# santiagolmedo/gnn_qot_estimation

Hardware: AMD Instinct MI355X
Metric: graphs/sec (train step) on 100-node/400-edge synthetic topologies, batch=1024 (higher is better)
Workload: dtype f32; 1 GPU; configs[1]: 2-layer TopologicalGNN (TransformerConv+NNConv) hidden=64, 100-node/400-directed-edge topologies, batch=1024 graphs per GPU, dropout 0.5, SGD momentum 0.9, SmoothL1; CSR build included in every step; graphs_per_gpu=1024, global_batch=1024, distinct_graphs_per_gpu=1024, launch=hip-graph replay, 4 whole steps (fwd+bwd+optimizer each) per graph, steps_per_graph=4, collective_in_graph=False, parallelism=dp1, prime_steps=45, collective_world_size=1, all_reduce_floats=68715

## Files before the change

### gnn_qot_estimation_amd/_lib.py

```python
from __future__ import annotations

import ctypes as C
import os
import subprocess

import torch

_HERE = os.path.dirname(os.path.abspath(__file__))
LIB_PATH = os.environ.get("QOT_LIB_PATH") or os.path.join(_HERE, "libqot_gnn.so")
CSRC_DIR = os.path.join(_HERE, "csrc")

_p = C.c_void_p
_i64 = C.c_int64
_int = C.c_int
_f = C.c_float
_u64 = C.c_uint64
_sz = C.c_size_t

ABI_VERSION = 11

SIGNATURES = {
    "qot_abi_version": (_int, []),
    "qot_error_string": (C.c_char_p, [_int]),
    "qot_csr_workspace_bytes": (_sz, [_i64, _i64, _int]),
    "qot_csr_build": (_int, [_p, _i64, _i64, _int, _p, _p, _p, _p, _p, _p, _p, _p, _p, _p, _sz, _p]),
    "qot_csr_gat_by_graph_supported": (_int, [_i64, _i64]),
    "qot_csr_build_gat_by_graph": (_int, [_p, _i64, _i64, _p, _p, _i64, _i64, _i64, _p, _p, _p, _p, _p, _p, _p, _p, _p, _p, _p,
                                          _p]),
    "qot_csr_build_by_graph": (_int, [_p, _i64, _i64, _p, _p, _i64, _i64, _i64, _p, _p, _p, _p, _p, _p, _p, _p, _p,
                                      _p, _p, _p, _p, _p, _p, _p]),
    "qot_i32_gather": (_int, [_p, _p, _p, _i64, _p]),
    "qot_i64_to_i32": (_int, [_p, _p, _i64, _p]),
    "qot_batch_ptr": (_int, [_p, _i64, _i64, _p, _p]),
    "qot_embed_fwd": (_int, [_p, _p, _p, _i64, _int, _int, _p]),
    "qot_embed_bwd": (_int, [_p, _p, _p, _i64, _int, _int, _p]),
    "qot_tconv_fwd_scores": (_int, [_p, _p, _p, _int, _p, _int, _p, _p, _p, _p, _p, _p, _p, _p, _i64, _int, _int,
                                    _int, _f, _f, _u64, _p, _p]),
    "qot_tconv_rows_supported": (_int, [_int, _int, _int]),
    "qot_tconv_rows_npad": (_int, [_int]),
    "qot_tconv_rows_ld": (_int, [_int, _int, _int]),
    "qot_tconv_bwd_dst_rows": (_int, [_p, _p, _p, _int, _p, _p, _p, _p, _p, _p, _p, _int, _p, _p, _p, _p, _f, _f, _u64, _p,
                                      _int, _i64, _int, _p, _p, _int, _int, _p]),
    "qot_tconv_fwd_rows": (_int, [_p, _p, _p, _int, _p, _int, _p, _p, _p, _p, _p, _p, _p, _int, _i64, _int, _int, _int,
                                  _int, _f, _f, _u64, _p, _p]),
    "qot_tconv_bwd_src_rows": (_int, [_p, _p, _p, _p, _p, _int, _i64, _int, _p, _int, _p]),
    "qot_tconv_fwd": (_int, [_p, _p, _p, _p, _int, _p, _p, _p, _p, _p, _p, _p, _p, _i64, _int, _int,
                             _int, _f, _f, _u64, _p, _p]),
    "qot_tconv_fwd_tile": (_int, [_p, _p, _p, _p, _int, _p, _p, _p, _p, _p, _p, _p, _p, _i64, _int, _int, _int, _i64,
                                  _int, _f, _f, _u64, _p, _p]),
    "qot_tconv_bwd_dst_workspace_floats": (_sz, [_i64, _int, _int]),
    "qot_tconv_rows_per_block": (_int, [_int]),
    "qot_tconv_bwd_dst_blocks": (_i64, [_i64, _int, _int, _i64]),
    "qot_tconv_bwd_dst": (_int, [_p, _p, _p, _p, _int, _p, _p, _p, _p, _p, _p, _p, _p, _p, _int, _p, _p, _p, _p,
                                 _p, _f, _f, _u64, _p, _p, _p, _int, _i64, _p, _i64, _int, _int, _p]),
    "qot_tconv_bwd_src": (_int, [_p, _int, _p, _int, _p, _p, _p, _p, _p, _p, _p, _p, _int, _int, _i64, _p, _i64, _int,
                                 _p]),
    "qot_tconv_graph_supported": (_int, [_int, _int, _int, _int]),
    "qot_tconv_graph_ldm": (_int, [_int]),
    "qot_tconv_graph_row_floats": (_sz, [_int, _int, _int]),
    "qot_tconv_bwd_graph_blocks": (_int, [_i64]),
    "qot_table_scores": (_int, [_p, _p, _p, _p, _p, _p, _p, _p, _int, _int, _int, _p]),
    "qot_tconv_fwd_graph": (_int, [_p, _int, _p, _p, _p, _p, _p, _p, _p, _p, _p, _p, _p, _p, _int, _i64, _int, _int, _int,
                                   _int, _f, _f, _u64, _p, _p]),
    "qot_tconv_bwd_graph": (_int, [_p, _p, _f, _f, _u64, _p, _p, _int, _p, _p, _p, _p, _p, _p, _p, _p, _p, _p, _p, _int,
                                   _i64, _int, _int, _int, _p]),
    "qot_table_project_bwd_scores": (_int, [_p, _p, _p, _p, _p, _p, _p, _p, _p, _p, _p, _p, _int, _int, _int, _int, _p]),
    "qot_nnconv_agg": (_int, [_p, _int, _p, _p, _p, _p, _p, _p, _p, _p, _int, _p, _i64, _int, _int, _p]),
    "qot_nnconv_fused": (_int, [_p, _int, _p, _p, _p, _p, _p, _p, _p, _int, _p, _p, _p, _i64, _int, _int,
                                _int, _f, _f, _u64, _p, _p]),
    "qot_nnconv_bwd_finalize": (_int, [_p, _p, _p, _p, _p, _i64, _int, _int, _p]),
    "qot_nnconv_dw_workspace_floats": (_sz, [_i64, _int, _int]),
    "qot_nnconv_dw": (_int, [_p, _int, _p, _int, _p, _p, _p, _p, _p, _p, _p, _p, _p, _i64, _int, _int, _p]),
    "qot_gemm_tn_workspace_floats": (_sz, [_int]),
    "qot_gemm_tn": (_int, [_p, _int, _p, _int, _i64, _int, _p, _p, _p]),
    "qot_nnconv_adjoint_dw_workspace_floats": (_sz, [_int]),
    "qot_nnconv_adjoint_dw": (_int, [_p, _int, _p, _int, _p, _p, _p, _p, _p, _p, _p, _p, _p, _p, _int, _p, _i64,
                                     _int, _int, _p]),
    "qot_nnconv_gradh_workspace_floats": (_sz, [_int]),
    "qot_nnconv_gradh_fused": (_int, [_p, _int, _p, _int, _p, _p, _p, _p, _p, _p, _p, _p, _p, _p, _p, _i64, _int,
                                      _int, _p]),
    "qot_nnconv_bwd_edge": (_int, [_p, _int, _p, _int, _p, _p, _p, _p, _p, _p, _p, _p, _p, _i64, _int,
                                   _int, _p]),
    "qot_tconv_edge_attr_grad": (_int, [_p, _p, _f, _f, _u64, _p, _p, _int, _p, _p, _p, _p, _p, _p, _p, _i64, _int, _int,
                                        _p]),
    "qot_nnconv_edge_attr_grad": (_int, [_p, _int, _p, _int, _p, _p, _p, _p, _p, _p, _p, _p, _i64, _int, _int, _p]),
    "qot_act_fwd": (_int, [_p, _p, _i64, _f, _f, _u64, _p, _p]),
    "qot_act_bwd": (_int, [_p, _p, _p, _i64, _f, _f, _u64, _p, _p]),
    "qot_pool_fwd": (_int, [_p, _p, _p, _i64, _int, _p]),
    "qot_pool_bwd": (_int, [_p, _p, _p, _p, _i64, _i64, _int, _p]),
    "qot_gat_blocks": (_int, [_i64, _int, _int]),
    "qot_gat_bn_partials_floats": (_sz, [_i64, _int, _int]),
    "qot_gat_logits": (_int, [_p, _p, _p, _p, _p, _i64, _int, _int, _p]),
    "qot_gat_fwd": (_int, [_p, _p, _p, _p, _p, _p, _p, _p, _i64, _int, _int, _f, _p, _p]),
    "qot_gat_att_grad": (_int, [_p, _p, _p, _p, _p, _p, _i64, _int, _int, _p]),
    "qot_gat_chunk_rows": (_i64, [_i64, _int, _int]),
    "qot_bn_stats_from_partials": (_int, [_p, _p, _int, _i64, _i64, _int, _f, _f, _p, _p, _p, _p, _p]),
    "qot_gat_thin_supported": (_int, [_int, _int, _int]),
    "qot_gat_fwd_thin": (_int, [_p, _int, _p, _p, _p, _p, _p, _p, _p, _p, _i64, _int, _int, _f, _p, _p]),
    "qot_gat_bwd_dst_thin": (_int, [_p, _p, _int, _p, _p, _p, _p, _p, _p, _p, _p, _p, _i64, _int, _int, _f, _p, _p, _p]),
    "qot_gat_bwd_dst": (_int, [_p, _p, _p, _p, _p, _p, _p, _p, _p, _p, _i64, _int, _int, _f, _p, _p, _p]),
    "qot_gat_bwd_src": (_int, [_p, _p, _p, _p, _p, _p, _p, _p, _p, _p, _i64, _int, _int, _f, _p, _p, _p, _p]),
    "qot_bn_partials_floats": (_sz, [_i64, _int]),
    "qot_bn_stats": (_int, [_p, _i64, _int, _f, _f, _p, _p, _p, _p, _p, _p]),
    "qot_bn_apply": (_int, [_p, _p, _p, _p, _p, _p, _i64, _int, _int, _p]),
    "qot_bn_bwd_reduce": (_int, [_p, _p, _p, _p, _p, _p, _p, _i64, _int, _int, _p, _p, _p, _p]),
    "qot_bn_bwd_apply": (_int, [_p, _p, _p, _p, _p, _p, _p, _p, _p, _i64, _int, _int, _int, _p, _p]),
    "qot_bn_apply_rows": (_int, [_p, _p, _i64, _p, _p, _p, _p, _p, _int, _int, _p]),
    "qot_bn_bwd_reduce_rows": (_int, [_p, _p, _i64, _p, _p, _p, _p, _p, _int, _int, _p, _p, _p, _p]),
    "qot_bn_bwd_apply_rows": (_int, [_p, _p, _i64, _p, _p, _p, _p, _p, _p, _p, _i64, _int, _int, _p, _p]),
    "qot_sgd_momentum": (_int, [_p, _p, _p, _i64, _f, _f, _int, _p]),
    "qot_sgd_momentum_multi": (_int, [_p, _p, _p, _int, _p, _p, _i64, _f, _p, _f, _int, _p]),
    "qot_sgd_momentum_dev": (_int, [_p, _p, _p, _i64, _p, _f, _int, _p]),
    "qot_small_gemm": (_int, [_p, _i64, _i64, _p, _i64, _i64, _p, _p, _int, _int, _int, _int, _int, _p]),
    "qot_colsum_workspace_floats": (_sz, [_int]),
    "qot_colsum": (_int, [_p, _int, _i64, _int, _p, _p, _p]),
    "qot_rowsum_wide_workspace_floats": (_sz, [_i64]),
    "qot_rowsum_wide": (_int, [_p, _i64, _i64, _p, _p, _p]),
    "qot_head_fwd": (_int, [_p, _p, _p, _p, _p, _p, _p, _p, _p, _i64, _int, _int, _f, _f, _u64, _p, _p]),
    "qot_head_fwd_loss": (_int, [_p, _p, _p, _p, _p, _p, _p, _p, _p, _i64, _int, _int, _f, _f, _u64, _p, _p, _f, _p, _p, _p]),
    "qot_head_train": (_int, [_p, _p, _p, _p, _p, _p, _p, _f, _p, _p, _p, _p, _p, _i64, _int, _int, _f, _f, _u64, _p, _int,
                              _f, _f, _u64, _p, _p]),
    "qot_head_train_blocks": (_int, [_i64, _int]),
    "qot_head_bwd_workspace_floats": (_sz, [_int, _int]),
    "qot_head_bwd_blocks": (_int, [_i64]),
    "qot_head_bwd": (_int, [_p, _p, _p, _p, _p, _p, _p, _p, _p, _i64, _int, _int, _f, _f, _u64, _p,
                            _p, _f, _f, _u64, _p, _p]),
    "qot_act_bwd_colsum": (_int, [_p, _p, _p, _i64, _int, _f, _f, _u64, _p, _p, _p, _p]),
    "qot_smooth_l1_workspace_floats": (_sz, []),
    "qot_smooth_l1": (_int, [_p, _p, _i64, _f, _p, _p, _p, _p]),
    "qot_table_project_fwd": (_int, [_p, _p, _p, _p, _p, _p, _p, _p, _p, _p, _int, _int, _p, _p, _p]),
    "qot_table_project_bwd": (_int, [_p, _p, _p, _p, _p, _p, _p, _p, _p, _int, _int, _p]),
    "qot_table_maps": (_int, [_p, _p, _p, _p, _p, _p, _i64, _i64, _p]),
    "qot_step_advance": (_int, [_p, _p, _p]),
    "qot_gather3": (_int, [_p, _i64, _p, _i64, _p, _p, _p, _i64, _p]),
    "qot_gemm_nt": (_int, [_p, _i64, _p, _i64, _p, _i64, _i64, _int, _int, _p, _p, _p, _p]),
    "qot_gemm_nt_planes": (_int, [_p, _i64, _p, _i64, _p, _i64, _int, _int, _int, _p]),
    "qot_gemm_tn_splits": (_int, [_int, _int, _i64]),
    "qot_gemm256_takes": (_int, [_i64, _int]),
    "qot_gemm_tn_planes": (_int, [_p, _i64, _p, _i64, _p, _int, _int, _i64, _int, _p, _p, _p]),
    "qot_skinny_linear_fwd": (_int, [_p, _p, _p, _i64, _int, _int, _p]),
    "qot_skinny_linear_fwd_logits": (_int, [_p, _p, _p, _i64, _int, _int, _p, _p, _p, _p, _p]),
    "qot_gemm_nt_logits": (_int, [_p, _i64, _p, _i64, _p, _i64, _i64, _int, _int, _p, _p, _p, _p, _p, _p, _p, _p]),
    "qot_skinny_linear_dw_blocks": (_int, [_i64]),
    "qot_skinny_linear_dw": (_int, [_p, _p, _p, _i64, _int, _int, _p]),
    "qot_run_roles": (_int, [_p, _int, _p]),
    "qot_rows_gather": (_int, [_p, _p, _p, _i64, _int, _p]),
    "qot_rows_scatter": (_int, [_p, _p, _p, _i64, _int, _p]),
}

MAX_ROLES = 12
(ROLE_CSR_BY_GRAPH, ROLE_TABLE_PROJECT_FWD, ROLE_GATHER3, ROLE_SUM_ROWS, ROLE_NNCONV_FINALIZE64, ROLE_TABLE_PROJECT_BWD,
 ROLE_TABLE_SCORES, ROLE_TABLE_PROJECT_BWD_SCORES) = range(1, 9)


class Role(C.Structure):
    _fields_ = [("kind", C.c_int32), ("reserved", C.c_int32), ("p", C.c_void_p * 18), ("i", C.c_int64 * 8)]


def make_role(kind: int, ptrs, ints) -> Role:
    r = Role()
    r.kind = kind
    for k, t in enumerate(ptrs):
        r.p[k] = None if t is None else (t.data_ptr() if isinstance(t, torch.Tensor) else int(t))
    for k, v in enumerate(ints):
        r.i[k] = int(v)
    return r


def run_roles(roles, stream_handle=None):
    if not roles:
        return
    if len(roles) > MAX_ROLES:
        for k in range(0, len(roles), MAX_ROLES):
            run_roles(roles[k:k + MAX_ROLES], stream_handle)
        return
    arr = (Role * len(roles))(*roles)
    code = (_lib or load()).qot_run_roles(C.addressof(arr), len(roles), stream() if stream_handle is None else stream_handle)
    if code != 0:
        check(code, "qot_run_roles")


_lib = None


class QotError(RuntimeError):
    """A libqot_gnn entry point returned a non-zero status."""


def build_library(verbose: bool = False) -> str:
    cmd = ["make", "-C", CSRC_DIR, "-j", str(min(8, os.cpu_count() or 1))]
    res = subprocess.run(cmd, capture_output=True, text=True)
    if res.returncode != 0:
        raise RuntimeError("building libqot_gnn.so failed:\n" + res.stdout[-4000:] + res.stderr[-8000:])
    if verbose:
        print(res.stdout[-2000:])
    return LIB_PATH


def load():
    global _lib
    if _lib is not None:
        return _lib
    if not os.path.exists(LIB_PATH):
        raise QotError(
            f"{LIB_PATH} not found: build it with `python -c 'import __graft_entry__ as g; g.build()'` "
            "or `make -C gnn_qot_estimation_amd/csrc` -- there is no CPU fallback for the HIP path"
        )
    lib = C.CDLL(LIB_PATH)
    for name, (res, args) in SIGNATURES.items():
        fn = getattr(lib, name)
        fn.restype = res
        fn.argtypes = args
    if lib.qot_abi_version() != ABI_VERSION:
        raise QotError(f"libqot_gnn ABI version {lib.qot_abi_version()} != {ABI_VERSION} expected by this package: "
                       "rebuild with `make -C gnn_qot_estimation_amd/csrc`")
    _lib = lib
    return lib


def ptr(t):
    return None if t is None else t.data_ptr()


_raw_stream = getattr(torch._C, "_cuda_getCurrentRawStream", None)
_raw_device = getattr(torch._C, "_cuda_getDevice", None)


def stream():
    if _raw_stream is not None and _raw_device is not None:
        return _raw_stream(_raw_device())
    return torch.cuda.current_stream().cuda_stream


def check(code: int, what: str):
    if code != 0:
        msg = load().qot_error_string(code).decode()
        raise QotError(f"{what} failed with status {code}: {msg}")


def call(name: str, *args):
    if any(isinstance(a, torch.Tensor) for a in args):
        raw = tuple(a.data_ptr() if isinstance(a, torch.Tensor) else a for a in args)
    else:
        raw = args
    code = getattr(_lib or load(), name)(*raw, stream())
    if code != 0:
        check(code, name)
```

### gnn_qot_estimation_amd/csrc/nnconv_gradh64.hip

```cpp
#include "common.hpp"
#include "mfma_tile.hpp"

namespace qot {

constexpr int kGaLd = 516;

constexpr int kGhCap = 256;

template <int D, int VARIANT = 0>
__global__ __launch_bounds__(256, 2) void nnconv_gradh64_kernel(
    const float* __restrict__ g, int ldg, const float* __restrict__ x, int ldx, const float* __restrict__ ea,
    const float* __restrict__ w1, const float* __restrict__ b1, const int32_t* __restrict__ rowptr,
    const int32_t* __restrict__ col, const int32_t* __restrict__ eidx, const float* __restrict__ invdeg,
    const float* __restrict__ Bp, float* __restrict__ partials, int64_t N) {
    constexpr int K = 2 * D;
    static_assert(K <= 8, "one k per lane of the 8-lane group");
    constexpr int NB = K * 2;
    constexpr int NBW = NB / 4;
    constexpr int EPG = kGhCap / 32;
    constexpr int EPF = 5;
    __shared__ __attribute__((aligned(16))) float Gt[8 * 2 * 32 * 4];
    __shared__ __attribute__((aligned(16))) float GAt[32 * (K * 64 + 4)];
    __shared__ int sj[kGhCap], sr[kGhCap];
    __shared__ __attribute__((aligned(16))) float sea[kGhCap * D];
    __shared__ int rp_l[36];
    constexpr int LDGA = K * 64 + 4;
    float4* Gt4 = reinterpret_cast<float4*>(Gt);
    const int lane = threadIdx.x & 63, wave = threadIdx.x >> 6;
    const int r31 = lane & 31, hi = lane >> 5;
    const int sub = threadIdx.x & 7, il = threadIdx.x >> 3;
    const int c0 = 8 * sub;
    const int64_t ntiles = (N + 31) / 32;

    float wrow[D], brow, aw[D], ab = 0.f;
    brow = (sub < K) ? b1[sub] : 0.f;
#pragma unroll
    for (int d = 0; d < D; ++d) { wrow[d] = (sub < K) ? w1[sub * D + d] : 0.f; aw[d] = 0.f; }

    auto edge = [&](int r, const float4& x0, const float4& x1, const float (&ee)[D]) {
        float pd[8];
#pragma unroll
        for (int k = 0; k < 8; ++k) {
            float a = 0.f;
            if (k < K) {
                const float4 u0 = *reinterpret_cast<const float4*>(&GAt[r * LDGA + k * 64 + c0]);
                const float4 u1 = *reinterpret_cast<const float4*>(&GAt[r * LDGA + k * 64 + c0 + 4]);
                float a0 = u0.x * x0.x, a1 = u0.y * x0.y;
                a0 = fmaf(u0.z, x0.z, a0); a1 = fmaf(u0.w, x0.w, a1);
                a0 = fmaf(u1.x, x1.x, a0); a1 = fmaf(u1.y, x1.y, a1);
                a0 = fmaf(u1.z, x1.z, a0); a1 = fmaf(u1.w, x1.w, a1);
                a = a0 + a1;
            }
            pd[k] = a;
        }
        float t4[4];
#pragma unroll
        for (int m = 0; m < 4; ++m) {
            const float keep = (sub & 4) ? pd[m + 4] : pd[m];
            const float send = (sub & 4) ? pd[m] : pd[m + 4];
            t4[m] = keep + dpp_move<0x141>(send);
        }
        float t2[2];
#pragma unroll
        for (int m = 0; m < 2; ++m) {
            const float keep = (sub & 2) ? t4[m + 2] : t4[m];
            const float send = (sub & 2) ? t4[m] : t4[m + 2];
            t2[m] = keep + dpp_move<0x4E>(send);
        }
        const float keep = (sub & 1) ? t2[1] : t2[0];
        const float send = (sub & 1) ? t2[0] : t2[1];
        const float tot = keep + dpp_move<0xB1>(send);
        float pre = brow;
#pragma unroll
        for (int d = 0; d < D; ++d) pre = fmaf(wrow[d], ee[d], pre);
        const float gh = (pre > 0.f && sub < K) ? tot : 0.f;
        ab += gh;
#pragma unroll
        for (int d = 0; d < D; ++d) aw[d] = fmaf(gh, ee[d], aw[d]);
    };

#pragma unroll 1
    for (int64_t it = 0;; ++it) {
        const int64_t tile = xcd_tile(it, ntiles);
        if (tile < 0) break;
        const int64_t tile0 = tile * 32;
        const int64_t i = tile0 + il;
        const int64_t tend = (tile0 + 32 < N) ? tile0 + 32 : N;
        float4 bf[2][8];
        {
            const float4* bp = reinterpret_cast<const float4*>(Bp) + (int64_t)(wave * NBW) * 8 * 64 + lane;
#pragma unroll
            for (int gq = 0; gq < 8; ++gq) bf[0][gq] = bp[gq * 64];
        }
        const int e_t0 = rowptr[tile0], e_t1 = rowptr[tend];
        const int nt = e_t1 - e_t0;
        const int ncap = nt < kGhCap ? nt : kGhCap;
        int64_t my_e = 0;
        if ((int)threadIdx.x < ncap) {
            sj[threadIdx.x] = col[e_t0 + threadIdx.x];
            my_e = eidx[e_t0 + threadIdx.x];
        }
        if (threadIdx.x < 33) rp_l[threadIdx.x] = rowptr[tile0 + threadIdx.x < N ? tile0 + threadIdx.x : N];
        {
            float4 g0 = f4zero(), g1 = f4zero();
            if (i < N) {
                const float sc = invdeg[i];
                const int beg = rowptr[i], end = rowptr[i + 1];
                g0 = scale4(sc, ld4(g + i * ldg + c0)); g1 = scale4(sc, ld4(g + i * ldg + c0 + 4));
                const int lim = e_t0 + ncap;
                for (int p = beg + sub; p < end && p < lim; p += 8) sr[p - e_t0] = il;
            }
            Gt4[at4_slot(sub, 0, il)] = make_float4(g0.x, g0.z, g1.x, g1.z);
            Gt4[at4_slot(sub, 1, il)] = make_float4(g0.y, g0.w, g1.y, g1.w);
        }
        float my_ea[D];
#pragma unroll
        for (int d = 0; d < D; ++d) my_ea[d] = ((int)threadIdx.x < ncap) ? ea[my_e * D + d] : 0.f;
        lds_barrier();
        const int mine = (ncap - il + 31) / 32;
        float4 xr0[EPF], xr1[EPF];
#pragma unroll
        for (int t = 0; t < EPF; ++t) {
            if (t < mine) {
                const float* xp = x + (int64_t)sj[il + 32 * t] * ldx + c0;
                xr0[t] = ld4(xp); xr1[t] = ld4(xp + 4);
            }
        }
        if (VARIANT != 3) {
            float4 af[8];
#pragma unroll
            for (int gq = 0; gq < 8; ++gq) af[gq] = Gt4[at4_slot(gq, hi, r31)];
#pragma unroll
            for (int t = 0; t < NBW; ++t) {
                const int nb = wave * NBW + t;
                if (t + 1 < NBW) {
                    const float4* bp = reinterpret_cast<const float4*>(Bp) +
                                       (int64_t)((VARIANT == 5) ? wave * NBW : nb + 1) * 8 * 64 + lane;
#pragma unroll
                    for (int gq = 0; gq < 8; ++gq) bf[(t + 1) & 1][gq] = bp[gq * 64];
                }
                f32x16 c;
#pragma unroll
                for (int r = 0; r < 16; ++r) c[r] = 0.f;
#pragma unroll
                for (int gq = 0; gq < 8; ++gq) {
                    c = __builtin_amdgcn_mfma_f32_32x32x2f32(af[gq].x, bf[t & 1][gq].x, c, 0, 0, 0);
                    c = __builtin_amdgcn_mfma_f32_32x32x2f32(af[gq].y, bf[t & 1][gq].y, c, 0, 0, 0);
                    c = __builtin_amdgcn_mfma_f32_32x32x2f32(af[gq].z, bf[t & 1][gq].z, c, 0, 0, 0);
                    c = __builtin_amdgcn_mfma_f32_32x32x2f32(af[gq].w, bf[t & 1][gq].w, c, 0, 0, 0);
                }
#pragma unroll
                for (int r = 0; r < 16; ++r) {
                    const int row = (r & 3) + 8 * (r >> 2) + 4 * hi;
                    GAt[row * LDGA + nb * 32 + r31] = c[r];
                }
            }
        }
        if ((int)threadIdx.x < ncap) {
#pragma unroll
            for (int d = 0; d < D; ++d) sea[threadIdx.x * D + d] = my_ea[d];
        }
        lds_barrier();
        if (VARIANT != 2) {
#pragma unroll
            for (int t = 0; t < EPF; ++t) {
                if (t < mine) {
                    const int s = il + 32 * t;
                    float ee[D];
#pragma unroll
                    for (int d = 0; d < D; ++d) ee[d] = sea[s * D + d];
                    edge(sr[s], xr0[t], xr1[t], ee);
                }
            }
            for (int t = EPF; t < mine; ++t) {
                const int s = il + 32 * t;
                const float* xp = x + (int64_t)sj[s] * ldx + c0;
                const float4 y0 = ld4(xp), y1 = ld4(xp + 4);
                float ee[D];
#pragma unroll
                for (int d = 0; d < D; ++d) ee[d] = sea[s * D + d];
                edge(sr[s], y0, y1, ee);
            }
            for (int s = kGhCap + il; s < nt; s += 32) {
                const int pp = e_t0 + s;
                int lo = 0;
#pragma unroll
                for (int st = 16; st > 0; st >>= 1)
                    if (rp_l[lo + st] <= pp) lo += st;
                const int64_t e = eidx[pp];
                const float* xp = x + (int64_t)col[pp] * ldx + c0;
                const float4 y0 = ld4(xp), y1 = ld4(xp + 4);
                float ee[D];
#pragma unroll
                for (int d = 0; d < D; ++d) ee[d] = ea[e * D + d];
                edge(lo, y0, y1, ee);
            }
        }
        lds_barrier();
    }
    float* red = GAt;
#pragma unroll
    for (int d = 0; d < D; ++d) red[(d * 32 + il) * 8 + sub] = aw[d];
    red[(D * 32 + il) * 8 + sub] = ab;
    lds_barrier();
    if (threadIdx.x < (D + 1) * 8) {
        const int s8 = threadIdx.x & 7, d = threadIdx.x >> 3;
        float sum = 0.f;
        for (int g32 = 0; g32 < 32; ++g32) sum += red[(d * 32 + g32) * 8 + s8];
        if (s8 < K) partials[(int64_t)blockIdx.x * (K * (D + 1)) + (d < D ? s8 * D + d : K * D + s8)] = sum;
    }
}

}

using namespace qot;

int qot_nnconv_gradh64_launch(const float* grad_out, int ld_g, const float* x, int ld_x, const float* edge_attr, const float* w1,
                              const float* b1, const int32_t* rowptr, const int32_t* col, const int32_t* eid, const float* invdeg,
                              const float* b_perm, float* workspace, int64_t N, int D, int grid, int variant, hipStream_t stream) {
#ifdef QOT_DIAG
    if (variant >= 1 && variant <= 5 && D == 4) {
#define QOT_GH_V(V) nnconv_gradh64_kernel<4, V><<<grid, 256, 0, stream>>>(grad_out, ld_g, x, ld_x, edge_attr, w1, b1, rowptr, col, \
                                                                        eid, invdeg, b_perm, workspace, N)
        switch (variant) {
            case 1: QOT_GH_V(1); break;
            case 2: QOT_GH_V(2); break;
            case 3: QOT_GH_V(3); break;
            case 4: QOT_GH_V(4); break;
            default: QOT_GH_V(5); break;
        }
#undef QOT_GH_V
        QOT_LAUNCH_CHECK();
        return QOT_OK;
    }
#endif
    (void)variant;
    QOT_DISPATCH_D(D, {
        if (kD <= 4)
            nnconv_gradh64_kernel<(kD <= 4 ? kD : 4)><<<grid, 256, 0, stream>>>(
                grad_out, ld_g, x, ld_x, edge_attr, w1, b1, rowptr, col, eid, invdeg, b_perm, workspace, N);
    });
    QOT_LAUNCH_CHECK();
    return QOT_OK;
}
```

### gnn_qot_estimation_amd/csrc/nnconv_mfma.hip

```cpp
#include "common.hpp"
#include "mfma_tile.hpp"
#include "nnconv_finalize_dev.hpp"

namespace qot {

template <int D, bool TRANSPOSE, int GV = 0>
__device__ __forceinline__ void nnconv_gather_tile(
    float* __restrict__ At, const float* __restrict__ x, int ldx, const float* __restrict__ ea,
    const float* __restrict__ w1, const float* __restrict__ b1, const int32_t* __restrict__ rowptr,
    const int32_t* __restrict__ col, const int32_t* __restrict__ eidx, const float* __restrict__ invdeg,
    int64_t tile0, int64_t N, float4& root0, float4& root1) {
    constexpr int K = 2 * D;
    const int sub = threadIdx.x & 7, il = threadIdx.x >> 3;
    const int c0 = 8 * sub;
    const int64_t i = tile0 + il;
    float4 acc0[K + 1], acc1[K + 1];
    root0 = f4zero(); root1 = f4zero();
    int beg = 0, end = 0;
    float srow = 0.f;
    if (i < N) {
        beg = rowptr[i]; end = rowptr[i + 1];
        if (!TRANSPOSE) srow = invdeg[i];
        root0 = ld4(x + i * ldx + c0);
        root1 = ld4(x + i * ldx + c0 + 4);
    }
    const int own = (i < N) ? (int)i : 0;
#define QOT_ACC(FIRSTSLOT, H, X, A) ((FIRSTSLOT) ? scale4((H), (X)) : fma4((H), (X), (A)))
#define QOT_EDGE4(U0, FIRST)                                                                            \
        {                                                                                               \
            float4 xa[4], xb[4];                                                                        \
            float sc[4];                                                                                \
            int jj[4];                                                                                  \
            jj[0] = group8_bcast<U0 + 0>(myj); jj[1] = group8_bcast<U0 + 1>(myj);                       \
            jj[2] = group8_bcast<U0 + 2>(myj); jj[3] = group8_bcast<U0 + 3>(myj);                       \
            sc[0] = group8_bcast<U0 + 0>(mysc); sc[1] = group8_bcast<U0 + 1>(mysc);                     \
            sc[2] = group8_bcast<U0 + 2>(mysc); sc[3] = group8_bcast<U0 + 3>(mysc);                     \
            _Pragma("unroll") for (int u = 0; u < 4; ++u) {                                             \
                const float* xr = x + (int64_t)(GV == 6 ? (jj[u] & 1) : jj[u]) * ldx + c0;              \
                xa[u] = ld4(xr);                                                                        \
                xb[u] = ld4(xr + 4);                                                                    \
            }                                                                                           \
            _Pragma("unroll") for (int kk = 0; kk < (GV == 8 ? 1 : K); ++kk) {                          \
                const float h0 = group8_bcast<U0 + 0>(myh[kk]), h1 = group8_bcast<U0 + 1>(myh[kk]);     \
                acc0[kk] = QOT_ACC(FIRST, h0, xa[0], acc0[kk]); acc1[kk] = QOT_ACC(FIRST, h0, xb[0], acc1[kk]); \
                acc0[kk] = fma4(h1, xa[1], acc0[kk]); acc1[kk] = fma4(h1, xb[1], acc1[kk]);             \
            }                                                                                           \
            if (GV == 8 && (FIRST)) {                                                                   \
                _Pragma("unroll") for (int kk = 1; kk < K; ++kk) { acc0[kk] = f4zero(); acc1[kk] = f4zero(); } \
            }                                                                                           \
            acc0[K] = QOT_ACC(FIRST, sc[0], xa[0], acc0[K]); acc1[K] = QOT_ACC(FIRST, sc[0], xb[0], acc1[K]); \
            acc0[K] = fma4(sc[1], xa[1], acc0[K]); acc1[K] = fma4(sc[1], xb[1], acc1[K]);               \
             \
             \
            if (cnt > U0 + 2) {                                                                         \
                _Pragma("unroll") for (int kk = 0; kk < (GV == 8 ? 1 : K); ++kk) {                      \
                    const float h2 = group8_bcast<U0 + 2>(myh[kk]), h3 = group8_bcast<U0 + 3>(myh[kk]); \
                    acc0[kk] = fma4(h2, xa[2], acc0[kk]); acc1[kk] = fma4(h2, xb[2], acc1[kk]);         \
                    acc0[kk] = fma4(h3, xa[3], acc0[kk]); acc1[kk] = fma4(h3, xb[3], acc1[kk]);         \
                }                                                                                       \
                _Pragma("unroll") for (int u = 2; u < 4; ++u) {                                         \
                    acc0[K] = fma4(sc[u], xa[u], acc0[K]);                                              \
                    acc1[K] = fma4(sc[u], xb[u], acc1[K]);                                              \
                }                                                                                       \
            }                                                                                           \
        }
#define QOT_FWD_BATCH(FIRST)                                                                            \
    {                                                                                                   \
        const int p = base + sub;                                                                       \
        int myj = own;                                                                                  \
        float myh[K], mysc = 0.f;                                                                       \
        _Pragma("unroll") for (int kk = 0; kk < K; ++kk) myh[kk] = 0.f;                                 \
        if (p < end) {                                                                                  \
            myj = (GV == 7) ? (int)(i ^ (p & 31)) : col[p];                                             \
            const int64_t e = (GV == 7) ? (int64_t)p : (int64_t)eidx[p];                                \
            float ee[D];                                                                                \
            _Pragma("unroll") for (int d = 0; d < D; ++d) ee[d] = ea[e * D + d];                        \
            mysc = TRANSPOSE ? invdeg[myj] : srow;                                                      \
            _Pragma("unroll") for (int kk = 0; kk < K; ++kk) {                                          \
                float h = b1[kk];                                                                       \
                _Pragma("unroll") for (int d = 0; d < D; ++d) h = fmaf(w1[kk * D + d], ee[d], h);       \
                myh[kk] = fmaxf(h, 0.f) * mysc;                                                         \
            }                                                                                           \
        }                                                                                               \
        const int cnt = (end - base < 8) ? end - base : 8;                                              \
        QOT_EDGE4(0, FIRST)                                                                             \
        if (cnt > 4) QOT_EDGE4(4, false)                                                                \
    }
    int base = beg;
    QOT_FWD_BATCH(true)
    for (base = beg + 8; base < end; base += 8) QOT_FWD_BATCH(false)
#undef QOT_FWD_BATCH
#undef QOT_EDGE4
#undef QOT_ACC
    float4* At4 = reinterpret_cast<float4*>(At);
#pragma unroll
    for (int kk = 0; kk <= K; ++kk) {
        const int g = kk * 8 + sub;
        At4[at4_slot(g, 0, il)] = make_float4(acc0[kk].x, acc0[kk].z, acc1[kk].x, acc1[kk].z);
        At4[at4_slot(g, 1, il)] = make_float4(acc0[kk].y, acc0[kk].w, acc1[kk].y, acc1[kk].w);
    }
}

#ifdef QOT_DIAG
#define QOT_DIAG_SECTION 1
#include "diag/nnconv_mfma_diag.inc"
#undef QOT_DIAG_SECTION
#endif

#ifdef QOT_DIAG
#define QOT_DIAG_SECTION 2
#include "diag/nnconv_mfma_diag.inc"
#undef QOT_DIAG_SECTION
#else
#define QOT_STAMP(slot)
#endif

template <int D, bool TRANSPOSE, int VARIANT = 0>
__global__ __launch_bounds__(256, 2) void nnconv_mfma64_kernel(
    const float* __restrict__ x, int ldx, const float* __restrict__ ea, const float* __restrict__ w1,
    const float* __restrict__ b1, const int32_t* __restrict__ rowptr, const int32_t* __restrict__ col,
    const int32_t* __restrict__ eidx, const float* __restrict__ invdeg, const float* __restrict__ Wp,
    const float* __restrict__ bias, float* __restrict__ out, int64_t N, ActParams act) {
    constexpr int K = 2 * D;
    constexpr int KM = (K + 1) * 64;
    constexpr int GM = KM / 16;
    constexpr int CH = 4;
    __shared__ __attribute__((aligned(16))) float At[KM * 32];
    const int64_t ntiles = (N + 31) / 32;
    const float bz = bias ? bias[((threadIdx.x >> 6) & 1) * 32 + (threadIdx.x & 31)] : 0.f;
    const uint64_t drop_step = (act.enabled && act.thr16) ? (uint64_t)act.step[0] : 0;
#pragma unroll 1
    for (int64_t it = 0;; ++it) {
    const int64_t tile = xcd_tile(it, ntiles);
    if (tile < 0) break;
    const int64_t tile0 = tile * 32;
    float4 root0, root1;
    unsigned long long t_prev = 0;
    if (VARIANT == 3 || VARIANT == 9) t_prev = __builtin_amdgcn_s_memtime();

#ifdef QOT_DIAG
    if (VARIANT == 11) {
        nnconv_gather_tile_rank1_shape<D>(At, x, ldx, rowptr, col, tile0, N, root0, root1);
    } else
#endif
    if (VARIANT != 1 && VARIANT != 4 && VARIANT != 5 && VARIANT != 9) {
        nnconv_gather_tile<D, TRANSPOSE, (VARIANT >= 6 && VARIANT <= 8) ? VARIANT : 0>(At, x, ldx, ea, w1, b1, rowptr, col, eidx, invdeg, tile0, N, root0, root1);
    } else {
        for (int t = threadIdx.x; t < KM * 32; t += 256) At[t] = 1.0f + (float)(t & 7);
        root0 = root1 = make_float4(1.f, 1.f, 1.f, 1.f);
    }
    const float4* At4 = reinterpret_cast<const float4*>(At);
    const int lane = threadIdx.x & 63, wave = threadIdx.x >> 6;
    const int nh = wave & 1, kh = wave >> 1;
    const int r31 = lane & 31, hi = lane >> 5;
    const float4* wpn = reinterpret_cast<const float4*>(Wp) + (int64_t)nh * (2 * GM + 8) * 64 + lane;
    const float4* wp = wpn + (int64_t)kh * GM * 64;
    const float4* rbp = wpn + (int64_t)(2 * GM + kh * 4) * 64;
    asm volatile("" : "+v"(rbp));
    float4 rb[4];
#pragma unroll
    for (int u = 0; u < 4; ++u) rb[u] = rbp[u * 64];
    constexpr int NCH = GM / CH;
    constexpr int NB = 4;
    float4 bb[NB][CH];
#pragma unroll
    for (int q = 0; q < NB - 1; ++q)
#pragma unroll
        for (int u = 0; u < CH; ++u) bb[q][u] = wp[(q * CH + u) * 64];
    QOT_STAMP(0)
    lds_barrier();
    QOT_STAMP(1)
    if (VARIANT == 2) {
        if (threadIdx.x < 32 && tile0 + threadIdx.x < N) out[(tile0 + threadIdx.x) * 64] = At[threadIdx.x * 33] + root0.x + rb[0].x + bb[0][0].x;
        __syncthreads();
        continue;
    }

    f32x16 c;
#pragma unroll
    for (int r = 0; r < 16; ++r) c[r] = 0.f;
    int ch = 0;
#pragma unroll 1
    for (; ch + NB <= NCH; ch += NB) {
#pragma unroll
        for (int q = 0; q < NB; ++q) {
            if (ch + q + NB - 1 < NCH && VARIANT != 4 && VARIANT != 5 && VARIANT != 9) {
#pragma unroll
                for (int u = 0; u < CH; ++u) bb[(q + NB - 1) % NB][u] = wp[((ch + q + NB - 1) * CH + u) * 64];
            }
#pragma unroll
            for (int u = 0; u < CH; ++u) {
                if (VARIANT == 5 || VARIANT == 9) {
                    const float4 a = rb[u & 3], b = bb[q][u];
                    c = __builtin_amdgcn_mfma_f32_32x32x2f32(a.x, b.x, c, 0, 0, 0);
                    c = __builtin_amdgcn_mfma_f32_32x32x2f32(a.y, b.y, c, 0, 0, 0);
                    c = __builtin_amdgcn_mfma_f32_32x32x2f32(a.z, b.z, c, 0, 0, 0);
                    c = __builtin_amdgcn_mfma_f32_32x32x2f32(a.w, b.w, c, 0, 0, 0);
                } else {
                    c = mfma_group(At4, kh * GM + (ch + q) * CH + u, hi, r31, bb[q][u], c);
                }
            }
        }
    }
#pragma unroll
    for (int q = 0; q < NB - 1; ++q) {
        if (ch + q < NCH) {
#pragma unroll
            for (int u = 0; u < CH; ++u) c = mfma_group(At4, kh * GM + (ch + q) * CH + u, hi, r31, bb[q][u], c);
        }
    }
    QOT_STAMP(2)
    lds_barrier();
    QOT_STAMP(3)
    {
        float4* At4 = reinterpret_cast<float4*>(At);
        const int sub = threadIdx.x & 7, il = threadIdx.x >> 3;
        At4[at4_slot(sub, 0, il)] = make_float4(root0.x, root0.z, root1.x, root1.z);
        At4[at4_slot(sub, 1, il)] = make_float4(root0.y, root0.w, root1.y, root1.w);
    }
    __syncthreads();
#pragma unroll
    for (int u = 0; u < 4; ++u) c = mfma_group(At4, kh * 4 + u, hi, r31, rb[u], c);
    QOT_STAMP(4)
    float* red = At + 64 * 32;
    if (kh) {
#pragma unroll
        for (int r = 0; r < 8; ++r) red[((2 + nh) * 8 + r) * 64 + lane] = c[r];
    } else {
#pragma unroll
        for (int r = 0; r < 8; ++r) red[(nh * 8 + r) * 64 + lane] = c[8 + r];
    }
    lds_barrier();
    {
        const int colg = nh * 32 + r31;
        float v[8];
        if (kh) {
#pragma unroll
            for (int r = 0; r < 8; ++r) v[r] = c[8 + r] + red[(nh * 8 + r) * 64 + lane] + bz;
        } else {
#pragma unroll
            for (int r = 0; r < 8; ++r) v[r] = c[r] + red[((2 + nh) * 8 + r) * 64 + lane] + bz;
        }
        uint32_t zlo[8], zhi[8];
        const bool drop = act.enabled && act.thr16;
        if (drop) {
            const int jq = r31 & 3;
            uint32_t mylo[2], myhi[2];
#pragma unroll
            for (int t = 0; t < 2; ++t) {
                const int rr = kh * 8 + 2 * jq + t;
                const int row = (rr & 3) + 8 * (rr >> 2) + 4 * hi;
                const uint64_t flat = (uint64_t)((tile0 + row) * 64 + colg);
                const uint64_t z = act_hash64(act.seed, drop_step, flat >> 2);
                mylo[t] = (uint32_t)z; myhi[t] = (uint32_t)(z >> 32);
            }
#define QOT_ZSHARE(S)                                                                                   \
            zlo[2 * (S)] = __builtin_amdgcn_update_dpp(0, mylo[0], (S) * 0x55, 0xF, 0xF, true);         \
            zhi[2 * (S)] = __builtin_amdgcn_update_dpp(0, myhi[0], (S) * 0x55, 0xF, 0xF, true);         \
            zlo[2 * (S) + 1] = __builtin_amdgcn_update_dpp(0, mylo[1], (S) * 0x55, 0xF, 0xF, true);     \
            zhi[2 * (S) + 1] = __builtin_amdgcn_update_dpp(0, myhi[1], (S) * 0x55, 0xF, 0xF, true);
            QOT_ZSHARE(0) QOT_ZSHARE(1) QOT_ZSHARE(2) QOT_ZSHARE(3)
#undef QOT_ZSHARE
        }
#pragma unroll
        for (int r = 0; r < 8; ++r) {
            const int rr = kh * 8 + r;
            const int row = (rr & 3) + 8 * (rr >> 2) + 4 * hi;
            const int64_t i = tile0 + row;
            float y = v[r];
            if (act.enabled) {
                y = y > 0.f ? y : act.slope * y;
                if (drop) {
                    const uint64_t z = ((uint64_t)zhi[r] << 32) | zlo[r];
                    const bool keep = ((uint32_t)(z >> (16 * (colg & 3))) & 0xFFFFu) >= act.thr16;
                    y = keep ? y * act.keep_scale : 0.f;
                }
            }
            if (i < N) out[i * 64 + colg] = y;
        }
    }
    QOT_STAMP(5)
    lds_barrier();
    QOT_STAMP(6)
    }
}


template <int D, int VARIANT = 0>
__global__ __launch_bounds__(512, 2) void nnconv_adjoint_dw64_kernel(
    const float* __restrict__ g, int ldg, const float* __restrict__ xf, int ldx, const float* __restrict__ ea,
    const float* __restrict__ w1, const float* __restrict__ b1, const int32_t* __restrict__ rowptr_t,
    const int32_t* __restrict__ col_t, const int32_t* __restrict__ eid_t, const float* __restrict__ invdeg,
    const float* __restrict__ Wp, float* __restrict__ gx, float* __restrict__ slabs, int64_t N) {
    constexpr int K = 2 * D;
    constexpr int KT = (K + 2) * 64;
    constexpr int GQ = KT / 8 / 4;
    constexpr int MB = KT / 32;
    constexpr int TPW = MB * 2 / 8;
    static_assert(GQ % 4 == 0 || GQ % 5 == 0, "chunking");
    constexpr int CH = (GQ % 4 == 0) ? 4 : 5;
    __shared__ __attribute__((aligned(16))) float Ut[KT * 32];
    __shared__ __attribute__((aligned(16))) float red[8 * 3 * 4 * 64];
    __shared__ __attribute__((aligned(16))) float xs[32 * 64];
    float4* Ut4 = reinterpret_cast<float4*>(Ut);
    const int lane = threadIdx.x & 63, wave = threadIdx.x >> 6;
    const int r31 = lane & 31, hi = lane >> 5;
    const int nh = wave & 1, kq = wave >> 1;
    const int ah = wave & 1, mb0 = wave >> 1;
    const int64_t ntiles = (N + 31) / 32;

    f32x16 dw[TPW];
#pragma unroll
    for (int t = 0; t < TPW; ++t)
#pragma unroll
        for (int r = 0; r < 16; ++r) dw[t][r] = 0.f;
    int dwoff[4];
    {
        const int kcol = mb0 * 32 + r31;
        const int gg = kcol >> 3, within = kcol & 7;
        const int base0 = ((2 * gg + (within & 1)) * 32) * 4 + (within >> 1);
        const int m = gg & 7;
#pragma unroll
        for (int b = 0; b < 4; ++b) dwoff[b] = base0 + ((((b ^ (m >> 1)) << 1) | (hi ^ (m & 1))) << 2);
    }
    const float4* wp = reinterpret_cast<const float4*>(Wp) + ((int64_t)nh * (KT / 8) + kq * GQ) * 64 + lane;
#ifdef QOT_ADJ_SETPRIO
    if (wave >= 4) __builtin_amdgcn_s_setprio(1);
#endif

#pragma unroll 1
    for (int64_t it = 0;; ++it) {
        const int64_t tile = xcd_tile(it, ntiles);
        if (tile < 0) break;
        const int64_t tile0 = tile * 32;
        float4 xown;
        {
            const int64_t j = tile0 + (threadIdx.x >> 4);
            xown = (j < N) ? ld4(xf + j * ldx + 4 * (threadIdx.x & 15)) : f4zero();
        }
        if (VARIANT != 4) {
            const int sub = threadIdx.x & 15, il = threadIdx.x >> 4;
            const int c0 = 4 * sub;
            const int64_t j = tile0 + il;
            float4 acc[K + 2];
            acc[K + 1] = f4zero();
            int beg = 0, end = 0;
            if (j < N) { beg = rowptr_t[j]; end = rowptr_t[j + 1]; acc[K + 1] = ld4(g + j * ldg + c0); }
            const int own = (j < N) ? (int)j : 0;
#define QOT_ADJ_EDGE(U)                                                                                  \
                {                                                                                        \
                    const int64_t i = (VARIANT == 1) ? (int64_t)(row16_bcast<U>(myi) & 1) : (int64_t)row16_bcast<U>(myi); \
                    gr[(U) & 3] = ld4(g + i * ldg + c0);                                                 \
                    sc[(U) & 3] = row16_bcast<U>(mysc);                                                  \
                }
#define QOT_ADJ_FMA(U, FIRSTSLOT)                                                                        \
                {                                                                                        \
                    _Pragma("unroll") for (int kk = 0; kk < (VARIANT == 6 ? 1 : K); ++kk)                \
                        acc[kk] = (FIRSTSLOT) ? scale4(row16_bcast<U>(myh[kk]), gr[(U) & 3])             \
                                              : fma4(row16_bcast<U>(myh[kk]), gr[(U) & 3], acc[kk]);     \
                    if (VARIANT == 6 && (FIRSTSLOT)) {                                                   \
                        _Pragma("unroll") for (int kk = 1; kk < K; ++kk) acc[kk] = f4zero();             \
                    }                                                                                    \
                    acc[K] = (FIRSTSLOT) ? scale4(sc[(U) & 3], gr[(U) & 3]) : fma4(sc[(U) & 3], gr[(U) & 3], acc[K]); \
                }
#define QOT_ADJ_EDGE4(U0, FIRST)                                                                         \
                {                                                                                        \
                    float4 gr[4];                                                                        \
                    float sc[4];                                                                         \
                    QOT_ADJ_EDGE(U0) QOT_ADJ_EDGE(U0 + 1) QOT_ADJ_EDGE(U0 + 2) QOT_ADJ_EDGE(U0 + 3)      \
                    QOT_ADJ_FMA(U0, FIRST) QOT_ADJ_FMA(U0 + 1, false)                                    \
                     \
                     \
                    if (cnt > U0 + 2) { QOT_ADJ_FMA(U0 + 2, false) QOT_ADJ_FMA(U0 + 3, false) }          \
                }
#define QOT_ADJ_BATCH(FIRST)                                                                             \
            {                                                                                            \
                const int p = base + sub;                                                                \
                int myi = own;                                                                           \
                float myh[K], mysc = 0.f;                                                                \
                _Pragma("unroll") for (int kk = 0; kk < K; ++kk) myh[kk] = 0.f;                          \
                if (p < end) {                                                                           \
                    myi = (VARIANT == 7) ? (int)(j ^ (p & 31)) : col_t[p];        \
                    const int64_t e = (VARIANT == 7) ? (int64_t)p : (int64_t)eid_t[p];                   \
                    float ee[D];                                                                         \
                    _Pragma("unroll") for (int d = 0; d < D; ++d) ee[d] = ea[e * D + d];                 \
                    mysc = (VARIANT == 7) ? 0.25f : invdeg[myi];                                         \
                    _Pragma("unroll") for (int kk = 0; kk < K; ++kk) {                                   \
                        float h = b1[kk];                                                                \
                        _Pragma("unroll") for (int d = 0; d < D; ++d) h = fmaf(w1[kk * D + d], ee[d], h); \
                        myh[kk] = fmaxf(h, 0.f) * mysc;                                                  \
                    }                                                                                    \
                }                                                                                        \
                const int cnt = (end - base < 16) ? end - base : 16;                                     \
                QOT_ADJ_EDGE4(0, FIRST)                                                                  \
                if (cnt > 4) QOT_ADJ_EDGE4(4, false)                                                     \
                if (cnt > 8) QOT_ADJ_EDGE4(8, false)                                                     \
                if (cnt > 12) QOT_ADJ_EDGE4(12, false)                                                   \
            }
            int base = beg;
            QOT_ADJ_BATCH(true)
            for (base = beg + 16; base < end; base += 16) QOT_ADJ_BATCH(false)
#undef QOT_ADJ_BATCH
#undef QOT_ADJ_EDGE4
#undef QOT_ADJ_FMA
#undef QOT_ADJ_EDGE
#pragma unroll
            for (int kk = 0; kk < K + 2; ++kk) {
                const int gg = kk * 8 + (sub >> 1);
                float2* s0 = reinterpret_cast<float2*>(&Ut4[at4_slot(gg, 0, il)]) + (sub & 1);
                float2* s1 = reinterpret_cast<float2*>(&Ut4[at4_slot(gg, 1, il)]) + (sub & 1);
                *s0 = make_float2(acc[kk].x, acc[kk].z);
                *s1 = make_float2(acc[kk].y, acc[kk].w);
            }
        }
        {
            const int sub = threadIdx.x & 15, il = threadIdx.x >> 4;
            *reinterpret_cast<float4*>(&xs[il * 64 + 4 * sub]) = xown;
        }
        constexpr int NCH = GQ / CH;
        float4 bc[CH], bn[CH];
#pragma unroll
        for (int u = 0; u < CH; ++u) bc[u] = wp[u * 64];
        lds_barrier();
        f32x16 c;
#pragma unroll
        for (int r = 0; r < 16; ++r) c[r] = 0.f;
        if (VARIANT != 2 && VARIANT != 5) {
            int ch = 0;
#pragma unroll 1
            for (; ch + 1 < NCH; ch += 2) {
#pragma unroll
                for (int u = 0; u < CH; ++u) bn[u] = wp[((ch + 1) * CH + u) * 64];
#pragma unroll
                for (int u = 0; u < CH; ++u) c = mfma_group(Ut4, kq * GQ + ch * CH + u, hi, r31, bc[u], c);
                if (ch + 2 < NCH) {
#pragma unroll
                    for (int u = 0; u < CH; ++u) bc[u] = wp[((ch + 2) * CH + u) * 64];
                }
#pragma unroll
                for (int u = 0; u < CH; ++u) c = mfma_group(Ut4, kq * GQ + (ch + 1) * CH + u, hi, r31, bn[u], c);
            }
            if (NCH & 1) {
#pragma unroll
                for (int u = 0; u < CH; ++u) c = mfma_group(Ut4, kq * GQ + (NCH - 1) * CH + u, hi, r31, bc[u], c);
            }
        }
#define QOT_GIVE(OWNER, SLOT)                                                                        \
        _Pragma("unroll") for (int rr = 0; rr < 4; ++rr)                                             \
            red[((((OWNER) * 2 + nh) * 3 + (SLOT)) * 4 + rr) * 64 + lane] = c[4 * (OWNER) + rr];
        if (kq == 0) { QOT_GIVE(1, 0) QOT_GIVE(2, 0) QOT_GIVE(3, 0) }
        else if (kq == 1) { QOT_GIVE(0, 0) QOT_GIVE(2, 1) QOT_GIVE(3, 1) }
        else if (kq == 2) { QOT_GIVE(0, 1) QOT_GIVE(1, 1) QOT_GIVE(3, 2) }
        else { QOT_GIVE(0, 2) QOT_GIVE(1, 2) QOT_GIVE(2, 2) }
#undef QOT_GIVE
        if (VARIANT != 3 && VARIANT != 5) {
            float abuf[2][TPW], xbuf[2];
            const float* xsl = xs + hi * 64 + ah * 32 + r31;
#pragma unroll
            for (int t = 0; t < TPW; ++t) abuf[0][t] = Ut[dwoff[0] + t * 4096];
            xbuf[0] = xsl[0];
#pragma unroll
            for (int sidx = 0; sidx < 16; ++sidx) {
                const int cur = sidx & 1;
                if (sidx + 1 < 16) {
                    const int sn = sidx + 1;
#pragma unroll
                    for (int t = 0; t < TPW; ++t) abuf[cur ^ 1][t] = Ut[dwoff[sn & 3] + (sn >> 2) * 32 + t * 4096];
                    xbuf[cur ^ 1] = xsl[sn * 128];
                }
                __builtin_amdgcn_sched_barrier(0);
#pragma unroll
                for (int t = 0; t < TPW; ++t)
                    dw[t] = __builtin_amdgcn_mfma_f32_32x32x2f32(abuf[cur][t], xbuf[cur], dw[t], 0, 0, 0);
                __builtin_amdgcn_sched_barrier(0);
            }
        }
        lds_barrier();
        {
            float v[4];
            if (kq == 0) { v[0] = c[0]; v[1] = c[1]; v[2] = c[2]; v[3] = c[3]; }
            else if (kq == 1) { v[0] = c[4]; v[1] = c[5]; v[2] = c[6]; v[3] = c[7]; }
            else if (kq == 2) { v[0] = c[8]; v[1] = c[9]; v[2] = c[10]; v[3] = c[11]; }
            else { v[0] = c[12]; v[1] = c[13]; v[2] = c[14]; v[3] = c[15]; }
            const int colg = nh * 32 + r31;
#pragma unroll
            for (int rr = 0; rr < 4; ++rr) {
#pragma unroll
                for (int slot = 0; slot < 3; ++slot) v[rr] += red[(((kq * 2 + nh) * 3 + slot) * 4 + rr) * 64 + lane];
                const int reg = 4 * kq + rr;
                const int row = (reg & 3) + 8 * (reg >> 2) + 4 * hi;
                const int64_t j = tile0 + row;
                if (j < N) gx[j * 64 + colg] = v[rr];
            }
        }
        lds_barrier();
    }
    float* slab = slabs + (int64_t)blockIdx.x * KT * 64;
#pragma unroll
    for (int t = 0; t < TPW; ++t)
#pragma unroll
        for (int r = 0; r < 16; ++r) {
            const int row = (r & 3) + 8 * (r >> 2) + 4 * hi;
            slab[((mb0 + 4 * t) * 32 + row) * 64 + ah * 32 + r31] = dw[t][r];
        }
}

__global__ void adj_slab_reduce_kernel(const float* __restrict__ slabs, int nslabs, int per_group, int64_t elems,
                                       int64_t slab_stride, float* __restrict__ dst, int64_t dst_stride) {
    int64_t t = blockIdx.x * (int64_t)blockDim.x + threadIdx.x;
    if (t * 4 >= elems) return;
    const int s0 = blockIdx.y * per_group;
    int s1 = s0 + per_group;
    if (s1 > nslabs) s1 = nslabs;
    float4 acc = f4zero();
    int sidx = s0;
    for (; sidx + 8 <= s1; sidx += 8) {
        float4 v[8];
#pragma unroll
        for (int u = 0; u < 8; ++u) v[u] = ld4(slabs + (int64_t)(sidx + u) * slab_stride + 4 * t);
#pragma unroll
        for (int u = 0; u < 8; ++u) acc = add4(acc, v[u]);
    }
    for (; sidx < s1; ++sidx) acc = add4(acc, ld4(slabs + (int64_t)sidx * slab_stride + 4 * t));
    st4(dst + blockIdx.y * dst_stride + 4 * t, acc);
}

__global__ void adj_slab_final_params_kernel(const float* __restrict__ slabs, int nslabs, int64_t elems,
                                             int64_t slab_stride, float* __restrict__ dst, int K) {
    int64_t t = blockIdx.x * (int64_t)blockDim.x + threadIdx.x;
    if (t * 4 >= elems) return;
    float4 acc = f4zero();
    for (int sidx = 0; sidx < nslabs; ++sidx) acc = add4(acc, ld4(slabs + (int64_t)sidx * slab_stride + 4 * t));
    const int64_t e = 4 * t;
    const int a0 = (int)(e & 63), o = (int)((e >> 6) & 63), kb = (int)(e >> 12);
    const float v[4] = {acc.x, acc.y, acc.z, acc.w};
#pragma unroll
    for (int c = 0; c < 4; ++c) {
        const int a = a0 + c;
        int64_t idx;
        if (kb < K) idx = ((int64_t)a * 64 + o) * K + kb;
        else if (kb == K) idx = (int64_t)4096 * K + a * 64 + o;
        else idx = (int64_t)4096 * (K + 1) + o * 64 + a;
        dst[idx] = v[c];
    }
}

__global__ void gradh_partial_sum_kernel(const float* __restrict__ partials, int nblk, int n, int KD,
                                         float* __restrict__ gw1, float* __restrict__ gb1) {
    const int t = blockIdx.x * (blockDim.x >> 6) + (threadIdx.x >> 6);
    if (t >= n) return;
    const float s = wave_sum_partials(partials, nblk, n, t);
    if ((threadIdx.x & 63) == 0) { if (t < KD) gw1[t] = s; else gb1[t - KD] = s; }
}

}

using namespace qot;

int qot_nnconv_gen_launch(const float* x, int ld_x, const float* edge_attr, const float* w1, const float* b1,
                          const int32_t* rowptr, const int32_t* col, const int32_t* edge_ids, const float* invdeg,
                          int transpose, const float* w_perm, const float* bias, float* out, int64_t N, int H, int D,
                          const ActParams& ap, hipStream_t stream);
int qot_nnconv_gradh_gen_launch(const float* grad_out, int ld_g, const float* x, int ld_x, const float* edge_attr,
                                const float* w1, const float* b1, const int32_t* rowptr, const int32_t* col,
                                const int32_t* eid, const float* invdeg, const float* b_perm, float* gw1, float* gb1,
                                float* workspace, int64_t N, int H, int D, hipStream_t stream);

#ifdef QOT_DIAG
extern "C" int qot_nnconv_fused_ws(const float* x, int ld_x, const float* edge_attr, const float* w1,
                                   const float* b1, const int32_t* rowptr, const int32_t* col,
                                   const int32_t* edge_ids, const float* invdeg, int transpose,
                                   const float* w_perm, const float* bias, float* out, int64_t N, int H, int D,
                                   int act, float act_slope, float act_p, uint64_t act_seed,
                                   const int64_t* act_step, qot_stream_t stream);

static int g_variant = 0;
extern "C" void qot_debug_set_variant(int v) { g_variant = v; }
extern "C" void qot_debug_stamps(unsigned long long* host8, int reset) {
    if (reset) { unsigned long long z[8] = {0}; (void)hipMemcpyToSymbol(HIP_SYMBOL(qot::g_stamps), z, sizeof(z)); }
    else (void)hipMemcpyFromSymbol(host8, HIP_SYMBOL(qot::g_stamps), 8 * sizeof(unsigned long long));
}
#endif

extern "C" int qot_nnconv_fused(const float* x, int ld_x, const float* edge_attr, const float* w1,
                                const float* b1, const int32_t* rowptr, const int32_t* col,
                                const int32_t* edge_ids, const float* invdeg, int transpose,
                                const float* w_perm, const float* bias, float* out, int64_t N, int H, int D,
                                int act, float act_slope, float act_p, uint64_t act_seed,
                                const int64_t* act_step, qot_stream_t stream) {
    if (N < 0 || !rowptr) return QOT_ERR_BADARG;
    if (H != 16 && H != 32 && H != 64 && H != 128 && H != 256) return QOT_ERR_UNSUPPORTED;
    if (N == 0) return QOT_OK;
    if (!x || !w1 || !b1 || !invdeg || !w_perm || !out || (ld_x & 3)) return QOT_ERR_BADARG;
    if (H != 64 || transpose == 2 || transpose == 3) {
        if (D > 4) return QOT_ERR_UNSUPPORTED;
        return qot_nnconv_gen_launch(x, ld_x, edge_attr, w1, b1, rowptr, col, edge_ids, invdeg, transpose & 1, w_perm,
                                     bias, out, N, H, D, make_act(act, act_slope, act_p, act_seed, act_step),
                                     (hipStream_t)stream);
    }
#ifdef QOT_DIAG
    static int use_ws = -1;
    if (use_ws < 0) { const char* e = getenv("QOT_NNCONV_WS"); use_ws = (e && e[0] == '1') ? 1 : 0; }
    if (use_ws && D <= 4 && !g_variant)
        return qot_nnconv_fused_ws(x, ld_x, edge_attr, w1, b1, rowptr, col, edge_ids, invdeg, transpose, w_perm, bias,
                                   out, N, H, D, act, act_slope, act_p, act_seed, act_step, stream);
#endif
    int grid = grid_for(N, 32);
    if (grid > 2 * num_cus()) grid = 2 * num_cus();
    const ActParams ap = make_act(act, act_slope, act_p, act_seed, act_step);
#ifdef QOT_DIAG
    if (g_variant >= 100 && g_variant < 110 && D == 4 && !transpose) {
        const int v = g_variant - 100, g1 = grid > num_cus() ? num_cus() : grid;
        if (v == 0)
            nnconv_mfma64_kernel<4, false, 0><<<g1, 256, 0, (hipStream_t)stream>>>(
                x, ld_x, edge_attr, w1, b1, rowptr, col, edge_ids, invdeg, w_perm, bias, out, N, ap);
        else if (v == 1)
            nnconv_mfma64_kernel<4, false, 1><<<g1, 256, 0, (hipStream_t)stream>>>(
                x, ld_x, edge_attr, w1, b1, rowptr, col, edge_ids, invdeg, w_perm, bias, out, N, ap);
        else if (v == 4)
            nnconv_mfma64_kernel<4, false, 4><<<g1, 256, 0, (hipStream_t)stream>>>(
                x, ld_x, edge_attr, w1, b1, rowptr, col, edge_ids, invdeg, w_perm, bias, out, N, ap);
        else if (v == 5)
            nnconv_mfma64_kernel<4, false, 5><<<g1, 256, 0, (hipStream_t)stream>>>(
                x, ld_x, edge_attr, w1, b1, rowptr, col, edge_ids, invdeg, w_perm, bias, out, N, ap);
        else if (v == 9)
            nnconv_mfma64_kernel<4, false, 9><<<g1, 256, 0, (hipStream_t)stream>>>(
                x, ld_x, edge_attr, w1, b1, rowptr, col, edge_ids, invdeg, w_perm, bias, out, N, ap);
        else
            nnconv_mfma64_kernel<4, false, 2><<<g1, 256, 0, (hipStream_t)stream>>>(
                x, ld_x, edge_attr, w1, b1, rowptr, col, edge_ids, invdeg, w_perm, bias, out, N, ap);
        QOT_LAUNCH_CHECK();
        return QOT_OK;
    }
    if (g_variant && g_variant <= 10 && D == 4 && !transpose) {
        if (g_variant == 3)
            nnconv_mfma64_kernel<4, false, 3><<<grid, 256, 0, (hipStream_t)stream>>>(
                x, ld_x, edge_attr, w1, b1, rowptr, col, edge_ids, invdeg, w_perm, bias, out, N, ap);
        else if (g_variant == 1)
            nnconv_mfma64_kernel<4, false, 1><<<grid, 256, 0, (hipStream_t)stream>>>(
                x, ld_x, edge_attr, w1, b1, rowptr, col, edge_ids, invdeg, w_perm, bias, out, N, ap);
        else if (g_variant == 4)
            nnconv_mfma64_kernel<4, false, 4><<<grid, 256, 0, (hipStream_t)stream>>>(
                x, ld_x, edge_attr, w1, b1, rowptr, col, edge_ids, invdeg, w_perm, bias, out, N, ap);
        else if (g_variant == 5)
            nnconv_mfma64_kernel<4, false, 5><<<grid, 256, 0, (hipStream_t)stream>>>(
                x, ld_x, edge_attr, w1, b1, rowptr, col, edge_ids, invdeg, w_perm, bias, out, N, ap);
        else if (g_variant == 6)
            nnconv_mfma64_kernel<4, false, 6><<<grid, 256, 0, (hipStream_t)stream>>>(
                x, ld_x, edge_attr, w1, b1, rowptr, col, edge_ids, invdeg, w_perm, bias, out, N, ap);
        else if (g_variant == 7)
            nnconv_mfma64_kernel<4, false, 7><<<grid, 256, 0, (hipStream_t)stream>>>(
                x, ld_x, edge_attr, w1, b1, rowptr, col, edge_ids, invdeg, w_perm, bias, out, N, ap);
        else if (g_variant == 8)
            nnconv_mfma64_kernel<4, false, 8><<<grid, 256, 0, (hipStream_t)stream>>>(
                x, ld_x, edge_attr, w1, b1, rowptr, col, edge_ids, invdeg, w_perm, bias, out, N, ap);
        else if (g_variant == 9)
            nnconv_mfma64_kernel<4, false, 9><<<grid, 256, 0, (hipStream_t)stream>>>(
                x, ld_x, edge_attr, w1, b1, rowptr, col, edge_ids, invdeg, w_perm, bias, out, N, ap);
        else if (g_variant == 10)
            nnconv_mfma64_kernel<4, false, 11><<<grid, 256, 0, (hipStream_t)stream>>>(
                x, ld_x, edge_attr, w1, b1, rowptr, col, edge_ids, invdeg, w_perm, bias, out, N, ap);
        else
            nnconv_mfma64_kernel<4, false, 2><<<grid, 256, 0, (hipStream_t)stream>>>(
                x, ld_x, edge_attr, w1, b1, rowptr, col, edge_ids, invdeg, w_perm, bias, out, N, ap);
        QOT_LAUNCH_CHECK();
        return QOT_OK;
    }
#endif
    QOT_DISPATCH_D(D, {
        if (transpose)
            nnconv_mfma64_kernel<kD, true><<<grid, 256, 0, (hipStream_t)stream>>>(
                x, ld_x, edge_attr, w1, b1, rowptr, col, edge_ids, invdeg, w_perm, bias, out, N, ap);
        else
            nnconv_mfma64_kernel<kD, false><<<grid, 256, 0, (hipStream_t)stream>>>(
                x, ld_x, edge_attr, w1, b1, rowptr, col, edge_ids, invdeg, w_perm, bias, out, N, ap);
    });
    QOT_LAUNCH_CHECK();
    return QOT_OK;
}

int qot_nnconv_gradh64_launch(const float* grad_out, int ld_g, const float* x, int ld_x, const float* edge_attr, const float* w1,
                              const float* b1, const int32_t* rowptr, const int32_t* col, const int32_t* eid, const float* invdeg,
                              const float* b_perm, float* workspace, int64_t N, int D, int grid, int variant, hipStream_t stream);
extern "C" size_t qot_nnconv_gradh_workspace_floats(int D) {
    return (size_t)2 * 256 * 2 * (size_t)(2 * D * (D + 1));
}

extern "C" int qot_nnconv_gradh_fused(const float* grad_out, int ld_g, const float* x, int ld_x,
                                      const float* edge_attr, const float* w1, const float* b1,
                                      const int32_t* rowptr, const int32_t* col, const int32_t* eid,
                                      const float* invdeg, const float* b_perm, float* gw1, float* gb1,
                                      float* workspace, int64_t N, int H, int D, qot_stream_t stream_) {
    hipStream_t stream = (hipStream_t)stream_;
    if (N < 0 || !rowptr) return QOT_ERR_BADARG;
    if ((H != 16 && H != 32 && H != 64 && H != 128 && H != 256) || D > 4) return QOT_ERR_UNSUPPORTED;
    if (!grad_out || !x || !w1 || !b1 || !invdeg || !b_perm || (!gw1 != !gb1) || !workspace || (ld_g & 3) || (ld_x & 3))
        return QOT_ERR_BADARG;
    if (!gw1 && H != 64) return QOT_ERR_UNSUPPORTED;
#ifdef QOT_DIAG
    if (H == 64 && g_variant == 9)
        return qot_nnconv_gradh_gen_launch(grad_out, ld_g, x, ld_x, edge_attr, w1, b1, rowptr, col, eid, invdeg, b_perm,
                                           gw1, gb1, workspace, N, H, D, stream);
#endif
    if (H != 64)
        return qot_nnconv_gradh_gen_launch(grad_out, ld_g, x, ld_x, edge_attr, w1, b1, rowptr, col, eid, invdeg, b_perm,
                                           gw1, gb1, workspace, N, H, D, stream);
    int grid = grid_for(N > 0 ? N : 1, 32);
    if (grid > 2 * num_cus()) grid = 2 * num_cus();
    const int K = 2 * D;
    int variant = 0;
#ifdef QOT_DIAG
    if (g_variant >= 31 && g_variant <= 35 && D == 4) variant = g_variant - 30;
#endif
    {
        const int rc = qot_nnconv_gradh64_launch(grad_out, ld_g, x, ld_x, edge_attr, w1, b1, rowptr, col, eid, invdeg, b_perm,
                                                 workspace, N, D, grid, variant, stream);
        if (rc != QOT_OK) return rc;
    }
    QOT_LAUNCH_CHECK();
    if (!gw1) return QOT_OK;
    const int n = K * (D + 1);
    gradh_partial_sum_kernel<<<grid_for(n, 4), 256, 0, stream>>>(workspace, grid, n, K * D, gw1, gb1);
    QOT_LAUNCH_CHECK();
    return QOT_OK;
}

extern "C" int qot_nnconv_bwd_finalize(const float* adj_workspace, const float* gradh_workspace, float* grad_params,
                                       float* gw1, float* gb1, int64_t N, int H, int D, qot_stream_t stream_) {
    if (N <= 0 || H != 64 || D < 1 || D > 4) return (H != 64 || D > 4) ? QOT_ERR_UNSUPPORTED : QOT_ERR_BADARG;
    qot_role_t r{};
    r.kind = QOT_ROLE_NNCONV_FINALIZE64;
    r.p[0] = adj_workspace; r.p[1] = gradh_workspace; r.p[2] = grad_params; r.p[3] = gw1; r.p[4] = gb1;
    r.i[0] = N; r.i[1] = D;
    return qot_run_roles(&r, 1, stream_);
}

extern "C" size_t qot_nnconv_adjoint_dw_workspace_floats(int D) {
    return (size_t)(num_cus() > 256 ? num_cus() : 256) * kAdjBlocksPerCu * (size_t)((2 * D + 2) * 64) * 64;
}

extern "C" int qot_nnconv_adjoint_dw(const float* grad_out, int ld_g, const float* x, int ld_x,
                                     const float* edge_attr, const float* w1, const float* b1,
                                     const int32_t* rowptr_t, const int32_t* col_t, const int32_t* eid_t,
                                     const float* invdeg, const float* w_perm, float* grad_x, float* gwcat_t,
                                     int param_layout, float* workspace, int64_t N, int H, int D,
                                     qot_stream_t stream_) {
    hipStream_t stream = (hipStream_t)stream_;
    if (N <= 0 || !rowptr_t) return QOT_ERR_BADARG;
    if (H != 64 || D > 4) return QOT_ERR_UNSUPPORTED;
    if (!grad_out || !x || !w1 || !b1 || !invdeg || !w_perm || !grad_x || !gwcat_t || !workspace || (ld_g & 3))
        return QOT_ERR_BADARG;
    int grid = grid_for(N, 32);
    const int cap = num_cus() * kAdjBlocksPerCu;
    if (grid > cap) grid = cap;
#ifdef QOT_DIAG
    if (g_variant >= 11 && g_variant <= 17 && D == 4) {
#define QOT_ADJ_V(V) nnconv_adjoint_dw64_kernel<4, V><<<grid, 512, 0, stream>>>(grad_out, ld_g, x, ld_x, edge_attr, w1, b1, \
            rowptr_t, col_t, eid_t, invdeg, w_perm, grad_x, workspace, N)
        switch (g_variant) {
            case 11: QOT_ADJ_V(1); break;
            case 12: QOT_ADJ_V(2); break;
            case 13: QOT_ADJ_V(3); break;
            case 14: QOT_ADJ_V(4); break;
            case 16: QOT_ADJ_V(6); break;
            case 17: QOT_ADJ_V(7); break;
            default: QOT_ADJ_V(5); break;
        }
#undef QOT_ADJ_V
        QOT_LAUNCH_CHECK();
        return QOT_OK;
    }
#endif
    QOT_DISPATCH_D(D, {
        if (kD <= 4)
            nnconv_adjoint_dw64_kernel<(kD <= 4 ? kD : 4)><<<grid, 512, 0, stream>>>(
                grad_out, ld_g, x, ld_x, edge_attr, w1, b1, rowptr_t, col_t, eid_t, invdeg, w_perm, grad_x,
                workspace, N);
    });
    QOT_LAUNCH_CHECK();
    if (param_layout == 2) return QOT_OK;
    const int64_t elems = (int64_t)(2 * D + 2) * 64 * 64;
    const int per_group = 16;
    const int groups = (grid + per_group - 1) / per_group;
    adj_slab_reduce_kernel<<<dim3(grid_for(elems / 4, 256), groups), 256, 0, stream>>>(
        workspace, grid, per_group, elems, elems, workspace, (int64_t)per_group * elems);
    QOT_LAUNCH_CHECK();
    if (param_layout)
        adj_slab_final_params_kernel<<<grid_for(elems / 4, 256), 256, 0, stream>>>(
            workspace, groups, elems, (int64_t)per_group * elems, gwcat_t, 2 * D);
    else
        adj_slab_reduce_kernel<<<dim3(grid_for(elems / 4, 256), 1), 256, 0, stream>>>(
            workspace, groups, groups, elems, (int64_t)per_group * elems, gwcat_t, 0);
    QOT_LAUNCH_CHECK();
    return QOT_OK;
}
```

### gnn_qot_estimation_amd/csrc/roles.hip

```cpp
#include <cstdlib>
#include "common.hpp"
#include "graph_prep_dev.hpp"
#include "mfma_tile.hpp"
#include "nnconv_finalize_dev.hpp"
#include "reduce_dev.hpp"
#include "small_dev.hpp"
#include "tconv_graph_dev.hpp"

namespace qot {

struct RoleTable {
    int n;
    int first[QOT_MAX_ROLES + 1];
    qot_role_t role[QOT_MAX_ROLES];
};

template <typename T>
__device__ __forceinline__ T* rp(const qot_role_t& r, int k) { return reinterpret_cast<T*>(const_cast<void*>(r.p[k])); }

#define QOT_ROLE_H(H, ...)                                            \
    switch (H) {                                                      \
        case 16:  { constexpr int kH = 16;  __VA_ARGS__; } break;     \
        case 32:  { constexpr int kH = 32;  __VA_ARGS__; } break;     \
        case 64:  { constexpr int kH = 64;  __VA_ARGS__; } break;     \
        case 128: { constexpr int kH = 128; __VA_ARGS__; } break;     \
        case 256: { constexpr int kH = 256; __VA_ARGS__; } break;     \
        default: break;                                               \
    }

__global__ __launch_bounds__(256) void roles_kernel(const RoleTable t_by_value) {
    extern __shared__ __attribute__((aligned(16))) int dyn_lds[];
#if defined(__HIP_DEVICE_COMPILE__)
    typedef const RoleTable __attribute__((address_space(4))) * KernargTable;
    const RoleTable& t = *(const RoleTable*)(KernargTable)__builtin_amdgcn_kernarg_segment_ptr();
    (void)t_by_value;
#else
    const RoleTable& t = t_by_value;
#endif
    int r = 0;
    while (r + 1 < t.n && (int)blockIdx.x >= t.first[r + 1]) ++r;
    const qot_role_t& ro = t.role[r];
    const int vb = (int)blockIdx.x - t.first[r];
    switch (ro.kind) {
    case QOT_ROLE_CSR_BY_GRAPH:
        csr_by_graph_body(rp<const int64_t>(ro, 0), ro.i[0], ro.i[1], rp<const int64_t>(ro, 1), rp<const int64_t>(ro, 2),
                          ro.i[2], rp<int32_t>(ro, 3), rp<int32_t>(ro, 4), rp<int32_t>(ro, 5), rp<int32_t>(ro, 6),
                          rp<int32_t>(ro, 7), rp<int32_t>(ro, 8), rp<int32_t>(ro, 9), rp<int32_t>(ro, 10),
                          rp<float>(ro, 11), rp<int32_t>(ro, 12), (int)ro.i[3], (int)ro.i[4], rp<const int64_t>(ro, 13),
                          rp<int32_t>(ro, 14), rp<int32_t>(ro, 15), rp<int32_t>(ro, 16), rp<int32_t>(ro, 17), (int64_t)vb,
                          dyn_lds);
        break;
    case QOT_ROLE_TABLE_PROJECT_FWD: {
        const Proj4 p{{rp<const float>(ro, 1), rp<const float>(ro, 3), rp<const float>(ro, 5), rp<const float>(ro, 7)},
                      {rp<const float>(ro, 2), rp<const float>(ro, 4), rp<const float>(ro, 6), rp<const float>(ro, 8)}};
        QOT_ROLE_H((int)ro.i[1], table_project_fwd_body<kH, 1>(rp<const float>(ro, 0), p, rp<float>(ro, 9), rp<int64_t>(ro, 10),
                                                               rp<int64_t>(ro, 11), (int)ro.i[0], vb,
                                                               reinterpret_cast<float*>(dyn_lds)));
        break;
    }
    case QOT_ROLE_GATHER3:
        gather3_body(rp<const float>(ro, 0), (int)ro.i[0], rp<const float>(ro, 1), (int)ro.i[1], rp<const float>(ro, 2),
                     rp<const int32_t>(ro, 3), rp<float>(ro, 4), ro.i[2], (int64_t)vb);
        break;
    case QOT_ROLE_SUM_ROWS:
        sum_rows_body(rp<const float>(ro, 0), rp<float>(ro, 1), ro.i[0], ro.i[1], ro.i[2], (int)ro.i[3], vb,
                      reinterpret_cast<float*>(dyn_lds));
        break;
    case QOT_ROLE_NNCONV_FINALIZE64:
        nnconv_bwd_finalize64_body(rp<const float>(ro, 0), (int)ro.i[2], ro.i[3], rp<float>(ro, 2), (int)ro.i[4], (int)ro.i[5],
                                   rp<const float>(ro, 1), (int)ro.i[6], (int)ro.i[7], (int)ro.i[4] * (int)ro.i[1],
                                   rp<float>(ro, 3), rp<float>(ro, 4), vb);
        break;
    case QOT_ROLE_TABLE_PROJECT_BWD: {
        const Proj4 p{{rp<const float>(ro, 2), rp<const float>(ro, 3), rp<const float>(ro, 4), rp<const float>(ro, 5)},
                      {nullptr, nullptr, nullptr, nullptr}};
        QOT_ROLE_H((int)ro.i[1], table_project_bwd_body<kH, 1>(rp<const float>(ro, 0), rp<const float>(ro, 1), p, rp<float>(ro, 6),
                                                               rp<float>(ro, 7), rp<float>(ro, 8), (int)ro.i[0], vb,
                                                               reinterpret_cast<float*>(dyn_lds)));
        break;
    }
    case QOT_ROLE_TABLE_SCORES:
        QOT_ROLE_H((int)ro.i[1], table_scores_body<kH>(rp<const float>(ro, 0), rp<const float>(ro, 1), rp<const float>(ro, 2),
                                                       rp<const float>(ro, 3), rp<const float>(ro, 4), rp<const float>(ro, 5),
                                                       rp<float>(ro, 6), rp<float>(ro, 7), (int)ro.i[0], (int)ro.i[2], vb,
                                                       reinterpret_cast<float*>(dyn_lds)));
        break;
    case QOT_ROLE_TABLE_PROJECT_BWD_SCORES: {
        const Proj4 p{{rp<const float>(ro, 4), rp<const float>(ro, 5), rp<const float>(ro, 6), rp<const float>(ro, 7)},
                      {nullptr, nullptr, nullptr, nullptr}};
        QOT_ROLE_H((int)ro.i[2], table_project_bwd_scores_body<kH>(rp<const float>(ro, 0), rp<const float>(ro, 1),
                                                                   rp<const float>(ro, 2), rp<const float>(ro, 3), p,
                                                                   rp<float>(ro, 8), rp<float>(ro, 9), rp<float>(ro, 10),
                                                                   rp<float>(ro, 11), (int)ro.i[0], (int)ro.i[1], (int)ro.i[3], vb,
                                                                   reinterpret_cast<float*>(dyn_lds)));
        break;
    }
    default:
        break;
    }
}

template <int H>
__global__ __launch_bounds__(256) void table_project_fwd_block_kernel(const float* __restrict__ table, Proj4 p,
                                                                      float* __restrict__ out, int64_t* __restrict__ counter,
                                                                      int64_t* __restrict__ snapshot, int V) {
    extern __shared__ __attribute__((aligned(16))) int dyn_lds[];
    table_project_fwd_body<H, kTableBlock>(table, p, out, counter, snapshot, V, (int)blockIdx.x, reinterpret_cast<float*>(dyn_lds));
}
template <int H>
__global__ __launch_bounds__(256) void table_project_bwd_block_kernel(const float* __restrict__ gp, const float* __restrict__ table,
                                                                      Proj4 p, float* __restrict__ gtable, float* __restrict__ gw,
                                                                      float* __restrict__ gb, int V) {
    extern __shared__ __attribute__((aligned(16))) int dyn_lds[];
    table_project_bwd_body<H, kTableBlock>(gp, table, p, gtable, gw, gb, V, (int)blockIdx.x, reinterpret_cast<float*>(dyn_lds));
}

}

using namespace qot;

static bool width_ok(int64_t H) { return H == 16 || H == 32 || H == 64 || H == 128 || H == 256; }

static int plan_role(qot_role_t& r, int64_t* blocks, size_t* lds) {
    *blocks = 0;
    *lds = 0;
    const void* const* p = r.p;
    int64_t* i = r.i;
    switch (r.kind) {
    case QOT_ROLE_CSR_BY_GRAPH: {
        const int64_t E = i[0], N = i[1], B = i[2], mn = i[3], me = i[4];
        if (p[13] && (!p[14] || (E > 0 && (!p[15] || !p[16])))) return QOT_ERR_BADARG;
        if (E < 0 || N < 0 || B <= 0 || mn < 0 || me < 0 || !p[3] || !p[7] || !p[11]) return QOT_ERR_BADARG;
        if (N >= (int64_t(1) << 31) - 1 || E >= (int64_t(1) << 31) - 1) return QOT_ERR_UNSUPPORTED;
        if (mn > kByGraphMaxNodes || by_graph_lds_bytes(mn, me) > kByGraphLdsMax) return QOT_ERR_UNSUPPORTED;
        if (!p[1] || !p[2] || (E > 0 && (!p[0] || !p[4] || !p[5] || !p[6] || !p[8] || !p[9] || !p[10]))) return QOT_ERR_BADARG;
        *blocks = B;
        *lds = by_graph_lds_bytes(mn, me);
        return QOT_OK;
    }
    case QOT_ROLE_TABLE_PROJECT_FWD: {
        const int64_t V = i[0], H = i[1];
        if (V <= 0 || (p[10] && !p[11])) return QOT_ERR_BADARG;
        if (!width_ok(H)) return QOT_ERR_UNSUPPORTED;
        for (int k = 0; k < 10; ++k) if (!p[k]) return QOT_ERR_BADARG;
        const int R = table_rows_per_block(V);
        *blocks = (V + R - 1) / R;
        *lds = (size_t)R * H * 4;
        return QOT_OK;
    }
    case QOT_ROLE_GATHER3: {
        const int64_t n0 = i[0], n1 = i[1], n = i[2];
        if (n <= 0 || n0 < 0 || n1 < 0 || n0 + n1 > 0x7fffffff) return QOT_ERR_BADARG;
        for (int k = 0; k < 5; ++k) if (!p[k]) return QOT_ERR_BADARG;
        *blocks = (n + 255) / 256;
        return QOT_OK;
    }
    case QOT_ROLE_SUM_ROWS: {
        const int64_t nblk = i[0], n = i[1];
        int64_t per = i[2];
        if (nblk <= 0 || n <= 0 || per < 0 || !p[0] || !p[1]) return QOT_ERR_BADARG;
        if (per == 0 || per > nblk) per = nblk;
        i[2] = per;
        const int64_t groups = (nblk + per - 1) / per;
        const bool v4 = (n % 4 == 0) && ((uintptr_t)p[0] % 16 == 0) && ((uintptr_t)p[1] % 16 == 0);
        i[3] = v4 ? 1 : 0;
        const int64_t cols = v4 ? n / 4 : n;
        i[4] = (cols + kSumCols - 1) / kSumCols;
        *blocks = i[4] * groups;
        *lds = (size_t)256 * 16;
        if (*blocks > 0x7fffffff) return QOT_ERR_UNSUPPORTED;
        return QOT_OK;
    }
    case QOT_ROLE_NNCONV_FINALIZE64: {
        const int64_t N = i[0], D = i[1];
        if (N <= 0 || D < 1) return QOT_ERR_BADARG;
        if (D > 4) return QOT_ERR_UNSUPPORTED;
        for (int k = 0; k < 5; ++k) if (!p[k]) return QOT_ERR_BADARG;
        int64_t agrid = (N + 31) / 32;
        if (agrid > (int64_t)num_cus() * kAdjBlocksPerCu) agrid = (int64_t)num_cus() * kAdjBlocksPerCu;
        int64_t hgrid = (N + 31) / 32;
        if (hgrid > 2 * (int64_t)num_cus()) hgrid = 2 * (int64_t)num_cus();
        const int64_t K = 2 * D;
        const int64_t elems = (K + 2) * 64 * 64;
        const int64_t nb1 = (elems / 4 * 16 + 255) / 256;
        const int64_t hn = K * (D + 1);
        i[2] = agrid; i[3] = elems; i[4] = K; i[5] = nb1; i[6] = hgrid; i[7] = hn;
        *blocks = nb1 + (hn + 3) / 4;
        return QOT_OK;
    }
    case QOT_ROLE_TABLE_PROJECT_BWD: {
        const int64_t V = i[0], H = i[1];
        if (V <= 0) return QOT_ERR_BADARG;
        if (!width_ok(H)) return QOT_ERR_UNSUPPORTED;
        for (int k = 0; k < 9; ++k) if (!p[k]) return QOT_ERR_BADARG;
        const int R = table_rows_per_block(V);
        *blocks = 4 * H / R + (V + R - 1) / R;
        *lds = (size_t)(512 * R + R * 4 * H) * 4;
        return QOT_OK;
    }
    case QOT_ROLE_TABLE_SCORES: {
        const int64_t n = i[0], H = i[1], D = i[2];
        if (n <= 0 || D <= 0) return QOT_ERR_BADARG;
        if (!width_ok(H) || D > 8) return QOT_ERR_UNSUPPORTED;
        for (int k = 0; k < 8; ++k) if (!p[k]) return QOT_ERR_BADARG;
        *blocks = (n + kScoreRows - 1) / kScoreRows;
        *lds = (size_t)kScoreRows * (3 * H + 1) * 4;
        return QOT_OK;
    }
    case QOT_ROLE_TABLE_PROJECT_BWD_SCORES: {
        const int64_t V = i[0], n = i[1], H = i[2], D = i[3];
        if (V <= 0 || n <= 0 || n > V || D <= 0) return QOT_ERR_BADARG;
        if (!width_ok(H) || D > 8 || table_rows_per_block(V) > 1) return QOT_ERR_UNSUPPORTED;
        if (n > kTgMaxN) return QOT_ERR_UNSUPPORTED;
        for (int k = 0; k < 12; ++k) if (!p[k]) return QOT_ERR_BADARG;
        *blocks = 4 * H + V + 1;
        *lds = (size_t)tg_bwd_scores_lds_floats((int)n, (int)H, (int)D) * 4;
        return QOT_OK;
    }
    default:
        return QOT_ERR_BADARG;
    }
}

__global__ __launch_bounds__(1024) void csr_by_graph_wide_kernel(
    const int64_t* __restrict__ ei, int64_t E, int64_t N, const int64_t* __restrict__ node_ptr,
    const int64_t* __restrict__ edge_ptr, int64_t B, int32_t* __restrict__ rowptr, int32_t* __restrict__ col,
    int32_t* __restrict__ eid, int32_t* __restrict__ row, int32_t* __restrict__ rowptr_t, int32_t* __restrict__ col_t,
    int32_t* __restrict__ pos_t, int32_t* __restrict__ eid_t, float* __restrict__ invdeg, int32_t* __restrict__ status,
    int cap_n, int cap_m, const int64_t* __restrict__ node_ids, int32_t* __restrict__ ids32, int32_t* __restrict__ colf,
    int32_t* __restrict__ colf_t, int32_t* __restrict__ ptr32) {
    extern __shared__ int wide_lds[];
    csr_by_graph_body<1024>(ei, E, N, node_ptr, edge_ptr, B, rowptr, col, eid, row, rowptr_t, col_t, pos_t, eid_t, invdeg, status,
                            cap_n, cap_m, node_ids, ids32, colf, colf_t, ptr32, (int64_t)blockIdx.x, wide_lds);
}
constexpr size_t kCsrWideMinLds = 64 * 1024;

static int launch_wide_csr(const qot_role_t& ro, int64_t blocks, size_t lds, hipStream_t stream) {
    static size_t allowed[kMaxDevices];
    const int lrc = ensure_dyn_lds(reinterpret_cast<const void*>(csr_by_graph_wide_kernel), lds, allowed);
    if (lrc != QOT_OK) return lrc;
    auto P = [&](int k) { return const_cast<void*>(ro.p[k]); };
    csr_by_graph_wide_kernel<<<(int)blocks, 1024, lds, stream>>>(
        (const int64_t*)P(0), ro.i[0], ro.i[1], (const int64_t*)P(1), (const int64_t*)P(2), ro.i[2], (int32_t*)P(3), (int32_t*)P(4),
        (int32_t*)P(5), (int32_t*)P(6), (int32_t*)P(7), (int32_t*)P(8), (int32_t*)P(9), (int32_t*)P(10), (float*)P(11),
        (int32_t*)P(12), (int)ro.i[3], (int)ro.i[4], (const int64_t*)P(13), (int32_t*)P(14), (int32_t*)P(15), (int32_t*)P(16),
        (int32_t*)P(17));
    QOT_LAUNCH_CHECK();
    return QOT_OK;
}

static int launch_heavy_role(const qot_role_t& ro, int64_t blocks, size_t lds, hipStream_t stream) {
    const int V = (int)ro.i[0];
    auto P = [&](int k) { return const_cast<void*>(ro.p[k]); };
    if (ro.kind == QOT_ROLE_TABLE_PROJECT_FWD) {
        const Proj4 p{{(const float*)P(1), (const float*)P(3), (const float*)P(5), (const float*)P(7)},
                      {(const float*)P(2), (const float*)P(4), (const float*)P(6), (const float*)P(8)}};
        QOT_ROLE_H((int)ro.i[1], (table_project_fwd_block_kernel<kH><<<(int)blocks, 256, lds, stream>>>(
                                      (const float*)P(0), p, (float*)P(9), (int64_t*)P(10), (int64_t*)P(11), V)));
    } else {
        const Proj4 p{{(const float*)P(2), (const float*)P(3), (const float*)P(4), (const float*)P(5)},
                      {nullptr, nullptr, nullptr, nullptr}};
        QOT_ROLE_H((int)ro.i[1], (table_project_bwd_block_kernel<kH><<<(int)blocks, 256, lds, stream>>>(
                                      (const float*)P(0), (const float*)P(1), p, (float*)P(6), (float*)P(7), (float*)P(8), V)));
    }
    QOT_LAUNCH_CHECK();
    return QOT_OK;
}

extern "C" int qot_run_roles(const qot_role_t* roles, int n_roles, qot_stream_t stream_) {
    hipStream_t stream = (hipStream_t)stream_;
    if (n_roles < 0 || n_roles > QOT_MAX_ROLES || (n_roles > 0 && !roles)) return QOT_ERR_BADARG;
    if (n_roles == 0) return QOT_OK;
    RoleTable t;
    t.n = 0;
    size_t lds = 0;
    int64_t total = 0;
    int n_light = 0;
    for (int r = 0; r < n_roles; ++r) {
        qot_role_t ro = roles[r];
        int64_t blocks;
        size_t need;
        const int rc = plan_role(ro, &blocks, &need);
        if (rc != QOT_OK) return rc;
        if ((ro.kind == QOT_ROLE_TABLE_PROJECT_FWD || ro.kind == QOT_ROLE_TABLE_PROJECT_BWD) && table_rows_per_block(ro.i[0]) > 1) {
            const int hrc = launch_heavy_role(ro, blocks, need, stream);
            if (hrc != QOT_OK) return hrc;
            continue;
        }
        if (ro.kind == QOT_ROLE_CSR_BY_GRAPH && need > kCsrWideMinLds && !getenv("QOT_NO_WIDE_CSR")) {
            const int hrc = launch_wide_csr(ro, blocks, need, stream);
            if (hrc != QOT_OK) return hrc;
            continue;
        }
        t.role[n_light] = ro;
        t.first[n_light] = (int)total;
        ++n_light;
        total += blocks;
        if (total > 0x7fffffff) return QOT_ERR_UNSUPPORTED;
        if (need > lds) lds = need;
    }
    if (n_light == 0) return QOT_OK;
    t.n = n_light;
    for (int r = n_light; r <= QOT_MAX_ROLES; ++r) t.first[r] = (int)total;
    {
        static size_t allowed[kMaxDevices];
        const int lrc = ensure_dyn_lds(reinterpret_cast<const void*>(roles_kernel), lds, allowed);
        if (lrc != QOT_OK) return lrc;
    }
    roles_kernel<<<(int)total, 256, lds, stream>>>(t);
    QOT_LAUNCH_CHECK();
    return QOT_OK;
}
```

### gnn_qot_estimation_amd/csrc/small_dev.hpp

```cpp
#pragma once
#include "common.hpp"

namespace qot {

struct Proj4 {
    const float* w[4];
    const float* b[4];
};
__device__ __forceinline__ const float* proj_w(const Proj4& p, int s) { return s == 0 ? p.w[0] : (s == 1 ? p.w[1] : (s == 2 ? p.w[2] : p.w[3])); }
__device__ __forceinline__ const float* proj_b(const Proj4& p, int s) { return s == 0 ? p.b[0] : (s == 1 ? p.b[1] : (s == 2 ? p.b[2] : p.b[3])); }

constexpr int kTableBlock = 8;
constexpr int kTableBlockMinV = 512;
__host__ __device__ inline int table_rows_per_block(int64_t V) { return V >= kTableBlockMinV ? kTableBlock : 1; }

template <int H, int R>
__device__ __forceinline__ void table_project_fwd_rows(const float* __restrict__ table, const Proj4& p,
                                                       float* __restrict__ out, int V, int v0, float* __restrict__ row) {
    for (int c = threadIdx.x; c < R * H; c += 256) {
        const int r = c / H, a = c % H;
        row[c] = v0 + r < V ? table[(int64_t)(v0 + r) * H + a] : 0.f;
    }
    __syncthreads();
    for (int c = threadIdx.x; c < 4 * H; c += 256) {
        const int s = H >= 64 ? __builtin_amdgcn_readfirstlane(c / H) : c / H, o = c % H;
        const float* w = proj_w(p, s) + (int64_t)o * H;
        float acc[R];
        const float b0 = p.b[0][o], b1 = p.b[1][o], b2 = p.b[2][o], b3 = p.b[3][o];
        const float bz = s == 0 ? b0 : (s == 1 ? b1 : (s == 2 ? b2 : b3));
#pragma unroll
        for (int r = 0; r < R; ++r) acc[r] = bz;
#pragma unroll 4
        for (int a = 0; a < H; a += 4) {
            const float4 ww = ld4(w + a);
#pragma unroll
            for (int r = 0; r < R; ++r) {
                const float4 xv = *reinterpret_cast<const float4*>(row + r * H + a);
                acc[r] = fmaf(ww.x, xv.x, acc[r]); acc[r] = fmaf(ww.y, xv.y, acc[r]);
                acc[r] = fmaf(ww.z, xv.z, acc[r]); acc[r] = fmaf(ww.w, xv.w, acc[r]);
            }
        }
#pragma unroll
        for (int r = 0; r < R; ++r)
            if (v0 + r < V) out[(int64_t)(v0 + r) * 4 * H + c] = acc[r];
    }
}

template <int H, int R>
__device__ __forceinline__ void table_project_fwd_body(const float* __restrict__ table, const Proj4& p,
                                                       float* __restrict__ out, int64_t* __restrict__ counter,
                                                       int64_t* __restrict__ snapshot, int V, int vb, float* __restrict__ row) {
    if (counter && vb == 0 && threadIdx.x == 0) {
        const int64_t cc = counter[0] + 1;
        counter[0] = cc;
        snapshot[0] = cc;
    }
    table_project_fwd_rows<H, R>(table, p, out, V, vb * R, row);
}

template <int H, int CB>
__device__ __forceinline__ void table_project_bwd_w(const float* __restrict__ gp, const float* __restrict__ table,
                                                    float* __restrict__ gw, float* __restrict__ gb, int V, int c0,
                                                    float* __restrict__ lds) {
    constexpr int PH = (H >= 256) ? 1 : 256 / H;
    float* red = lds;
    float* redb = lds + 256 * CB;
    const int a = threadIdx.x % H, ph = threadIdx.x / H;
    float acc[CB], sb[CB];
#pragma unroll
    for (int u = 0; u < CB; ++u) { acc[u] = 0.f; sb[u] = 0.f; }
    if constexpr (CB == 1) {
        const int c = c0;
        int v = ph;
        for (; v + 7 * PH < V; v += 8 * PH) {
            float gv[8], tv[8];
#pragma unroll
            for (int u = 0; u < 8; ++u) {
                gv[u] = gp[(int64_t)(v + u * PH) * 4 * H + c];
                tv[u] = table[(int64_t)(v + u * PH) * H + a];
            }
#pragma unroll
            for (int u = 0; u < 8; ++u) { acc[0] = fmaf(gv[u], tv[u], acc[0]); sb[0] += gv[u]; }
        }
        for (; v < V; v += PH) {
            const float gv = gp[(int64_t)v * 4 * H + c];
            acc[0] = fmaf(gv, table[(int64_t)v * H + a], acc[0]);
            sb[0] += gv;
        }
    } else {
        static_assert(CB == 1 || CB == 8, "two float4 of gp per row");
        int v = ph;
        for (; v + 3 * PH < V; v += 4 * PH) {
            float4 g0[4], g1[4];
            float tv[4];
#pragma unroll
            for (int u = 0; u < 4; ++u) {
                const float* gr = gp + (int64_t)(v + u * PH) * 4 * H + c0;
                g0[u] = ld4(gr); g1[u] = ld4(gr + 4);
                tv[u] = table[(int64_t)(v + u * PH) * H + a];
            }
#pragma unroll
            for (int u = 0; u < 4; ++u) {
                const float gv[8] = {g0[u].x, g0[u].y, g0[u].z, g0[u].w, g1[u].x, g1[u].y, g1[u].z, g1[u].w};
#pragma unroll
                for (int q = 0; q < 8; ++q) { acc[q] = fmaf(gv[q], tv[u], acc[q]); sb[q] += gv[q]; }
            }
        }
        for (; v < V; v += PH) {
            const float* gr = gp + (int64_t)v * 4 * H + c0;
            const float4 g0 = ld4(gr), g1 = ld4(gr + 4);
            const float tv = table[(int64_t)v * H + a];
            const float gv[8] = {g0.x, g0.y, g0.z, g0.w, g1.x, g1.y, g1.z, g1.w};
#pragma unroll
            for (int q = 0; q < 8; ++q) { acc[q] = fmaf(gv[q], tv, acc[q]); sb[q] += gv[q]; }
        }
    }
#pragma unroll
    for (int u = 0; u < CB; ++u) { red[u * 256 + threadIdx.x] = acc[u]; redb[u * 256 + threadIdx.x] = sb[u]; }
    __syncthreads();
    if (ph == 0) {
#pragma unroll
        for (int u = 0; u < CB; ++u) {
            float s = acc[u], t = sb[u];
            for (int k = 1; k < PH; ++k) { s += red[u * 256 + k * H + a]; t += redb[u * 256 + k * H + a]; }
            gw[(int64_t)(c0 + u) * H + a] = s;
            if (a == 0) gb[c0 + u] = t;
        }
    }
}

template <int H, int R>
__device__ __forceinline__ void table_project_bwd_t(const float* __restrict__ gp, const Proj4& p, float* __restrict__ gtable,
                                                    int V, int v0, float* __restrict__ lds) {
    constexpr int PH = (H >= 256) ? 1 : 256 / H;
    float* red = lds;
    float* g = lds + 512 * R;
    const int a = threadIdx.x % H, ph = threadIdx.x / H;
    for (int c = threadIdx.x; c < R * 4 * H; c += 256) {
        const int r = c / (4 * H);
        g[c] = v0 + r < V ? gp[(int64_t)(v0 + r) * 4 * H + c % (4 * H)] : 0.f;
    }
    __syncthreads();
    float acc[R];
#pragma unroll
    for (int r = 0; r < R; ++r) acc[r] = 0.f;
    for (int c0 = ph; c0 < 4 * H; c0 += 8 * PH) {
        float wv[8];
#pragma unroll
        for (int u = 0; u < 8; ++u) {
            const int c = c0 + u * PH;
            const int cc = c < 4 * H ? c : ph;
            wv[u] = proj_w(p, cc / H)[(int64_t)(cc % H) * H + a];
        }
#pragma unroll
        for (int u = 0; u < 8; ++u) {
            const int c = c0 + u * PH;
            if (c < 4 * H) {
#pragma unroll
                for (int r = 0; r < R; ++r) acc[r] = fmaf(g[r * 4 * H + c], wv[u], acc[r]);
            }
        }
    }
#pragma unroll
    for (int r = 0; r < R; ++r) red[r * 256 + threadIdx.x] = acc[r];
    __syncthreads();
    if (ph == 0) {
#pragma unroll
        for (int r = 0; r < R; ++r) {
            float s = acc[r];
            for (int k = 1; k < PH; ++k) s += red[r * 256 + k * H + a];
            if (v0 + r < V) gtable[(int64_t)(v0 + r) * H + a] = s;
        }
    }
}

template <int H, int R>
__device__ __forceinline__ void table_project_bwd_body(const float* __restrict__ gp, const float* __restrict__ table,
                                                       const Proj4& p, float* __restrict__ gtable,
                                                       float* __restrict__ gw, float* __restrict__ gb, int V, int vb,
                                                       float* __restrict__ lds) {
    constexpr int NW = 4 * H / R;
    if (vb < NW) table_project_bwd_w<H, R>(gp, table, gw, gb, V, vb * R, lds);
    else table_project_bwd_t<H, R>(gp, p, gtable, V, (vb - NW) * R, lds);
}

__device__ __forceinline__ void gather3_body(const float* __restrict__ s0, int n0, const float* __restrict__ s1, int n1,
                                             const float* __restrict__ s2, const int32_t* __restrict__ idx,
                                             float* __restrict__ out, int64_t n, int64_t vb) {
    const int64_t i = vb * 256 + threadIdx.x;
    if (i >= n) return;
    const int v = idx[i];
    out[i] = v < 0 ? 0.f : (v < n0 ? s0[v] : (v < n0 + n1 ? s1[v - n0] : s2[v - n0 - n1]));
}

}
```

### gnn_qot_estimation_amd/functional.py

```python
from __future__ import annotations

import os
from typing import Optional

import torch

from . import _lib, launch_group as LG
from .graph import GraphIndex, require_cuda

P = _lib.ptr


def _f32c(t: torch.Tensor) -> torch.Tensor:
    if t.dtype != torch.float32:
        raise TypeError("the HIP path computes in fp32; got %s" % t.dtype)
    return t.contiguous()


def _off(t: torch.Tensor, floats: int) -> int:
    return t.data_ptr() + 4 * floats


class EmbedFn(torch.autograd.Function):

# ... 327 lines not shown
                per = 128
                groups = (blocks + per - 1) // per
                level1 = torch.empty(groups, H * D, dtype=torch.float32, device=dev)
                LG.defer(_lib.ROLE_SUM_ROWS, (ws, level1), (blocks, H * D, per), stage=1)
                LG.defer(_lib.ROLE_SUM_ROWS, (level1, gwe_flat), (groups, H * D, 0), stage=2)
            else:
                LG.defer(_lib.ROLE_SUM_ROWS, (ws, gwe_flat), (blocks, H * D, 0), stage=1)
        if not tiled:
            gq = gnode
        else:
            if gb == 1:
                gq = gpart[0]
            else:
                gq_flat = torch.empty(n * H4, dtype=torch.float32, device=dev)
                if LG.enabled() and ctx.table_from_project:
                    LG.defer(_lib.ROLE_SUM_ROWS, (gpart, gq_flat), (gb, n * H4, 0), stage=1)
                else:
                    wsr = torch.empty(_lib.load().qot_rowsum_wide_workspace_floats(n * H4), dtype=torch.float32, device=dev)
                    _lib.call("qot_rowsum_wide", P(gpart), gb, n * H4, P(gq_flat), P(wsr))
                gq = gq_flat.view(n, H4)
            if n < qkvs.shape[0]:
                if LG.enabled():
                    LG.flush()
                gq = torch.cat([gq, gq.new_zeros(qkvs.shape[0] - n, H4)], 0)
        return gq, gea, gwe_flat.view(H, D), None, None, None


def tconv_edge_attr_grad(g, y, act, act_step, qkvs, edge_attr, w_edge, graph: GraphIndex, maps):
    H = qkvs.shape[1] // 4
    E, D = edge_attr.shape
    gea = torch.empty(E, D, dtype=torch.float32, device=g.device)
    if act is not None:
        slope, p, seed = act
        act_args = (y, float(slope), float(p if act_step is not None else 0.0), int(seed), act_step)
    else:
        act_args = (None, 0.0, 0.0, 0, None)
    rowmap, col = (maps[0], maps[1]) if maps is not None else (None, graph.col)
    _lib.call("qot_tconv_edge_attr_grad", g, *act_args, qkvs, qkvs.shape[1], rowmap, col, graph.rowptr, graph.eid,
              edge_attr, w_edge, gea, graph.num_nodes, H, D)
    return gea


def tconv_rows_ok(qkvs: torch.Tensor, maps, H: int, D: int) -> bool:
    if maps is None or os.environ.get("QOT_NO_TCONV_ROWS"):
        return False
    B, n = maps[3]
    return (B >= 1 and n == qkvs.shape[0] and bool(_lib.load().qot_tconv_rows_supported(int(n), int(H), int(D))))


def _tconv_backward_rows(ctx, g, qkvs, edge_attr, w_edge, stats, y, act_step):
    graph, maps = ctx.graph, ctx.maps
    lib = _lib.load()
    dev = qkvs.device
    H4 = qkvs.shape[1]
    H = H4 // 4
    D = w_edge.shape[1]
    N = graph.num_nodes
    B, n = maps[3]
    colf = maps[1]
    scores = ctx.scores
    parts = int(max(1, min(B, 8)))
    npad, ldrow = lib.qot_tconv_rows_npad(n), lib.qot_tconv_rows_ld(n, H, D)
    f32 = dict(dtype=torch.float32, device=dev)
    escr = torch.empty(max(graph.cap, 1), 2, **f32)
    delta = torch.empty(N, **f32)
    gskip = torch.empty(N, H, **f32)
    drows = torch.empty(parts, n * ldrow, **f32)
    wparts = torch.empty(parts * n, H * D, **f32)
    vrows = torch.empty(parts, n * H, **f32)
    if ctx.act is not None:
        slope, p, seed = ctx.act
        act_args = (P(y), float(slope), float(p if act_step is not None else 0.0), int(seed), P(act_step))
    else:
        act_args = (None, 0.0, 0.0, 0, None)
    _lib.call("qot_tconv_bwd_dst_rows", P(g), _off(qkvs, 0), _off(qkvs, 2 * H), H4, P(edge_attr), P(w_edge), P(stats),
              P(graph.rowptr), P(colf), P(graph.eid), P(scores), scores.shape[1], P(gskip), P(escr), P(delta), *act_args,
              int(n), int(B), parts, P(drows), P(wparts), H, D)
    _lib.call("qot_tconv_bwd_src_rows", P(gskip), P(escr), P(graph.rowptr_t), P(graph.col_t), P(graph.pos_t), int(n), int(B),
              parts, P(vrows), H)
    K1 = 32 * (((npad // 32) + 1 + 7) // 8 * 8)
    S_buf = torch.zeros(n * ldrow + K1, **f32)
    S = S_buf[:n * ldrow]
    gv = torch.empty(n * H, **f32)
    gwe_g = torch.empty(H * D, **f32)
    roles = [_lib.make_role(_lib.ROLE_SUM_ROWS, (drows, S), (parts, n * ldrow, 0)),
             _lib.make_role(_lib.ROLE_SUM_ROWS, (vrows, gv), (parts, n * H, 0))]
    blocks = parts * n
    two_level = blocks > 256
    if two_level:
        per = 128
        groups = (blocks + per - 1) // per
        level1 = torch.empty(groups, H * D, **f32)
        roles.append(_lib.make_role(_lib.ROLE_SUM_ROWS, (wparts, level1), (blocks, H * D, per)))
    else:
        roles.append(_lib.make_role(_lib.ROLE_SUM_ROWS, (wparts, gwe_g), (blocks, H * D, 0)))
    _lib.run_roles(roles)
    S = S.view(n, ldrow)
    rs = 1.0 / float(H) ** 0.5
    gM = S[:, H:H + npad]
    gP = S[:, H + npad:H + npad + D]
    tq, tk = qkvs[:, 0:H], qkvs[:, H:2 * H]
    Bq = torch.zeros(H, K1, **f32)
    Bq[:, :n] = tk.t()
    Bq[:, npad:npad + D] = w_edge
    Bq.mul_(rs)
    ks = 8
    planes_q = torch.empty(ks, n * H, **f32)
    _lib.call("qot_gemm_nt_planes", P(gM), ldrow, P(Bq), K1, P(planes_q), n, H, K1, ks)
    splits = lib.qot_gemm_tn_splits(npad, H, n)
    planes_k = torch.empty(splits, npad * H, **f32)
    _lib.call("qot_gemm_tn_planes", P(gM), ldrow, _off(qkvs, 0), H4, P(planes_k), npad, H, n, splits, None, None)
    gq_, gk_ = torch.empty(n * H, **f32), torch.empty(npad * H, **f32)
    roles = [_lib.make_role(_lib.ROLE_SUM_ROWS, (planes_q, gq_), (ks, n * H, 0)),
             _lib.make_role(_lib.ROLE_SUM_ROWS, (planes_k, gk_), (splits, npad * H, 0))]
    if two_level:
        roles.append(_lib.make_role(_lib.ROLE_SUM_ROWS, (level1, gwe_g), (groups, H * D, 0)))
    _lib.run_roles(roles)
    g4 = torch.cat([gq_.view(n, H), gk_.view(npad, H)[:n] * rs, gv.view(n, H), S[:, 0:H]], dim=1)
    tqp = _small_gemm(tq, gP, None, H, D, n, 1, H4, ldrow, 1)
    gwe = torch.add(gwe_g.view(H, D), tqp, alpha=rs)
    return g4, None, gwe, None, None, None


def tconv_graph_plan(table, H: int, D: int, graph: GraphIndex, maps):
    if maps is None or graph.sizes is None or os.environ.get("QOT_NO_TCONV_GRAPH"):
        return None
    B, n = maps[3]
    if B <= 0 or n <= 0 or graph.num_nodes != B * n or table.shape[0] >= 512 or n > table.shape[0]:
        return None
    max_e = int(graph.sizes[1])
    if not _lib.load().qot_tconv_graph_supported(int(n), max_e, int(H), int(D)):
        return None
    return int(n), int(B), max_e


def tconv_graph_prepare(table, wq, bq, wk, bk, wv, bv, ws, bs, w_edge, n: int, step_pair=None, group=None):
    ts = [_f32c(t.detach()) for t in (table, wq, bq, wk, bk, wv, bv, ws, bs, w_edge)]
    require_cuda(*ts)
    table, wq, bq, wk, bk, wv, bv, ws, bs, w_edge = ts
    V, H = table.shape
    D = w_edge.shape[1]
    dev = table.device
    t4 = torch.empty(V, 4 * H, dtype=torch.float32, device=dev)
    M = torch.empty(n, _lib.load().qot_tconv_graph_ldm(n), dtype=torch.float32, device=dev)
    Pm = torch.empty(n, D, dtype=torch.float32, device=dev)
    cnt, snap = step_pair if step_pair is not None else (None, None)
    if group is not None:
        group.add(_lib.ROLE_TABLE_PROJECT_FWD, (table, wq, bq, wk, bk, wv, bv, ws, bs, t4, cnt, snap), (V, H))
        group.add(_lib.ROLE_TABLE_SCORES, (table, wq, bq, wk, bk, w_edge, M, Pm), (n, H, D))
    else:
        _lib.call("qot_table_project_fwd", table, wq, bq, wk, bk, wv, bv, ws, bs, t4, V, H, P(cnt), P(snap))
        _lib.call("qot_table_scores", table, wq, bq, wk, bk, w_edge, M, Pm, n, H, D)
    return t4, M, Pm


class TConvGraphFn(torch.autograd.Function):

    @staticmethod
    def forward(ctx, table, wq, bq, wk, bk, wv, bv, ws, bs, w_edge, edge_attr, pre, graph: GraphIndex, maps, plan, act=None):
        t4, M, Pm = pre
        n, B, max_e = plan
        edge_attr, w_edge_c = _f32c(edge_attr), _f32c(w_edge.detach())
        require_cuda(edge_attr, t4, M, Pm)
        H, D = table.shape[1], w_edge.shape[1]
        N = graph.num_nodes
        if edge_attr.shape != (graph.num_edges_in, D):
            raise ValueError(f"edge_attr must be [{graph.num_edges_in}, {D}], got {tuple(edge_attr.shape)}")
        dev = t4.device
        out = torch.empty(N, H, dtype=torch.float32, device=dev)
        E = max(graph.num_edges_in, 1)
        alpha = torch.empty(E, dtype=torch.float32, device=dev)
        ea_csr = torch.empty(E, D, dtype=torch.float32, device=dev)
        aa = torch.empty(max(N, 1), D, dtype=torch.float32, device=dev)
        _lib.call("qot_tconv_fwd_graph", t4, 4 * H, M, Pm, w_edge_c, edge_attr, graph.rowptr, maps[1], graph.eid, graph.row,
                  out, alpha, ea_csr, aa, n, B, max_e, H, D, *_act_args(act))
        ctx.save_for_backward(table, wq, wk, wv, ws, w_edge_c, t4, alpha, ea_csr, aa, out if act is not None else None,
                              act[3] if act is not None else None, edge_attr if ctx.needs_input_grad[10] else None)
        ctx.graph, ctx.maps, ctx.plan = graph, maps, plan
        ctx.act = None if act is None else (act[0], act[1], act[2])
        return out

    @staticmethod
    def backward(ctx, g):
        table, wq, wk, wv, ws, w_edge, t4, alpha, ea_csr, aa, y, act_step, edge_attr = ctx.saved_tensors
        graph, maps = ctx.graph, ctx.maps
        n, B, max_e = ctx.plan
        g = _f32c(g)
        gea = tconv_edge_attr_grad(g, y, ctx.act, act_step, t4, edge_attr, w_edge, graph, maps) \
            if ctx.needs_input_grad[10] else None
        V, H = table.shape
        D = w_edge.shape[1]
        dev = g.device
        lib = _lib.load()
        blocks, rowlen = int(lib.qot_tconv_bwd_graph_blocks(B)), int(lib.qot_tconv_graph_row_floats(n, H, D))
        partials = torch.empty(blocks, rowlen, dtype=torch.float32, device=dev)
        if ctx.act is not None:
            slope, p, seed = ctx.act
            act_args = (y, float(slope), float(p if act_step is not None else 0.0), int(seed), act_step)
        else:
            act_args = (None, 0.0, 0.0, 0, None)
        _lib.call("qot_tconv_bwd_graph", g, *act_args, t4, 4 * H, w_edge, ea_csr, alpha, aa, graph.rowptr, maps[1],
                  graph.row, graph.rowptr_t, graph.col_t, graph.pos_t, partials, n, B, max_e, H, D)
        S = partials[0] if blocks == 1 else torch.empty(rowlen, dtype=torch.float32, device=dev)
        gt = torch.empty(V * H, dtype=torch.float32, device=dev)
        gw = torch.empty(4 * H * H, dtype=torch.float32, device=dev)
        gb = torch.empty(4 * H, dtype=torch.float32, device=dev)
        gwe = torch.empty(H, D, dtype=torch.float32, device=dev)
        wq_, wk_, wv_, ws_ = (_f32c(t.detach()) for t in (wq, wk, wv, ws))
        tab = _f32c(table.detach())
        if LG.enabled():
            if blocks > 1:
                LG.defer(_lib.ROLE_SUM_ROWS, (partials, S), (blocks, rowlen, 0), stage=1)
            LG.defer(_lib.ROLE_TABLE_PROJECT_BWD_SCORES, (S, t4, w_edge, tab, wq_, wk_, wv_, ws_, gt, gw, gb, gwe),
                     (V, n, H, D), stage=2)
            LG.flush()
        else:
            if blocks > 1:
                wsr = torch.empty(lib.qot_rowsum_wide_workspace_floats(rowlen), dtype=torch.float32, device=dev)
                _lib.call("qot_rowsum_wide", partials, blocks, rowlen, S, wsr)
            _lib.call("qot_table_project_bwd_scores", S, t4, w_edge, tab, wq_, wk_, wv_, ws_, gt, gw, gb, gwe, V, n, H, D)
        gw2 = gw.view(4 * H, H)
        return (gt.view(V, H), gw2[:H], gb[:H], gw2[H:2 * H], gb[H:2 * H], gw2[2 * H:3 * H], gb[2 * H:3 * H], gw2[3 * H:],
                gb[3 * H:], gwe, gea, None, None, None, None, None)


def nnconv_wcat(w2, b2, wroot, hin, hout, k):
    return torch.cat([
        w2.view(hin, hout, k).permute(2, 0, 1).reshape(k * hin, hout),
        b2.view(hin, hout),
        wroot.t(),
    ], dim=0)


def nnconv_wcat_t(w2, b2, wroot, hin, hout, k):
    return torch.cat([
        w2.view(hin, hout, k).permute(2, 1, 0).reshape(k * hout, hin),
        b2.view(hin, hout).t(),
        wroot,
    ], dim=0)


def gemm_tn(a: torch.Tensor, g: torch.Tensor) -> torch.Tensor:
    n, kt = a.shape
    if g.shape[1] != 64 or kt % 128 != 0 or kt > 1280 or n == 0 or os.environ.get("QOT_DISABLE_GEMM_TN"):
        return a.t() @ g
    a, g = a.contiguous(), g.contiguous()
    out = torch.empty(kt, 64, dtype=torch.float32, device=a.device)
    ws = torch.empty(_lib.load().qot_gemm_tn_workspace_floats(kt), dtype=torch.float32, device=a.device)
    _lib.call("qot_gemm_tn", P(a), kt, P(g), 64, n, kt, P(out), P(ws))
    return out


_PERM_CACHE = {}


def nnconv_perm_index(kt: int, device) -> torch.Tensor:
    key = (kt, str(device))
    if key not in _PERM_CACHE:
        nh, g, l, r = torch.meshgrid(torch.arange(2), torch.arange(kt // 8), torch.arange(64), torch.arange(4),
                                     indexing="ij")
        k = 8 * g + 2 * r + (l >> 5)
        n = nh * 32 + (l & 31)
        _PERM_CACHE[key] = (k * 64 + n).reshape(-1).to(device)
    return _PERM_CACHE[key]


def nnconv_gradh_perm_index(k: int, device) -> torch.Tensor:
    key = ("gradh", k, str(device))
    if key not in _PERM_CACHE:
        nb, gq, l, r = torch.meshgrid(torch.arange(2 * k), torch.arange(8), torch.arange(64), torch.arange(4),
                                      indexing="ij")
        o = 8 * gq + 2 * r + (l >> 5)
        n = nb * 32 + (l & 31)
        _PERM_CACHE[key] = (n * 64 + o).reshape(-1).to(device)
    return _PERM_CACHE[key]


def nnconv_fused_indices(k: int, device):
    key = ("fusedidx", k, str(device))
    if key not in _PERM_CACHE:
        h = 64
        kk, a, o = torch.meshgrid(torch.arange(k), torch.arange(h), torch.arange(h), indexing="ij")
        w2_off = (a * h + o) * k + kk
        a2, o2 = torch.meshgrid(torch.arange(h), torch.arange(h), indexing="ij")
        b2_off = h * h * k + a2 * h + o2
        root_off = h * h * k + h * h + o2 * h + a2
        wcat_idx = torch.cat([w2_off.reshape(k * h, h), b2_off, root_off], 0)
        wcat_t_idx = wcat_idx.view(k + 2, h, h).transpose(1, 2).reshape((k + 2) * h, h)
        fwd = wcat_idx.reshape(-1)[nnconv_perm_index((k + 2) * h, "cpu")]
        adj = wcat_t_idx.reshape(-1)[nnconv_perm_index((k + 2) * h, "cpu")]
        gh = wcat_idx[:k * h].reshape(-1)[nnconv_gradh_perm_index(k, "cpu")]
        allidx = torch.cat([fwd, adj, gh]).to(torch.int32).contiguous().to(device)
        _PERM_CACHE[key] = (allidx, fwd.numel(), adj.numel(), gh.numel())
    return _PERM_CACHE[key]


def nnconv_pack_operands(w2, b2, wroot, k: int):
    allidx, n_f, n_a, n_g = nnconv_fused_indices(k, w2.device)
    packed = torch.empty(allidx.numel(), dtype=torch.float32, device=w2.device)
    _lib.call("qot_gather3", P(w2), w2.numel(), P(b2), b2.numel(), P(wroot), P(allidx), P(packed), allidx.numel())
    return packed[:n_f], packed[n_f:n_f + n_a], packed[n_f + n_a:]


def nnconv_pack(w2, b2, wroot, h: int, k: int, group=None):
    allidx, n_f, n_a, n_g = nnconv_fused_indices(k, w2.device) if h == 64 else nnconv_gen_indices(h, k, w2.device)
    packed = torch.empty(allidx.numel(), dtype=torch.float32, device=w2.device)
    if group is not None:
        group.add(_lib.ROLE_GATHER3, (w2, b2, wroot, allidx, packed), (w2.numel(), b2.numel(), allidx.numel()))
    else:
        _lib.call("qot_gather3", P(w2), w2.numel(), P(b2), b2.numel(), P(wroot), P(allidx), P(packed), allidx.numel())
    return packed[:n_f], packed[n_f:n_f + n_a], packed[n_f + n_a:]


GEN_WIDTHS = (16, 32, 128, 256)


def nnconv_gen_indices(h: int, k: int, device, cw: int = 0):
    key = ("genidx", h, k, str(device), cw)
    if key not in _PERM_CACHE:
        cw = cw or min(h, 64)
        n_pass, ncb, gall = h // cw, (h + 31) // 32, (k + 2) * cw // 8
        P_, CB, G_, L_, R_ = torch.meshgrid(torch.arange(n_pass), torch.arange(ncb), torch.arange(gall), torch.arange(64),
                                            torch.arange(4), indexing="ij")
        kl = 8 * G_ + 2 * R_ + (L_ >> 5)
        kk, a = kl // cw, P_ * cw + kl % cw
        col = CB * 32 + (L_ & 31)

        def wcat_off(kk, a, o):
            return torch.where(kk < k, (a * h + o) * k + kk,
                               torch.where(kk == k, h * h * k + a * h + o, h * h * (k + 1) + o * h + a))
        pad = col >= h
        colc = col.clamp(max=h - 1)
        fwd = torch.where(pad, torch.full_like(col, -1), wcat_off(kk, a, colc))
        adj = torch.where(pad, torch.full_like(col, -1), wcat_off(kk, colc, a))
        cwg = min(h, 32)
        npg, nbg, gh_ = h // cwg, k * cwg // 32, h // 8
        P2, NB, GQ, L2, R2 = torch.meshgrid(torch.arange(npg), torch.arange(nbg), torch.arange(gh_), torch.arange(64),
                                            torch.arange(4), indexing="ij")
        o = 8 * GQ + 2 * R2 + (L2 >> 5)
        n = NB * 32 + (L2 & 31)
        kq, al = n // cwg, n % cwg
        gh = ((P2 * cwg + al) * h + o) * k + kq
        allidx = torch.cat([fwd.reshape(-1), adj.reshape(-1), gh.reshape(-1)]).to(torch.int32).contiguous().to(device)
        _PERM_CACHE[key] = (allidx, fwd.numel(), adj.numel(), gh.numel())
    return _PERM_CACHE[key]


def nnconv_pack_operands_gen(w2, b2, wroot, h: int, k: int):
    allidx, n_f, n_a, n_g = nnconv_gen_indices(h, k, w2.device)
    packed = torch.empty(allidx.numel(), dtype=torch.float32, device=w2.device)
    _lib.call("qot_gather3", P(w2), w2.numel(), P(b2), b2.numel(), P(wroot), P(allidx), P(packed), allidx.numel())
    return packed[:n_f], packed[n_f:n_f + n_a], packed[n_f + n_a:]


def nnconv_edge_attr_grad(GA, x, edge_attr, w1, b1, graph: GraphIndex):
    N, hin = x.shape
    E, D = edge_attr.shape
    GA = GA.contiguous()
    gea = torch.empty(E, D, dtype=torch.float32, device=x.device)
    _lib.call("qot_nnconv_edge_attr_grad", GA, GA.shape[1], x, hin, edge_attr, w1, b1, graph.rowptr, graph.col, graph.eid,
              graph.invdeg, gea, N, hin, D)
    return gea


class NNConvFn(torch.autograd.Function):

    @staticmethod
    def forward(ctx, x, edge_attr, w1, b1, w2, b2, wroot, bias, graph: GraphIndex, act=None, side=None, packed=None):
        require_cuda(x, edge_attr, w1, b1, w2, b2, wroot, bias)
        ctx.receivers = (w1, b1, w2, b2, wroot)
        if side is not None and act is not None:
            side["bias_param"] = bias
        x, edge_attr = _f32c(x), _f32c(edge_attr)
        w1, b1, w2, b2, wroot, bias = (_f32c(t) for t in (w1, b1, w2, b2, wroot, bias))
        N, hin = x.shape
        hout = wroot.shape[0]
        K, D = w1.shape
        if K != 2 * D:
            raise _lib.QotError("NNConv edge MLP must be Linear(D, 2D) -> ReLU -> Linear(2D, Hin*Hout)")
        if edge_attr.shape != (graph.num_edges_in, D):
            raise ValueError(f"edge_attr must be [{graph.num_edges_in}, {D}], got {tuple(edge_attr.shape)}")
        if hin != hout:
            raise _lib.QotError("NNConv HIP path needs in_channels == out_channels")
        if hin != 64 and hin not in GEN_WIDTHS:
            raise _lib.QotError(f"NNConv HIP path: hidden width {hin} not in (16, 32, 64, 128, 256)")
        if D > 8:
            raise _lib.QotError("NNConv HIP path: edge_dim <= 8 (include/qot_gnn.h)")
        if D > 4:
            return NNConvFn._forward_wide_edge(ctx, x, edge_attr, w1, b1, w2, b2, wroot, bias, graph, act, side)
        wp, wp_adj, bp = packed if packed is not None else nnconv_pack(w2, b2, wroot, hin, K)
        out = torch.empty(N, hout, dtype=torch.float32, device=x.device)
        _lib.call("qot_nnconv_fused", P(x), hin, P(edge_attr), P(w1), P(b1), P(graph.rowptr), P(graph.col),
                  P(graph.eid), P(graph.invdeg), 0, P(wp), P(bias), P(out), N, hin, D, *_act_args(act))
        ctx.save_for_backward(x, edge_attr, w1, b1, w2, b2, wroot, None, wp_adj, bp, out if act is not None else None,
                              act[3] if act is not None else None)
        ctx.graph = graph
        ctx.act = None if act is None else (act[0], act[1], act[2])
        ctx.side = side if act is not None else None
        return out

    @staticmethod
    def _forward_wide_edge(ctx, x, edge_attr, w1, b1, w2, b2, wroot, bias, graph, act, side):
        N, hin = x.shape
        hout = wroot.shape[0]
        K, D = w1.shape
        A = torch.empty(N, (K + 2) * hin, dtype=torch.float32, device=x.device)
        _lib.call("qot_nnconv_agg", P(x), hin, P(edge_attr), P(w1), P(b1), P(graph.rowptr), P(graph.col),
                  P(graph.eid), None, P(graph.invdeg), 0, P(A), N, hin, D)
        out = torch.addmm(bias, A, nnconv_wcat(w2, b2, wroot, hin, hout, K))
        if act is not None:
            pre = out
            out = torch.empty_like(pre)
            _lib.call("qot_act_fwd", P(pre), P(out), pre.numel(), *_act_args(act)[1:])
        ctx.save_for_backward(x, edge_attr, w1, b1, w2, b2, wroot, A, None, None, out if act is not None else None,
                              act[3] if act is not None else None)
        ctx.graph = graph
        ctx.act = None if act is None else (act[0], act[1], act[2])
        ctx.side = side if act is not None else None
        return out

    @staticmethod
    def _backward_wide_edge(ctx, g, gbias):
        x, edge_attr, w1, b1, w2, b2, wroot, A, _, _, _, _ = ctx.saved_tensors
        graph = ctx.graph
        N, hin = x.shape
        hout = wroot.shape[0]
        K, D = w1.shape
        dev = x.device
        gwcat = gemm_tn(A, g)
        gx = None
        if ctx.needs_input_grad[0]:
            U = torch.empty(N, (K + 2) * hout, dtype=torch.float32, device=dev)
            _lib.call("qot_nnconv_agg", P(g), hout, P(edge_attr), P(w1), P(b1), P(graph.rowptr_t), P(graph.col_t),
                      P(graph.pos_t), P(graph.eid), P(graph.invdeg), 1, P(U), N, hout, D)
            gx = U @ nnconv_wcat_t(w2, b2, wroot, hin, hout, K)
        gw2 = gwcat[:K * hin].view(K, hin, hout).permute(1, 2, 0).reshape(hin * hout, K)
        gb2 = gwcat[K * hin:(K + 1) * hin].reshape(hin * hout)
        gwroot = gwcat[(K + 1) * hin:].t()
        wk = w2.view(hin, hout, K).permute(2, 0, 1).reshape(K * hin, hout)
        GA = (g @ wk.t()).contiguous()
        gw1 = torch.zeros(K, D, dtype=torch.float32, device=dev)
        gb1 = torch.zeros(K, dtype=torch.float32, device=dev)
        _lib.call("qot_nnconv_bwd_edge", P(GA), K * hin, P(x), hin, P(edge_attr), P(w1), P(b1),
                  P(graph.rowptr), P(graph.col), P(graph.eid), P(graph.invdeg), P(gw1), P(gb1), N, hin, D)
        gea = nnconv_edge_attr_grad(GA, x, edge_attr, w1, b1, graph) if ctx.needs_input_grad[1] else None
        return gx, gea, gw1, gb1, gw2, gb2, gwroot, gbias, None, None, None, None

    @staticmethod
    def backward(ctx, g):
        x, edge_attr, w1, b1, w2, b2, wroot, A, wp_adj, bp, y, act_step = ctx.saved_tensors
        graph = ctx.graph
        g = _f32c(g)
        if ctx.side is not None:
            if "gbias" not in ctx.side:
                raise RuntimeError("NNConv output was folded into the fused read-out, but the read-out's backward "
                                   "has not run: the conv output must feed only the read-out head "
                                   "(set model._qot_fold_head = False for other graphs)")
            gbias = ctx.side.pop("gbias")
        elif ctx.act is not None:
            g, gbias = act_backward_colsum(g, y, ctx.act + (act_step,))
        else:
            gbias = colsum(g)
        if A is not None:
            return NNConvFn._backward_wide_edge(ctx, g, gbias)
        N, hin = x.shape
        hout = wroot.shape[0]
        K, D = w1.shape
        dev = x.device
        hh = hin * hout
        gea = None
        if ctx.needs_input_grad[1]:
            wk = w2.view(hin, hout, K).permute(2, 0, 1).reshape(K * hin, hout)
            gea = nnconv_edge_attr_grad(g @ wk.t(), x, edge_attr, w1, b1, graph)
        gw1f = torch.empty(K * D, dtype=torch.float32, device=dev)
        gb1f = torch.empty(K, dtype=torch.float32, device=dev)
        gw1, gb1 = gw1f.view(K, D), gb1f.view(K)
        wsh = torch.empty(_lib.load().qot_nnconv_gradh_workspace_floats(D), dtype=torch.float32, device=dev)
        gpar = torch.empty((K + 2) * hh, dtype=torch.float32, device=dev)
        gradh_args = (P(g), hout, P(x), hin, P(edge_attr), P(w1), P(b1), P(graph.rowptr), P(graph.col), P(graph.eid),
                      P(graph.invdeg), P(bp))
        if hin == 64 and not os.environ.get("QOT_SPLIT_NNCONV_BWD"):
            gx = torch.empty(N, hin, dtype=torch.float32, device=dev)
            ws = torch.empty(_lib.load().qot_nnconv_adjoint_dw_workspace_floats(D), dtype=torch.float32, device=dev)
            deferred = LG.can_defer(*ctx.receivers)
            fork_mode = os.environ.get("QOT_FORK", "off") if deferred else "off"
            launch_gradh = lambda: _lib.call("qot_nnconv_gradh_fused", *gradh_args, None, None, P(wsh), N, hin, D)
            keep = (g, x, edge_attr, w1, b1, graph.rowptr, graph.col, graph.eid, graph.invdeg, bp, wsh)
            if fork_mode == "before":
                LG.fork(launch_gradh, keep=keep)
            _lib.call("qot_nnconv_adjoint_dw", P(g), hout, P(x), hin, P(edge_attr), P(w1), P(b1), P(graph.rowptr_t),
                      P(graph.col_t), P(graph.eid_t), P(graph.invdeg), P(wp_adj), P(gx), P(gpar), 2, P(ws), N, hin, D)
            if fork_mode == "after":
                LG.fork(launch_gradh, keep=keep)
            elif fork_mode != "before":
                launch_gradh()
            if deferred:
                LG.defer(_lib.ROLE_NNCONV_FINALIZE64, (ws, wsh, gpar, gw1f, gb1f), (N, D), stage=1)
            else:
                _lib.call("qot_nnconv_bwd_finalize", P(ws), P(wsh), P(gpar), P(gw1f), P(gb1f), N, hin, D)
        else:
            gx = None
            if ctx.needs_input_grad[0]:
                gx = torch.empty(N, hin, dtype=torch.float32, device=dev)
                _lib.call("qot_nnconv_fused", P(g), hout, P(edge_attr), P(w1), P(b1), P(graph.rowptr_t),
                          P(graph.col_t), P(graph.eid_t), P(graph.invdeg), 1, P(wp_adj), None, P(gx), N, hout, D,
                          0, 0.0, 0.0, 0, None)
            ws = torch.empty(_lib.load().qot_nnconv_dw_workspace_floats(N, hin, D), dtype=torch.float32, device=dev)
            _lib.call("qot_nnconv_dw", P(x), hin, P(g), hout, P(edge_attr), P(w1), P(b1), P(graph.rowptr), P(graph.col),
                      P(graph.eid), P(graph.invdeg), P(gpar), P(ws), N, hin, D)
            _lib.call("qot_nnconv_gradh_fused", *gradh_args, P(gw1), P(gb1), P(wsh), N, hin, D)
        gw2, gb2, gwroot = gpar[:hh * K].view(hh, K), gpar[hh * K:hh * (K + 1)], gpar[hh * (K + 1):].view(hout, hin)
        return gx, gea, gw1, gb1, gw2, gb2, gwroot, gbias, None, None, None, None


class ActFn(torch.autograd.Function):

    @staticmethod
    def forward(ctx, x, slope, p, seed, step_counter):
        require_cuda(x)
        x = _f32c(x)
        y = torch.empty_like(x)
        _lib.call("qot_act_fwd", P(x), P(y), x.numel(), float(slope), float(p), int(seed), P(step_counter))
        ctx.save_for_backward(y, step_counter if step_counter is not None else torch.empty(0))
        ctx.cfg = (float(slope), float(p), int(seed), step_counter is not None)
        return y

    @staticmethod
    def backward(ctx, g):
        y, counter = ctx.saved_tensors
        slope, p, seed, has_counter = ctx.cfg
        g = _f32c(g)
        gx = torch.empty_like(g)
        _lib.call("qot_act_bwd", P(g), P(y), P(gx), g.numel(), slope, p, seed, P(counter) if has_counter else None)
        return gx, None, None, None, None


class PoolFn(torch.autograd.Function):
    @staticmethod
    def forward(ctx, x, batch32, ptr32, B):
        require_cuda(x)
        x = _f32c(x)
        N, H = x.shape
        out = torch.empty(B, H, dtype=torch.float32, device=x.device)
        _lib.call("qot_pool_fwd", P(x), P(ptr32), P(out), B, H)
        ctx.save_for_backward(batch32, ptr32)
        ctx.dims = (N, H, B)
        return out

    @staticmethod
    def backward(ctx, g):
        batch32, ptr32 = ctx.saved_tensors
        N, H, B = ctx.dims
        g = _f32c(g)
        gx = torch.empty(N, H, dtype=torch.float32, device=g.device)
        _lib.call("qot_pool_bwd", P(g), P(ptr32), P(batch32), P(gx), N, B, H)
        return gx, None, None, None


class HeadFn(torch.autograd.Function):

    @staticmethod
    def forward(ctx, x, ptr32, w0, b0, w3, b3, B, act, in_act=None, side=None, loss=None):
        require_cuda(x, w0, b0, w3, b3)
        ctx.receivers = (w0, b0, w3, b3)
        x, w0, b0, w3, b3 = (_f32c(t) for t in (x, w0, b0, w3, b3))
        N, H = x.shape
        O = w3.shape[0]
        slope, p, seed, step = act
        dev = x.device
        pooled = torch.empty(B, H, dtype=torch.float32, device=dev)
        hidden = torch.empty(B, H, dtype=torch.float32, device=dev)
        out = torch.empty(B, O, dtype=torch.float32, device=dev)
        gout = loss_rows = None
        fold = in_act is not None and side is not None
        ctx.train_fused = None
        if loss is not None:
            target, beta, loss_out = loss[:3]
            target = _f32c(target.detach())
            if target.shape != (B, O):
                raise ValueError(f"target must be [{B}, {O}], got {tuple(target.shape)}")
            gout = torch.empty(B, O, dtype=torch.float32, device=dev)
            loss_rows = torch.empty(B, dtype=torch.float32, device=dev)
            ctx.loss = (loss_rows, loss_out)
            if len(loss) > 3 and loss[3] and not os.environ.get("QOT_NO_HEAD_TRAIN"):
                nb = H * H + H + O * H + O
                gx = torch.empty(N, H, dtype=torch.float32, device=dev)
                ws = torch.empty(_lib.load().qot_head_bwd_workspace_floats(H, O), dtype=torch.float32, device=dev)
                fa = (1, float(in_act[0]), float(in_act[1] if in_act[3] is not None else 0.0), int(in_act[2]), P(in_act[3])) \
                    if fold else (0, 0.0, 0.0, 0, None)
                _lib.call("qot_head_train", P(x), P(ptr32), P(w0), P(b0), P(w3), P(b3), P(target), float(beta), P(out), P(gout),
                          P(loss_rows), P(gx), P(ws), B, H, O, float(slope), float(p if step is not None else 0.0), int(seed),
                          P(step), *fa)
                ctx.train_fused = (gx, ws, gout, nb + (H if fold else 0))
                ctx.cfg = (N, H, O, B, float(slope), float(p if step is not None else 0.0), int(seed))
                ctx.fold = fold
                ctx.side = side if fold else None
                ctx.mark_non_differentiable(gout)
                ctx.set_materialize_grads(False)
                return out, gout
            _lib.call("qot_head_fwd_loss", P(x), P(ptr32), P(w0), P(b0), P(w3), P(b3), P(pooled), P(hidden), P(out), B, H,
                      O, float(slope), float(p if step is not None else 0.0), int(seed), P(step), P(target), float(beta),
                      P(gout), P(loss_rows))
        else:
            _lib.call("qot_head_fwd", P(x), P(ptr32), P(w0), P(b0), P(w3), P(b3), P(pooled), P(hidden), P(out), B, H, O,
                      float(slope), float(p if step is not None else 0.0), int(seed), P(step))
            ctx.loss = None
        ctx.save_for_backward(ptr32, w0, w3, pooled, hidden, step, x if fold else None,
                              in_act[3] if fold else None)
        ctx.cfg = (N, H, O, B, float(slope), float(p if step is not None else 0.0), int(seed))
        ctx.fold = (float(in_act[0]), float(in_act[1] if in_act[3] is not None else 0.0), int(in_act[2])) if fold else None
        ctx.side = side if fold else None
        if loss is not None:
            ctx.mark_non_differentiable(gout)
            ctx.set_materialize_grads(False)
            return out, gout
        return out

    @staticmethod
    def _backward_train_fused(ctx, g):
        gx, ws, gout, ntot = ctx.train_fused
        N, H, O, B, slope, p, seed = ctx.cfg
        if g is None or g.data_ptr() != gout.data_ptr() or g.shape != gout.shape:
            raise RuntimeError("the read-out ran its backward inside forward_loss with the criterion's own gradient: call "
                               "out.backward(g) with the g forward_loss returned (or use forward() + a criterion)")
        nb = H * H + H + O * H + O
        grads = torch.empty(ntot, dtype=torch.float32, device=gx.device)
        loss_rows, loss_out = ctx.loss
        roles = [(_lib.ROLE_SUM_ROWS, (ws, grads), (_lib.load().qot_head_train_blocks(B, H), ntot, 0)),
                 (_lib.ROLE_SUM_ROWS, (loss_rows, loss_out), (B, 1, 0))]
        if LG.can_defer(*ctx.receivers, ctx.side.get("bias_param") if ctx.fold else None):
            for r in roles:
                LG.defer(*r, stage=1)
        else:
            _lib.run_roles([_lib.make_role(*r) for r in roles])
        if ctx.fold:
            ctx.side["gbias"] = grads[nb:]
        gw0 = grads[:H * H].view(H, H)
        gb0 = grads[H * H:H * H + H]
        gw3 = grads[H * H + H:H * H + H + O * H].view(O, H)
        gb3 = grads[H * H + H + O * H:H * H + H + O * H + O]
        return gx, None, gw0, gb0, gw3, gb3, None, None, None, None, None

    @staticmethod
    def backward(ctx, g, _g_gout=None):
        if ctx.train_fused is not None:
            return HeadFn._backward_train_fused(ctx, g)
        ptr32, w0, w3, pooled, hidden, step, x_in, in_step = ctx.saved_tensors
        N, H, O, B, slope, p, seed = ctx.cfg
        if g is None:
            g = torch.zeros(B, O, dtype=torch.float32, device=pooled.device)
        g = _f32c(g)
        dev = g.device
        gx = torch.empty(N, H, dtype=torch.float32, device=dev)
        nb = H * H + H + O * H + O
        ntot = nb + (H if ctx.fold else 0)
        grads = torch.empty(ntot, dtype=torch.float32, device=dev)
        ws = torch.empty(_lib.load().qot_head_bwd_workspace_floats(H, O), dtype=torch.float32, device=dev)
        fold_args = (P(x_in), ctx.fold[0], ctx.fold[1], ctx.fold[2], P(in_step)) if ctx.fold else (None, 0.0, 0.0, 0, None)
        grouped = LG.can_defer(*ctx.receivers, ctx.side.get("bias_param") if ctx.fold else None)
        _lib.call("qot_head_bwd", P(g), P(pooled), P(hidden), P(ptr32), P(w0), P(w3), P(gx), None if grouped else P(grads),
                  P(ws), B, H, O, slope, p, seed, P(step), *fold_args)
        if grouped:
            LG.defer(_lib.ROLE_SUM_ROWS, (ws, grads), (_lib.load().qot_head_bwd_blocks(B), ntot, 0), stage=1)
        if ctx.loss is not None:
            loss_rows, loss_out = ctx.loss
            role = (_lib.ROLE_SUM_ROWS, (loss_rows, loss_out), (B, 1, 0))
            if LG.enabled():
                LG.defer(*role, stage=1)
            else:
                _lib.run_roles([_lib.make_role(*role)])
        if ctx.fold:
            ctx.side["gbias"] = grads[nb:]
        gw0 = grads[:H * H].view(H, H)
        gb0 = grads[H * H:H * H + H]
        gw3 = grads[H * H + H:H * H + H + O * H].view(O, H)
        gb3 = grads[H * H + H + O * H:H * H + H + O * H + O]
        return gx, None, gw0, gb0, gw3, gb3, None, None, None, None, None


class GatFn(torch.autograd.Function):

    @staticmethod
    def forward(ctx, z, att_src, att_dst, bias, graph: GraphIndex, neg_slope: float, bn_stats: bool = False,
                a_src=None, a_dst=None):
        require_cuda(z, att_src, att_dst, bias)
        z, bias = _f32c(z), _f32c(bias)
        heads, C = att_src.shape[-2], att_src.shape[-1]
        att_s, att_d = _f32c(att_src).reshape(-1), _f32c(att_dst).reshape(-1)
        N, HC = z.shape
        dev = z.device
        if a_src is None or a_dst is None:
            a_src = torch.empty(N, heads, dtype=torch.float32, device=dev)
            a_dst = torch.empty(N, heads, dtype=torch.float32, device=dev)
            _lib.call("qot_gat_logits", P(z), P(att_s), P(att_d), P(a_src), P(a_dst), N, heads, C)
        else:
            a_src, a_dst = _f32c(a_src), _f32c(a_dst)
        out = torch.empty(N, HC, dtype=torch.float32, device=dev)
        stats = torch.empty(N, heads, 2, dtype=torch.float32, device=dev)
        partials = None
        if bn_stats and N > 0:
            partials = torch.empty(_lib.load().qot_gat_bn_partials_floats(N, heads, C), dtype=torch.float32, device=dev)
        _lib.call("qot_gat_fwd", P(z), P(a_src), P(a_dst), P(bias), P(graph.rowptr), P(graph.col), P(out),
                  P(stats), N, heads, C, float(neg_slope), P(partials))
        ctx.save_for_backward(z, a_src, a_dst, stats, att_s, att_d)
        ctx.graph, ctx.ns, ctx.att_shape = graph, float(neg_slope), tuple(att_src.shape)
        if bn_stats:
            if partials is None:
                partials = torch.empty(0, dtype=torch.float32, device=dev)
            ctx.mark_non_differentiable(partials)
            return out, partials
        return out

    @staticmethod
    def backward(ctx, g, _gp=None):
        z, a_src, a_dst, stats, att_s, att_d = ctx.saved_tensors
        graph, ns = ctx.graph, ctx.ns
        g = _f32c(g)
        N, HC = z.shape
        heads = a_src.shape[1]
        C = HC // heads
        dev = z.device
        gad = torch.empty(N, heads, dtype=torch.float32, device=dev)
        gas = torch.empty(N, heads, dtype=torch.float32, device=dev)
        gz = torch.empty(N, HC, dtype=torch.float32, device=dev)
        escr = torch.empty(max(graph.cap, 1), heads, 2, dtype=torch.float32, device=dev)
        delta = torch.empty(N, heads, dtype=torch.float32, device=dev)
        g_bias = torch.empty(HC, dtype=torch.float32, device=dev)
        ws = torch.empty(_lib.load().qot_gat_bn_partials_floats(N, heads, C), dtype=torch.float32, device=dev)
        _lib.call("qot_gat_bwd_dst", P(g), P(z), P(a_src), P(a_dst), P(stats), P(graph.rowptr), P(graph.col),
                  P(gad), P(escr), P(delta), N, heads, C, ns, P(g_bias), P(ws))
        _lib.call("qot_gat_bwd_src", P(g), P(a_src), P(a_dst), P(escr), P(delta), P(graph.rowptr_t),
                  P(graph.col_t), P(graph.pos_t), P(gz), P(gas), N, heads, C, ns, P(att_s), P(att_d), P(gad))
        g_att = torch.empty(2, HC, dtype=torch.float32, device=dev)
        _lib.call("qot_gat_att_grad", P(z), P(gas), P(gad), _off(g_att, 0), _off(g_att, HC), P(ws), N, heads, C)
        return gz, g_att[0].view(ctx.att_shape), g_att[1].view(ctx.att_shape), g_bias, None, None, None, None, None


def gat_thin_ok(x: torch.Tensor, heads: int, C: int) -> bool:
    if os.environ.get("QOT_NO_GAT_THIN", "0") == "1" or not x.is_cuda or x.dtype != torch.float32 or x.requires_grad:
        return False
    if x.dim() != 2 or x.shape[0] < int(os.environ.get("QOT_GAT_THIN_MIN_ROWS", "32768")) or not skinny_ok(x.shape[1], 4):
        return False
    return bool(_lib.load().qot_gat_thin_supported(heads, C, x.shape[1]))


def _skinny_dw(g, x):
    N, C = g.shape
    F = x.shape[1]
    nblk = _lib.load().qot_skinny_linear_dw_blocks(N)
    part = torch.empty(nblk, C * F, dtype=torch.float32, device=g.device)
    _lib.call("qot_skinny_linear_dw", P(g), P(x), P(part), N, F, C)
    gw = torch.empty(C * F, dtype=torch.float32, device=g.device)
    _lib.run_roles([_lib.make_role(_lib.ROLE_SUM_ROWS, (part, gw), (nblk, C * F, 0))])
    return gw.view(C, F)


class GatThinFn(torch.autograd.Function):

    @staticmethod
    def forward(ctx, x, lin_weight, att_src, att_dst, bias, graph: GraphIndex, neg_slope: float, bn_stats: bool = False):
        require_cuda(x, lin_weight, att_src, att_dst, bias)
        x, w, bias = _f32c(x), _f32c(lin_weight), _f32c(bias)
        heads, C = att_src.shape[-2], att_src.shape[-1]
        N, F = x.shape
        HC = heads * C
        dev = x.device
        w3 = w.view(heads, C, F)
        v_src = (w3 * _f32c(att_src).view(heads, C, 1)).sum(1).contiguous()
        v_dst = (w3 * _f32c(att_dst).view(heads, C, 1)).sum(1).contiguous()
        a_src = torch.empty(N, heads, dtype=torch.float32, device=dev)
        a_dst = torch.empty(N, heads, dtype=torch.float32, device=dev)
        _lib.call("qot_skinny_linear_fwd", P(x), P(v_src), P(a_src), N, F, heads)
        _lib.call("qot_skinny_linear_fwd", P(x), P(v_dst), P(a_dst), N, F, heads)
        out = torch.empty(N, HC, dtype=torch.float32, device=dev)
        stats = torch.empty(N, heads, 2, dtype=torch.float32, device=dev)
        partials = None
        if bn_stats and N > 0:
            partials = torch.empty(_lib.load().qot_gat_bn_partials_floats(N, heads, C), dtype=torch.float32, device=dev)
        _lib.call("qot_gat_fwd_thin", P(x), F, P(w), P(a_src), P(a_dst), P(bias), P(graph.rowptr), P(graph.col), P(out),
                  P(stats), N, heads, C, float(neg_slope), P(partials))
        ctx.save_for_backward(x, w, a_src, a_dst, stats, _f32c(att_src).reshape(-1), _f32c(att_dst).reshape(-1))
        ctx.graph, ctx.ns, ctx.att_shape = graph, float(neg_slope), tuple(att_src.shape)
        if bn_stats:
            if partials is None:
                partials = torch.empty(0, dtype=torch.float32, device=dev)
            ctx.mark_non_differentiable(partials)
            return out, partials
        return out

    @staticmethod
    def backward(ctx, g, _gp=None):
        x, w, a_src, a_dst, stats, att_s, att_d = ctx.saved_tensors
        graph, ns = ctx.graph, ctx.ns
        g = _f32c(g)
        N, F = x.shape
        heads = a_src.shape[1]
        HC = w.shape[0]
        C = HC // heads
        dev = x.device
        gad = torch.empty(N, heads, dtype=torch.float32, device=dev)
        gas = torch.empty(N, heads, dtype=torch.float32, device=dev)
        gz = torch.empty(N, HC, dtype=torch.float32, device=dev)
        escr = torch.empty(max(graph.cap, 1), heads, 2, dtype=torch.float32, device=dev)
        delta = torch.empty(N, heads, dtype=torch.float32, device=dev)
        g_bias = torch.empty(HC, dtype=torch.float32, device=dev)
        ws = torch.empty(_lib.load().qot_gat_bn_partials_floats(N, heads, C), dtype=torch.float32, device=dev)
        _lib.call("qot_gat_bwd_dst_thin", P(g), P(x), F, P(w), P(a_src), P(a_dst), P(stats), P(graph.rowptr), P(graph.col),
                  P(gad), P(escr), P(delta), N, heads, C, ns, P(g_bias), P(ws))
        _lib.call("qot_gat_bwd_src", P(g), P(a_src), P(a_dst), P(escr), P(delta), P(graph.rowptr_t),
                  P(graph.col_t), P(graph.pos_t), P(gz), P(gas), N, heads, C, ns, P(att_s), P(att_d), P(gad))
        g_lin = _skinny_dw(gz, x)
        w3 = w.view(heads, C, F)
        g_att_src = (w3 * _skinny_dw(gas, x).view(heads, 1, F)).sum(-1)
# ... 330 lines not shown
```

### include/qot_gnn.h

```cpp
#ifndef QOT_GNN_H
#define QOT_GNN_H

#include <stddef.h>
#include <stdint.h>

#ifdef __cplusplus
extern "C" {
#endif

typedef void* qot_stream_t;

#define QOT_ABI_VERSION 11
#define QOT_OK 0
#define QOT_ERR_UNSUPPORTED (-1)
#define QOT_ERR_BADARG (-2)

int qot_abi_version(void);
const char* qot_error_string(int code);

size_t qot_csr_workspace_bytes(int64_t E, int64_t N, int gat_self_loops);
int qot_csr_build(const int64_t* edge_index, int64_t E, int64_t N, int gat_self_loops,
                  int32_t* rowptr, int32_t* col, int32_t* eid, int32_t* row,
                  int32_t* rowptr_t, int32_t* col_t, int32_t* pos_t, int32_t* eid_t, float* invdeg,
                  void* workspace, size_t workspace_bytes, qot_stream_t stream);
int qot_csr_build_by_graph(const int64_t* edge_index, int64_t E, int64_t N, const int64_t* node_ptr,
                           const int64_t* edge_ptr, int64_t B, int64_t max_nodes, int64_t max_edges,
                           int32_t* rowptr, int32_t* col, int32_t* eid, int32_t* row, int32_t* rowptr_t,
                           int32_t* col_t, int32_t* pos_t, int32_t* eid_t, float* invdeg, int32_t* status,
                           const int64_t* node_ids, int32_t* ids32, int32_t* colf, int32_t* colf_t, int32_t* ptr32,
                           qot_stream_t stream);
int qot_csr_gat_by_graph_supported(int64_t max_nodes, int64_t max_edges);
int qot_csr_build_gat_by_graph(const int64_t* edge_index, int64_t E, int64_t N, const int64_t* node_ptr,
                               const int64_t* edge_ptr, int64_t B, int64_t max_nodes, int64_t max_edges, int32_t* rowptr,
                               int32_t* col, int32_t* eid, int32_t* row, int32_t* rowptr_t, int32_t* col_t, int32_t* pos_t,
                               int32_t* eid_t, float* invdeg, int32_t* status, int32_t* ptr32, qot_stream_t stream);
int qot_i32_gather(const int32_t* map, const int32_t* idx, int32_t* out, int64_t n, qot_stream_t stream);
int qot_i64_to_i32(const int64_t* in, int32_t* out, int64_t n, qot_stream_t stream);
int qot_batch_ptr(const int32_t* batch, int64_t N, int64_t B, int32_t* ptr, qot_stream_t stream);

int qot_embed_fwd(const float* table, const int32_t* ids, float* out, int64_t N, int V, int H,
                  qot_stream_t stream);
int qot_embed_bwd(const float* grad_out, const int32_t* ids, float* grad_table, int64_t N, int V,
                  int H, qot_stream_t stream);

int qot_tconv_fwd_scores(const float* q, const float* v, const float* skip, int ld, const float* scores, int ld_scores,
                         const float* edge_attr, const float* w_edge, const int32_t* rowptr, const int32_t* col,
                         const int32_t* eid, const int32_t* rowmap, float* out, float* stats, int64_t N, int H, int D,
                         int act, float act_slope, float act_p, uint64_t act_seed, const int64_t* act_step,
                         qot_stream_t stream);
int qot_tconv_rows_supported(int n, int H, int D);
int qot_tconv_rows_npad(int n);
int qot_tconv_rows_ld(int n, int H, int D);
int qot_tconv_bwd_dst_rows(const float* grad_out, const float* q, const float* v, int ld, const float* edge_attr,
                           const float* w_edge, const float* stats, const int32_t* rowptr, const int32_t* colf,
                           const int32_t* eid, const float* scores, int ld_scores, float* grad_skip, float* escr, float* delta,
                           const float* y_act, float act_slope, float act_p, uint64_t act_seed, const int64_t* act_step, int n,
                           int64_t B, int parts, float* part_rows, float* wedge_partials, int H, int D, qot_stream_t stream);
int qot_tconv_fwd_rows(const float* q, const float* v, const float* skip, int ld, const float* scores, int ld_scores,
                       const float* edge_attr, const float* w_edge, const int32_t* rowptr, const int32_t* colf, const int32_t* eid,
                       float* out, float* stats, int n, int64_t B, int parts, int H, int D, int act, float act_slope, float act_p,
                       uint64_t act_seed, const int64_t* act_step, qot_stream_t stream);
int qot_tconv_bwd_src_rows(const float* grad_skip, const float* escr, const int32_t* rowptr_t, const int32_t* col_t,
                           const int32_t* pos_t, int n, int64_t B, int parts, float* part_rows, int H, qot_stream_t stream);
int qot_tconv_fwd(const float* q, const float* k, const float* v, const float* skip, int ld,
                  const float* edge_attr, const float* w_edge, const int32_t* rowptr,
                  const int32_t* col, const int32_t* eid, const int32_t* rowmap, float* out,
                  float* stats, int64_t N, int H, int D, int act, float act_slope, float act_p,
                  uint64_t act_seed, const int64_t* act_step, qot_stream_t stream);
int qot_tconv_fwd_tile(const float* q, const float* k, const float* v, const float* skip, int ld,
                       const float* edge_attr, const float* w_edge, const int32_t* rowptr, const int32_t* col,
                       const int32_t* eid, const int32_t* rowmap, float* out, float* stats, int64_t N, int H, int D,
                       int tile_n, int64_t tile_B, int act, float act_slope, float act_p, uint64_t act_seed,
                       const int64_t* act_step, qot_stream_t stream);
int qot_tconv_rows_per_block(int H);
int64_t qot_tconv_bwd_dst_blocks(int64_t N, int H, int tile_n, int64_t tile_B);
size_t qot_tconv_bwd_dst_workspace_floats(int64_t N, int H, int D);
int qot_tconv_bwd_dst(const float* grad_out, const float* q, const float* k, const float* v, int ld,
                      const float* edge_attr, const float* w_edge, const float* stats,
                      const int32_t* rowptr, const int32_t* col, const int32_t* eid,
                      const int32_t* rowmap, float* grad_q, float* grad_skip, int ld_g, float* escr,
                      float* delta, float* pds, float* pal, const float* y_act, float act_slope, float act_p,
                      uint64_t act_seed, const int64_t* act_step, float* grad_w_edge, float* workspace,
                      int tile_n, int64_t tile_B, float* grad_part, int64_t N, int H, int D, qot_stream_t stream);
int qot_tconv_bwd_src(const float* grad_out, int ld_go, const float* q, int ld, const float* escr,
                      const float* delta, const int32_t* rowptr_t, const int32_t* col_t,
                      const int32_t* pos_t, const int32_t* qmap_t, float* grad_k, float* grad_v,
                      int ld_g, int tile_n, int64_t tile_B, float* grad_part, int64_t N, int H,
                      qot_stream_t stream);

int qot_tconv_graph_supported(int n, int max_e, int H, int D);
int qot_tconv_graph_ldm(int n);
size_t qot_tconv_graph_row_floats(int n, int H, int D);
int qot_tconv_bwd_graph_blocks(int64_t B);
int qot_table_scores(const float* table, const float* wq, const float* bq, const float* wk, const float* bk,
                     const float* w_edge, float* M, float* P, int n, int H, int D, qot_stream_t stream);
int qot_tconv_fwd_graph(const float* t4, int ld, const float* M, const float* P, const float* w_edge,
                        const float* edge_attr, const int32_t* rowptr, const int32_t* colf, const int32_t* eid,
                        const int32_t* row, float* out, float* alpha, float* ea_csr, float* aa, int n, int64_t B, int max_e,
                        int H, int D, int act, float act_slope, float act_p, uint64_t act_seed, const int64_t* act_step,
                        qot_stream_t stream);
int qot_tconv_bwd_graph(const float* grad_out, const float* y_act, float act_slope, float act_p, uint64_t act_seed,
                        const int64_t* act_step, const float* t4, int ld, const float* w_edge, const float* ea_csr,
                        const float* alpha, const float* aa, const int32_t* rowptr, const int32_t* colf,
                        const int32_t* row, const int32_t* rowptr_t, const int32_t* col_t, const int32_t* pos_t,
                        float* partials, int n, int64_t B, int max_e, int H, int D, qot_stream_t stream);
int qot_table_project_bwd_scores(const float* S, const float* t4, const float* w_edge, const float* table,
                                 const float* wq, const float* wk, const float* wv, const float* ws, float* grad_table,
                                 float* grad_w, float* grad_b, float* grad_w_edge, int V, int n, int H, int D,
                                 qot_stream_t stream);

int qot_nnconv_agg(const float* x, int ld_x, const float* edge_attr, const float* w1,
                   const float* b1, const int32_t* rowptr, const int32_t* col,
                   const int32_t* eid_or_pos, const int32_t* eid_of_pos, const float* invdeg,
                   int transpose, float* A, int64_t N, int H, int D, qot_stream_t stream);
int qot_nnconv_fused(const float* x, int ld_x, const float* edge_attr, const float* w1,
                     const float* b1, const int32_t* rowptr, const int32_t* col,
                     const int32_t* edge_ids, const float* invdeg, int transpose,
                     const float* w_perm, const float* bias, float* out, int64_t N, int H, int D,
                     int act, float act_slope, float act_p, uint64_t act_seed, const int64_t* act_step,
                     qot_stream_t stream);
size_t qot_gemm_tn_workspace_floats(int KT);
int qot_gemm_tn(const float* A, int lda, const float* G, int ldg, int64_t N, int KT, float* C,
                float* workspace, qot_stream_t stream);
size_t qot_nnconv_adjoint_dw_workspace_floats(int D);
int qot_nnconv_adjoint_dw(const float* grad_out, int ld_g, const float* x, int ld_x,
                          const float* edge_attr, const float* w1, const float* b1,
                          const int32_t* rowptr_t, const int32_t* col_t, const int32_t* eid_t,
                          const float* invdeg, const float* w_perm, float* grad_x, float* gwcat_t, int param_layout,
                          float* workspace, int64_t N, int H, int D, qot_stream_t stream);
size_t qot_nnconv_gradh_workspace_floats(int D);
int qot_nnconv_gradh_fused(const float* grad_out, int ld_g, const float* x, int ld_x,
                           const float* edge_attr, const float* w1, const float* b1,
                           const int32_t* rowptr, const int32_t* col, const int32_t* eid,
                           const float* invdeg, const float* b_perm, float* gw1, float* gb1,
                           float* workspace, int64_t N, int H, int D, qot_stream_t stream);
size_t qot_nnconv_dw_workspace_floats(int64_t N, int H, int D);
int qot_nnconv_dw(const float* x, int ld_x, const float* grad_out, int ld_g, const float* edge_attr,
                  const float* w1, const float* b1, const int32_t* rowptr, const int32_t* col,
                  const int32_t* eid, const float* invdeg, float* grad_params, float* workspace, int64_t N,
                  int H, int D, qot_stream_t stream);
int qot_nnconv_bwd_finalize(const float* adj_workspace, const float* gradh_workspace, float* grad_params,
                            float* gw1, float* gb1, int64_t N, int H, int D, qot_stream_t stream);
int qot_nnconv_bwd_edge(const float* GA, int ld_ga, const float* x, int ld_x,
                        const float* edge_attr, const float* w1, const float* b1,
                        const int32_t* rowptr, const int32_t* col, const int32_t* eid,
                        const float* invdeg, float* gw1, float* gb1, int64_t N, int H, int D,
                        qot_stream_t stream);

int qot_tconv_edge_attr_grad(const float* grad_out, const float* y_act, float act_slope, float act_p, uint64_t act_seed,
                             const int64_t* act_step, const float* qkvs, int ld, const int32_t* rowmap, const int32_t* col,
                             const int32_t* rowptr, const int32_t* eid, const float* edge_attr, const float* w_edge,
                             float* grad_edge_attr, int64_t N, int H, int D, qot_stream_t stream);
int qot_nnconv_edge_attr_grad(const float* GA, int ld_ga, const float* x, int ld_x, const float* edge_attr,
                              const float* w1, const float* b1, const int32_t* rowptr, const int32_t* col,
                              const int32_t* eid, const float* invdeg, float* grad_edge_attr, int64_t N, int H, int D,
                              qot_stream_t stream);

int qot_act_fwd(const float* x, float* y, int64_t n, float slope, float p, uint64_t seed,
                const int64_t* step_counter, qot_stream_t stream);
int qot_act_bwd(const float* grad_y, const float* y_or_x, float* grad_x, int64_t n, float slope,
                float p, uint64_t seed, const int64_t* step_counter, qot_stream_t stream);

int qot_pool_fwd(const float* x, const int32_t* ptr, float* out, int64_t B, int H,
                 qot_stream_t stream);
int qot_pool_bwd(const float* grad_out, const int32_t* ptr, const int32_t* batch, float* grad_x,
                 int64_t N, int64_t B, int H, qot_stream_t stream);

int qot_gat_blocks(int64_t N, int heads, int C);
size_t qot_gat_bn_partials_floats(int64_t N, int heads, int C);
int qot_gat_logits(const float* z, const float* att_src, const float* att_dst, float* a_src, float* a_dst,
                   int64_t N, int heads, int C, qot_stream_t stream);
int qot_gat_fwd(const float* z, const float* a_src, const float* a_dst, const float* bias,
                const int32_t* rowptr, const int32_t* col, float* out, float* stats, int64_t N,
                int heads, int C, float neg_slope, float* bn_partials, qot_stream_t stream);
int qot_gat_thin_supported(int heads, int C, int K);
int qot_gat_fwd_thin(const float* x, int K, const float* w, const float* a_src, const float* a_dst, const float* bias,
                     const int32_t* rowptr, const int32_t* col, float* out, float* stats, int64_t N, int heads, int C,
                     float neg_slope, float* bn_partials, qot_stream_t stream);
int qot_gat_bwd_dst_thin(const float* grad_out, const float* x, int K, const float* w, const float* a_src,
                         const float* a_dst, const float* stats, const int32_t* rowptr, const int32_t* col,
                         float* grad_a_dst, float* escr, float* delta, int64_t N, int heads, int C, float neg_slope,
                         float* grad_bias, float* workspace, qot_stream_t stream);
int qot_gat_bwd_dst(const float* grad_out, const float* z, const float* a_src, const float* a_dst,
                    const float* stats, const int32_t* rowptr, const int32_t* col, float* grad_a_dst,
                    float* escr, float* delta, int64_t N, int heads, int C, float neg_slope,
                    float* grad_bias, float* workspace, qot_stream_t stream);
int qot_gat_bwd_src(const float* grad_out, const float* a_src, const float* a_dst, const float* escr,
                    const float* delta, const int32_t* rowptr_t, const int32_t* col_t,
                    const int32_t* pos_t, float* grad_z, float* grad_a_src, int64_t N, int heads,
                    int C, float neg_slope, const float* att_src, const float* att_dst,
                    const float* grad_a_dst, qot_stream_t stream);
int qot_gat_att_grad(const float* z, const float* grad_a_src, const float* grad_a_dst, float* grad_att_src,
                     float* grad_att_dst, float* workspace, int64_t N, int heads, int C, qot_stream_t stream);

size_t qot_bn_partials_floats(int64_t N, int C);
int qot_bn_stats(const float* x, int64_t N, int C, float eps, float momentum, float* mean,
                 float* rstd, float* running_mean, float* running_var, float* partials,
                 qot_stream_t stream);
int64_t qot_gat_chunk_rows(int64_t N, int heads, int C);
int qot_bn_stats_from_partials(const float* shift, const float* partials, int nblk, int64_t chunk_rows, int64_t N, int C,
                               float eps, float momentum, float* mean, float* rstd, float* running_mean,
                               float* running_var, qot_stream_t stream);
int qot_bn_apply(const float* x, const float* mean, const float* rstd, const float* w,
                 const float* b, float* y, int64_t N, int C, int relu, qot_stream_t stream);
int qot_bn_bwd_reduce(const float* grad_y, const float* y, const float* x, const float* mean,
                      const float* rstd, float* gw, float* gb, int64_t N, int C, int relu,
                      float* partials, const float* w, const float* b, qot_stream_t stream);
int qot_bn_bwd_apply(const float* grad_y, const float* y, const float* x, const float* mean,
                     const float* rstd, const float* w, const float* gw, const float* gb,
                     float* grad_x, int64_t N, int C, int relu, int batch_stats, const float* b,
                     qot_stream_t stream);
int qot_bn_apply_rows(const float* x, const int32_t* idx, int64_t n, const float* mean, const float* rstd, const float* w,
                      const float* b, float* y_rows, int C, int relu, qot_stream_t stream);
int qot_bn_bwd_reduce_rows(const float* grad_rows, const int32_t* idx, int64_t n, const float* x, const float* mean,
                           const float* rstd, float* gw, float* gb, int C, int relu, float* partials, const float* w,
                           const float* b, qot_stream_t stream);
int qot_bn_bwd_apply_rows(const float* grad_rows, const int32_t* idx, int64_t n, const float* x, const float* mean,
                          const float* rstd, const float* w, const float* gw, const float* gb, float* grad_x, int64_t N,
                          int C, int relu, const float* b, qot_stream_t stream);

int qot_sgd_momentum(float* param, const float* grad, float* momentum_buf, int64_t n, float lr,
                     float momentum, int first_step, qot_stream_t stream);
int qot_sgd_momentum_multi(float* param, const float* const* grads, const int64_t* offsets, int count,
                           float* grad_flat, float* momentum_buf, int64_t n, float lr, const float* lr_dev,
                           float momentum, int first_step, qot_stream_t stream);
int qot_sgd_momentum_dev(float* param, const float* grad, float* momentum_buf, int64_t n, const float* lr_dev,
                         float momentum, int first_step, qot_stream_t stream);
int qot_small_gemm(const float* A, int64_t stride_am, int64_t stride_ak, const float* B, int64_t stride_bk,
                   int64_t stride_bn, const float* bias, float* C, int ldc, int M, int N, int K,
                   int split_k, qot_stream_t stream);
size_t qot_colsum_workspace_floats(int C);
size_t qot_rowsum_wide_workspace_floats(int64_t C);
int qot_rowsum_wide(const float* x, int64_t B, int64_t C, float* out, float* workspace, qot_stream_t stream);
int qot_colsum(const float* x, int ld, int64_t N, int C, float* out, float* workspace, qot_stream_t stream);
int qot_act_bwd_colsum(const float* grad_y, const float* y, float* grad_x, int64_t N, int C, float slope, float p,
                       uint64_t seed, const int64_t* step_counter, float* colsum_out, float* workspace,
                       qot_stream_t stream);

int qot_head_fwd(const float* x, const int32_t* ptr, const float* w0, const float* b0, const float* w3,
                 const float* b3, float* pooled, float* hidden, float* out, int64_t B, int H, int O,
                 float slope, float p, uint64_t seed, const int64_t* step_counter, qot_stream_t stream);
int qot_head_fwd_loss(const float* x, const int32_t* ptr, const float* w0, const float* b0, const float* w3,
                      const float* b3, float* pooled, float* hidden, float* out, int64_t B, int H, int O,
                      float slope, float p, uint64_t seed, const int64_t* step_counter, const float* target,
                      float beta, float* grad_out, float* loss_rows, qot_stream_t stream);
int qot_head_train_blocks(int64_t B, int H);
int qot_head_train(const float* x, const int32_t* ptr, const float* w0, const float* b0, const float* w3, const float* b3,
                   const float* target, float beta, float* out, float* grad_out, float* loss_rows, float* grad_x,
                   float* workspace, int64_t B, int H, int O, float slope, float p, uint64_t seed,
                   const int64_t* step_counter, int fold, float in_slope, float in_p, uint64_t in_seed,
                   const int64_t* in_step, qot_stream_t stream);
size_t qot_head_bwd_workspace_floats(int H, int O);
int qot_head_bwd_blocks(int64_t B);
int qot_head_bwd(const float* grad_out, const float* pooled, const float* hidden, const int32_t* ptr,
                 const float* w0, const float* w3, float* grad_x, float* grads, float* workspace, int64_t B,
                 int H, int O, float slope, float p, uint64_t seed, const int64_t* step_counter,
                 const float* x_in, float in_slope, float in_p, uint64_t in_seed, const int64_t* in_step,
                 qot_stream_t stream);

size_t qot_smooth_l1_workspace_floats(void);
int qot_smooth_l1(const float* pred, const float* target, int64_t n, float beta, float* loss, float* grad,
                  float* workspace, qot_stream_t stream);

int qot_table_project_fwd(const float* table, const float* wq, const float* bq, const float* wk, const float* bk,
                          const float* wv, const float* bv, const float* ws, const float* bs, float* out, int V,
                          int H, int64_t* step_counter, int64_t* step_snapshot, qot_stream_t stream);
int qot_table_project_bwd(const float* grad_out, const float* table, const float* wq, const float* wk,
                          const float* wv, const float* ws, float* grad_table, float* grad_w, float* grad_b, int V,
                          int H, qot_stream_t stream);

int qot_table_maps(const int64_t* node_ids, const int32_t* col, const int32_t* col_t, int32_t* ids32,
                   int32_t* colf, int32_t* colf_t, int64_t N, int64_t E, qot_stream_t stream);
int qot_step_advance(int64_t* counter, int64_t* snapshot, qot_stream_t stream);

int qot_gather3(const float* s0, int64_t n0, const float* s1, int64_t n1, const float* s2, const int32_t* idx,
                float* out, int64_t n, qot_stream_t stream);

int qot_gemm_nt(const float* A, int64_t lda, const float* B, int64_t ldb, float* C, int64_t ldc, int64_t M, int N, int K,
                const float* scale, const float* shift, const float* bias, qot_stream_t stream);
int qot_gemm_nt_logits(const float* A, int64_t lda, const float* B, int64_t ldb, float* C, int64_t ldc, int64_t M, int N, int K,
                       const float* scale, const float* shift, const float* bias, const float* att_src,
                       const float* att_dst, float* a_src, float* a_dst, qot_stream_t stream);
int qot_gemm_nt_planes(const float* A, int64_t lda, const float* B, int64_t ldb, float* Cpart, int64_t M, int N, int K,
                       int kslices, qot_stream_t stream);
int qot_gemm_tn_splits(int M, int N, int64_t K);
int qot_gemm256_takes(int64_t M, int N);
int qot_gemm_tn_planes(const float* A, int64_t lda, const float* B, int64_t ldb, float* Cpart, int M, int N, int64_t K,
                       int splits, const float* scale, const float* shift, qot_stream_t stream);

int qot_skinny_linear_fwd(const float* x, const float* w, float* out, int64_t N, int F, int C, qot_stream_t stream);
int qot_skinny_linear_fwd_logits(const float* x, const float* w, float* out, int64_t N, int F, int C, const float* att_src,
                                 const float* att_dst, float* a_src, float* a_dst, qot_stream_t stream);
int qot_skinny_linear_dw_blocks(int64_t N);
int qot_skinny_linear_dw(const float* g, const float* x, float* partials, int64_t N, int F, int C, qot_stream_t stream);

#define QOT_MAX_ROLES 12
enum {
    QOT_ROLE_CSR_BY_GRAPH = 1,
    QOT_ROLE_TABLE_PROJECT_FWD = 2,
    QOT_ROLE_GATHER3 = 3,
    QOT_ROLE_SUM_ROWS = 4,
    QOT_ROLE_NNCONV_FINALIZE64 = 5,
    QOT_ROLE_TABLE_PROJECT_BWD = 6,
    QOT_ROLE_TABLE_SCORES = 7,
    QOT_ROLE_TABLE_PROJECT_BWD_SCORES = 8
};
typedef struct qot_role {
    int32_t kind;
    int32_t reserved;
    const void* p[18];
    int64_t i[8];
} qot_role_t;
int qot_run_roles(const qot_role_t* roles, int n_roles, qot_stream_t stream);

int qot_rows_gather(const float* x, const int32_t* idx, float* out, int64_t n_idx, int C,
                    qot_stream_t stream);
int qot_rows_scatter(const float* grad_out, const int32_t* idx, float* grad_x, int64_t n_idx, int C,
                     qot_stream_t stream);

#ifdef __cplusplus
}
#endif
#endif
```

Baseline: 2.134 million graphs/s.

## Use three-plane bf16 split weights for NNConv forward and gradh MFMA

After: 2.330 million graphs/s, median of 6. +9.2%, better.

```diff
diff --git a/gnn_qot_estimation_amd/_lib.py b/gnn_qot_estimation_amd/_lib.py
--- a/gnn_qot_estimation_amd/_lib.py
+++ b/gnn_qot_estimation_amd/_lib.py
@@ -17,7 +17,7 @@
 _u64 = C.c_uint64
 _sz = C.c_size_t
 
-ABI_VERSION = 11
+ABI_VERSION = 12
 
 SIGNATURES = {
     "qot_abi_version": (_int, []),
@@ -68,6 +68,10 @@
     "qot_nnconv_agg": (_int, [_p, _int, _p, _p, _p, _p, _p, _p, _p, _p, _int, _p, _i64, _int, _int, _p]),
     "qot_nnconv_fused": (_int, [_p, _int, _p, _p, _p, _p, _p, _p, _p, _int, _p, _p, _p, _i64, _int, _int,
                                 _int, _f, _f, _u64, _p, _p]),
+    "qot_nnconv_fused_split": (_int, [_p, _int, _p, _p, _p, _p, _p, _p, _p, _p, _i64, _p, _p, _i64, _int, _int,
+                                      _int, _f, _f, _u64, _p, _p]),
+    "qot_nnconv_gradh_split": (_int, [_p, _int, _p, _int, _p, _p, _p, _p, _p, _p, _p, _p, _i64, _p, _p, _p, _i64, _int,
+                                      _int, _p]),
     "qot_nnconv_bwd_finalize": (_int, [_p, _p, _p, _p, _p, _i64, _int, _int, _p]),
     "qot_nnconv_dw_workspace_floats": (_sz, [_i64, _int, _int]),
     "qot_nnconv_dw": (_int, [_p, _int, _p, _int, _p, _p, _p, _p, _p, _p, _p, _p, _p, _i64, _int, _int, _p]),
diff --git a/gnn_qot_estimation_amd/csrc/nnconv_gradh64.hip b/gnn_qot_estimation_amd/csrc/nnconv_gradh64.hip
--- a/gnn_qot_estimation_amd/csrc/nnconv_gradh64.hip
+++ b/gnn_qot_estimation_amd/csrc/nnconv_gradh64.hip
@@ -1,5 +1,6 @@
 #include "common.hpp"
 #include "mfma_tile.hpp"
+#include "split_bf16.hpp"
 
 namespace qot {
 
@@ -7,12 +8,13 @@
 
 constexpr int kGhCap = 256;
 
-template <int D, int VARIANT = 0>
+template <int D, int VARIANT = 0, bool SPLIT = false>
 __global__ __launch_bounds__(256, 2) void nnconv_gradh64_kernel(
     const float* __restrict__ g, int ldg, const float* __restrict__ x, int ldx, const float* __restrict__ ea,
     const float* __restrict__ w1, const float* __restrict__ b1, const int32_t* __restrict__ rowptr,
     const int32_t* __restrict__ col, const int32_t* __restrict__ eidx, const float* __restrict__ invdeg,
-    const float* __restrict__ Bp, float* __restrict__ partials, int64_t N) {
+    const float* __restrict__ Bp, float* __restrict__ partials, int64_t N, const u32x4* __restrict__ Bs = nullptr,
+    int64_t bs_planes = 0) {
     constexpr int K = 2 * D;
     static_assert(K <= 8, "one k per lane of the 8-lane group");
     constexpr int NB = K * 2;
@@ -86,8 +88,14 @@
         const int64_t tile0 = tile * 32;
         const int64_t i = tile0 + il;
         const int64_t tend = (tile0 + 32 < N) ? tile0 + 32 : N;
+        constexpr int SL = 3;
         float4 bf[2][8];
-        {
+        Bf3 bsp[SL + 1];
+        const u32x4* bsw = Bs + (int64_t)(wave * NBW) * 4 * 64 + lane;
+        if constexpr (SPLIT) {
+#pragma unroll
+            for (int s = 0; s < SL; ++s) bsp[s] = load_split_b(bsw + s * 64, bs_planes);
+        } else {
             const float4* bp = reinterpret_cast<const float4*>(Bp) + (int64_t)(wave * NBW) * 8 * 64 + lane;
 #pragma unroll
             for (int gq = 0; gq < 8; ++gq) bf[0][gq] = bp[gq * 64];
@@ -126,7 +134,26 @@
                 xr0[t] = ld4(xp); xr1[t] = ld4(xp + 4);
             }
         }
-        if (VARIANT != 3) {
+        if (SPLIT) {
+#pragma unroll 1
+            for (int t = 0; t < NBW; ++t) {
+                const int nb = wave * NBW + t;
+                f32x16 c;
+#pragma unroll
+                for (int r = 0; r < 16; ++r) c[r] = 0.f;
+#pragma unroll
+                for (int s = 0; s < 4; ++s) {
+                    const int q = 4 * t + s;
+                    if (q + SL < 4 * NBW) bsp[(s + SL) % (SL + 1)] = load_split_b(bsw + (q + SL) * 64, bs_planes);
+                    c = mfma_split_step(Gt4, 2 * s, hi, r31, bsp[s], c);
+                }
+#pragma unroll
+                for (int r = 0; r < 16; ++r) {
+                    const int row = (r & 3) + 8 * (r >> 2) + 4 * hi;
+                    GAt[row * LDGA + nb * 32 + r31] = c[r];
+                }
+            }
+        } else if (VARIANT != 3) {
             float4 af[8];
 #pragma unroll
             for (int gq = 0; gq < 8; ++gq) af[gq] = Gt4[at4_slot(gq, hi, r31)];
@@ -217,7 +244,8 @@
 
 int qot_nnconv_gradh64_launch(const float* grad_out, int ld_g, const float* x, int ld_x, const float* edge_attr, const float* w1,
                               const float* b1, const int32_t* rowptr, const int32_t* col, const int32_t* eid, const float* invdeg,
-                              const float* b_perm, float* workspace, int64_t N, int D, int grid, int variant, hipStream_t stream) {
+                              const float* b_perm, const void* b_split, int64_t split_stride, float* workspace, int64_t N, int D,
+                              int grid, int variant, hipStream_t stream) {
 #ifdef QOT_DIAG
     if (variant >= 1 && variant <= 5 && D == 4) {
 #define QOT_GH_V(V) nnconv_gradh64_kernel<4, V><<<grid, 256, 0, stream>>>(grad_out, ld_g, x, ld_x, edge_attr, w1, b1, rowptr, col, \
@@ -235,6 +263,16 @@
     }
 #endif
     (void)variant;
+    if (b_split) {
+        QOT_DISPATCH_D(D, {
+            if (kD <= 4)
+                nnconv_gradh64_kernel<(kD <= 4 ? kD : 4), 0, true><<<grid, 256, 0, stream>>>(
+                    grad_out, ld_g, x, ld_x, edge_attr, w1, b1, rowptr, col, eid, invdeg, nullptr, workspace, N,
+                    static_cast<const u32x4*>(b_split), split_stride / 8);
+        });
+        QOT_LAUNCH_CHECK();
+        return QOT_OK;
+    }
     QOT_DISPATCH_D(D, {
         if (kD <= 4)
             nnconv_gradh64_kernel<(kD <= 4 ? kD : 4)><<<grid, 256, 0, stream>>>(
diff --git a/gnn_qot_estimation_amd/csrc/nnconv_mfma.hip b/gnn_qot_estimation_amd/csrc/nnconv_mfma.hip
--- a/gnn_qot_estimation_amd/csrc/nnconv_mfma.hip
+++ b/gnn_qot_estimation_amd/csrc/nnconv_mfma.hip
@@ -1,6 +1,7 @@
 #include "common.hpp"
 #include "mfma_tile.hpp"
 #include "nnconv_finalize_dev.hpp"
+#include "split_bf16.hpp"
 
 namespace qot {
 
@@ -115,12 +116,14 @@
 #define QOT_STAMP(slot)
 #endif
 
-template <int D, bool TRANSPOSE, int VARIANT = 0>
+template <int D, bool TRANSPOSE, int VARIANT = 0, bool SPLIT = false>
 __global__ __launch_bounds__(256, 2) void nnconv_mfma64_kernel(
     const float* __restrict__ x, int ldx, const float* __restrict__ ea, const float* __restrict__ w1,
     const float* __restrict__ b1, const int32_t* __restrict__ rowptr, const int32_t* __restrict__ col,
     const int32_t* __restrict__ eidx, const float* __restrict__ invdeg, const float* __restrict__ Wp,
-    const float* __restrict__ bias, float* __restrict__ out, int64_t N, ActParams act) {
+    const float* __restrict__ bias, float* __restrict__ out, int64_t N, ActParams act,
+    const u32x4* __restrict__ Ws = nullptr, int64_t ws_planes = 0) {
+    static_assert(!SPLIT || (!TRANSPOSE && VARIANT == 0), "split form: production forward only");
     constexpr int K = 2 * D;
     constexpr int KM = (K + 1) * 64;
     constexpr int GM = KM / 16;
@@ -153,6 +156,61 @@
     const int lane = threadIdx.x & 63, wave = threadIdx.x >> 6;
     const int nh = wave & 1, kh = wave >> 1;
     const int r31 = lane & 31, hi = lane >> 5;
+    f32x16 c;
+#pragma unroll
+    for (int r = 0; r < 16; ++r) c[r] = 0.f;
+    if constexpr (SPLIT) {
+        constexpr int ST = (K + 2) * 64 / 16;
+        constexpr int SM = GM / 2;
+        constexpr int SC = 2;
+        constexpr int NCS = SM / SC;
+        constexpr int NBS = 3;
+        static_assert(GM % 4 == 0, "chunking");
+        const u32x4* wsn = Ws + (int64_t)nh * ST * 64 + lane;
+        const u32x4* wsp = wsn + (int64_t)kh * SM * 64;
+        const u32x4* rsp = wsn + (int64_t)(2 * SM + 2 * kh) * 64;
+        asm volatile("" : "+v"(rsp));
+        Bf3 rbs[2];
+#pragma unroll
+        for (int u = 0; u < 2; ++u) rbs[u] = load_split_b(rsp + u * 64, ws_planes);
+        Bf3 sb[NBS][SC];
+#pragma unroll
+        for (int q = 0; q < NBS - 1; ++q)
+#pragma unroll
+            for (int u = 0; u < SC; ++u) sb[q][u] = load_split_b(wsp + (q * SC + u) * 64, ws_planes);
+        lds_barrier();
+        int ch = 0;
+#pragma unroll 1
+        for (; ch + NBS <= NCS; ch += NBS) {
+#pragma unroll
+            for (int q = 0; q < NBS; ++q) {
+                if (ch + q + NBS - 1 < NCS) {
+#pragma unroll
+                    for (int u = 0; u < SC; ++u)
+                        sb[(q + NBS - 1) % NBS][u] = load_split_b(wsp + ((ch + q + NBS - 1) * SC + u) * 64, ws_planes);
+                }
+#pragma unroll
+                for (int u = 0; u < SC; ++u) c = mfma_split_step(At4, kh * GM + 2 * ((ch + q) * SC + u), hi, r31, sb[q][u], c);
+            }
+        }
+#pragma unroll
+        for (int q = 0; q < NBS - 1; ++q) {
+            if (ch + q < NCS) {
+#pragma unroll
+                for (int u = 0; u < SC; ++u) c = mfma_split_step(At4, kh * GM + 2 * ((ch + q) * SC + u), hi, r31, sb[q][u], c);
+            }
+        }
+        lds_barrier();
+        {
+            float4* At4w = reinterpret_cast<float4*>(At);
+            const int sub = threadIdx.x & 7, il = threadIdx.x >> 3;
+            At4w[at4_slot(sub, 0, il)] = make_float4(root0.x, root0.z, root1.x, root1.z);
+            At4w[at4_slot(sub, 1, il)] = make_float4(root0.y, root0.w, root1.y, root1.w);
+        }
+        __syncthreads();
+#pragma unroll
+        for (int u = 0; u < 2; ++u) c = mfma_split_step(At4, kh * 4 + 2 * u, hi, r31, rbs[u], c);
+    } else {
     const float4* wpn = reinterpret_cast<const float4*>(Wp) + (int64_t)nh * (2 * GM + 8) * 64 + lane;
     const float4* wp = wpn + (int64_t)kh * GM * 64;
     const float4* rbp = wpn + (int64_t)(2 * GM + kh * 4) * 64;
@@ -176,9 +234,6 @@
         continue;
     }
 
-    f32x16 c;
-#pragma unroll
-    for (int r = 0; r < 16; ++r) c[r] = 0.f;
     int ch = 0;
 #pragma unroll 1
     for (; ch + NB <= NCH; ch += NB) {
@@ -221,6 +276,7 @@
     __syncthreads();
 #pragma unroll
     for (int u = 0; u < 4; ++u) c = mfma_group(At4, kh * 4 + u, hi, r31, rb[u], c);
+    }
     QOT_STAMP(4)
     float* red = At + 64 * 32;
     if (kh) {
@@ -679,23 +735,52 @@
     return QOT_OK;
 }
 
+extern "C" int qot_nnconv_fused_split(const float* x, int ld_x, const float* edge_attr, const float* w1,
+                                      const float* b1, const int32_t* rowptr, const int32_t* col,
+                                      const int32_t* edge_ids, const float* invdeg, const void* w_split,
+                                      int64_t split_stride, const float* bias, float* out, int64_t N, int H, int D,
+                                      int act, float act_slope, float act_p, uint64_t act_seed,
+                                      const int64_t* act_step, qot_stream_t stream) {
+    if (N < 0 || !rowptr) return QOT_ERR_BADARG;
+    if (H != 64 || D > 4) return QOT_ERR_UNSUPPORTED;
+    if (N == 0) return QOT_OK;
+    if (!x || !w1 || !b1 || !invdeg || !w_split || !out || (ld_x & 3) || ((uintptr_t)w_split & 15) || (split_stride & 7) ||
+        split_stride < (int64_t)(2 * D + 2) * 4096)
+        return QOT_ERR_BADARG;
+    int grid = grid_for(N, 32);
+    if (grid > 2 * num_cus()) grid = 2 * num_cus();
+    const ActParams ap = make_act(act, act_slope, act_p, act_seed, act_step);
+    QOT_DISPATCH_D(D, {
+        if (kD <= 4)
+            nnconv_mfma64_kernel<(kD <= 4 ? kD : 4), false, 0, true><<<grid, 256, 0, (hipStream_t)stream>>>(
+                x, ld_x, edge_attr, w1, b1, rowptr, col, edge_ids, invdeg, nullptr, bias, out, N, ap,
+                static_cast<const u32x4*>(w_split), split_stride / 8);
+    });
+    QOT_LAUNCH_CHECK();
+    return QOT_OK;
+}
+
 int qot_nnconv_gradh64_launch(const float* grad_out, int ld_g, const float* x, int ld_x, const float* edge_attr, const float* w1,
                               const float* b1, const int32_t* rowptr, const int32_t* col, const int32_t* eid, const float* invdeg,
-                              const float* b_perm, float* workspace, int64_t N, int D, int grid, int variant, hipStream_t stream);
+                              const float* b_perm, const void* b_split, int64_t split_stride, float* workspace, int64_t N, int D,
+                              int grid, int variant, hipStream_t stream);
 extern "C" size_t qot_nnconv_gradh_workspace_floats(int D) {
     return (size_t)2 * 256 * 2 * (size_t)(2 * D * (D + 1));
 }
 
-extern "C" int qot_nnconv_gradh_fused(const float* grad_out, int ld_g, const float* x, int ld_x,
-                                      const float* edge_attr, const float* w1, const float* b1,
-                                      const int32_t* rowptr, const int32_t* col, const int32_t* eid,
-                                      const float* invdeg, const float* b_perm, float* gw1, float* gb1,
-                                      float* workspace, int64_t N, int H, int D, qot_stream_t stream_) {
+static int nnconv_gradh_impl(const float* grad_out, int ld_g, const float* x, int ld_x,
+                             const float* edge_attr, const float* w1, const float* b1,
+                             const int32_t* rowptr, const int32_t* col, const int32_t* eid,
+                             const float* invdeg, const float* b_perm, const void* b_split, int64_t split_stride,
+                             float* gw1, float* gb1,
+                             float* workspace, int64_t N, int H, int D, qot_stream_t stream_) {
     hipStream_t stream = (hipStream_t)stream_;
     if (N < 0 || !rowptr) return QOT_ERR_BADARG;
     if ((H != 16 && H != 32 && H != 64 && H != 128 && H != 256) || D > 4) return QOT_ERR_UNSUPPORTED;
-    if (!grad_out || !x || !w1 || !b1 || !invdeg || !b_perm || (!gw1 != !gb1) || !workspace || (ld_g & 3) || (ld_x & 3))
+    if (!grad_out || !x || !w1 || !b1 || !invdeg || !(b_perm || b_split) || (!gw1 != !gb1) || !workspace || (ld_g & 3) ||
+        (ld_x & 3) || ((uintptr_t)b_split & 15) || (b_split && ((split_stride & 7) || split_stride < (int64_t)2 * D * 64 * 64)))
         return QOT_ERR_BADARG;
+    if (b_split && H != 64) return QOT_ERR_UNSUPPORTED;
     if (!gw1 && H != 64) return QOT_ERR_UNSUPPORTED;
 #ifdef QOT_DIAG
     if (H == 64 && g_variant == 9)
@@ -714,7 +799,7 @@
 #endif
     {
         const int rc = qot_nnconv_gradh64_launch(grad_out, ld_g, x, ld_x, edge_attr, w1, b1, rowptr, col, eid, invdeg, b_perm,
-                                                 workspace, N, D, grid, variant, stream);
+                                                 b_split, split_stride, workspace, N, D, grid, variant, stream);
         if (rc != QOT_OK) return rc;
     }
     QOT_LAUNCH_CHECK();
@@ -723,6 +808,26 @@
     gradh_partial_sum_kernel<<<grid_for(n, 4), 256, 0, stream>>>(workspace, grid, n, K * D, gw1, gb1);
     QOT_LAUNCH_CHECK();
     return QOT_OK;
+}
+
+extern "C" int qot_nnconv_gradh_fused(const float* grad_out, int ld_g, const float* x, int ld_x,
+                                      const float* edge_attr, const float* w1, const float* b1,
+                                      const int32_t* rowptr, const int32_t* col, const int32_t* eid,
+                                      const float* invdeg, const float* b_perm, float* gw1, float* gb1,
+                                      float* workspace, int64_t N, int H, int D, qot_stream_t stream) {
+    return nnconv_gradh_impl(grad_out, ld_g, x, ld_x, edge_attr, w1, b1, rowptr, col, eid, invdeg, b_perm, nullptr, 0, gw1, gb1,
+                             workspace, N, H, D, stream);
+}
+
+extern "C" int qot_nnconv_gradh_split(const float* grad_out, int ld_g, const float* x, int ld_x,
+                                      const float* edge_attr, const float* w1, const float* b1,
+                                      const int32_t* rowptr, const int32_t* col, const int32_t* eid,
+                                      const float* invdeg, const void* b_split, int64_t split_stride, float* gw1, float* gb1,
+                                      float* workspace, int64_t N, int H, int D, qot_stream_t stream) {
+    if (!b_split) return QOT_ERR_BADARG;
+    return nnconv_gradh_impl(grad_out, ld_g, x, ld_x, edge_attr, w1, b1, rowptr, col, eid, invdeg, nullptr, b_split, split_stride,
+                             gw1, gb1,
+                             workspace, N, H, D, stream);
 }
 
 extern "C" int qot_nnconv_bwd_finalize(const float* adj_workspace, const float* gradh_workspace, float* grad_params,
diff --git a/gnn_qot_estimation_amd/csrc/roles.hip b/gnn_qot_estimation_amd/csrc/roles.hip
--- a/gnn_qot_estimation_amd/csrc/roles.hip
+++ b/gnn_qot_estimation_amd/csrc/roles.hip
@@ -60,7 +60,8 @@
     }
     case QOT_ROLE_GATHER3:
         gather3_body(rp<const float>(ro, 0), (int)ro.i[0], rp<const float>(ro, 1), (int)ro.i[1], rp<const float>(ro, 2),
-                     rp<const int32_t>(ro, 3), rp<float>(ro, 4), ro.i[2], (int64_t)vb);
+                     rp<const int32_t>(ro, 3), rp<float>(ro, 4), ro.i[2], (int64_t)vb, rp<const int32_t>(ro, 5),
+                     rp<uint16_t>(ro, 6), ro.i[3]);
         break;
     case QOT_ROLE_SUM_ROWS:
         sum_rows_body(rp<const float>(ro, 0), rp<float>(ro, 1), ro.i[0], ro.i[1], ro.i[2], (int)ro.i[3], vb,
@@ -149,10 +150,11 @@
         return QOT_OK;
     }
     case QOT_ROLE_GATHER3: {
-        const int64_t n0 = i[0], n1 = i[1], n = i[2];
-        if (n <= 0 || n0 < 0 || n1 < 0 || n0 + n1 > 0x7fffffff) return QOT_ERR_BADARG;
+        const int64_t n0 = i[0], n1 = i[1], n = i[2], m = i[3];
+        if (n <= 0 || n0 < 0 || n1 < 0 || m < 0 || n0 + n1 > 0x7fffffff) return QOT_ERR_BADARG;
         for (int k = 0; k < 5; ++k) if (!p[k]) return QOT_ERR_BADARG;
-        *blocks = (n + 255) / 256;
+        if (m > 0 && (!p[5] || !p[6])) return QOT_ERR_BADARG;
+        *blocks = (n + m + 255) / 256;
         return QOT_OK;
     }
     case QOT_ROLE_SUM_ROWS: {
diff --git a/gnn_qot_estimation_amd/csrc/small_dev.hpp b/gnn_qot_estimation_amd/csrc/small_dev.hpp
--- a/gnn_qot_estimation_amd/csrc/small_dev.hpp
+++ b/gnn_qot_estimation_amd/csrc/small_dev.hpp
@@ -1,5 +1,6 @@
 #pragma once
 #include "common.hpp"
+#include "split_bf16.hpp"
 
 namespace qot {
 
@@ -186,11 +187,21 @@
 
 __device__ __forceinline__ void gather3_body(const float* __restrict__ s0, int n0, const float* __restrict__ s1, int n1,
                                              const float* __restrict__ s2, const int32_t* __restrict__ idx,
-                                             float* __restrict__ out, int64_t n, int64_t vb) {
+                                             float* __restrict__ out, int64_t n, int64_t vb,
+                                             const int32_t* __restrict__ idx2 = nullptr,
+                                             uint16_t* __restrict__ out2 = nullptr, int64_t m = 0) {
     const int64_t i = vb * 256 + threadIdx.x;
-    if (i >= n) return;
-    const int v = idx[i];
-    out[i] = v < 0 ? 0.f : (v < n0 ? s0[v] : (v < n0 + n1 ? s1[v - n0] : s2[v - n0 - n1]));
-}
-
-}
+    if (i >= n + m) return;
+    const bool sp = i >= n;
+    const int v = sp ? idx2[i - n] : idx[i];
+    const float val = v < 0 ? 0.f : (v < n0 ? s0[v] : (v < n0 + n1 ? s1[v - n0] : s2[v - n0 - n1]));
+    if (!sp) {
+        out[i] = val;
+    } else {
+        uint16_t h, md, l;
+        split3(val, h, md, l);
+        out2[i - n] = h; out2[m + i - n] = md; out2[2 * m + i - n] = l;
+    }
+}
+
+}
diff --git a/gnn_qot_estimation_amd/csrc/split_bf16.hpp b/gnn_qot_estimation_amd/csrc/split_bf16.hpp
--- /dev/null
+++ b/gnn_qot_estimation_amd/csrc/split_bf16.hpp
@@ -0,0 +1,77 @@
+#pragma once
+#include "mfma_tile.hpp"
+
+namespace qot {
+
+typedef __bf16 bf16x8 __attribute__((ext_vector_type(8)));
+typedef unsigned int u32x4 __attribute__((ext_vector_type(4)));
+
+struct Bf3 {
+    bf16x8 h, m, l;
+};
+
+__device__ __forceinline__ uint32_t cvt_pk_bf16(float a, float b) {
+    typedef __bf16 bf16x2 __attribute__((ext_vector_type(2)));
+    bf16x2 p;
+    p[0] = (__bf16)a;
+    p[1] = (__bf16)b;
+    return __builtin_bit_cast(uint32_t, p);
+}
+
+__device__ __forceinline__ void split3(float x, uint16_t& h, uint16_t& m, uint16_t& l) {
+    const __bf16 bh = (__bf16)x;
+    const float r = x - (float)bh;
+    const __bf16 bm = (__bf16)r;
+    const __bf16 bl = (__bf16)(r - (float)bm);
+    h = __builtin_bit_cast(uint16_t, bh);
+    m = __builtin_bit_cast(uint16_t, bm);
+    l = __builtin_bit_cast(uint16_t, bl);
+}
+
+__device__ __forceinline__ Bf3 split8(float4 a, float4 b) {
+    const float v[8] = {a.x, a.y, a.z, a.w, b.x, b.y, b.z, b.w};
+    uint32_t h[4], m[4], l[4];
+#pragma unroll
+    for (int j = 0; j < 4; ++j) {
+        h[j] = cvt_pk_bf16(v[2 * j], v[2 * j + 1]);
+        asm("" : "+v"(h[j]));
+        float r0 = v[2 * j] - __uint_as_float(h[j] << 16), r1 = v[2 * j + 1] - __uint_as_float(h[j] & 0xffff0000u);
+        asm("" : "+v"(r0), "+v"(r1));
+        m[j] = cvt_pk_bf16(r0, r1);
+        asm("" : "+v"(m[j]));
+        float q0 = r0 - __uint_as_float(m[j] << 16), q1 = r1 - __uint_as_float(m[j] & 0xffff0000u);
+        asm("" : "+v"(q0), "+v"(q1));
+        l[j] = cvt_pk_bf16(q0, q1);
+    }
+    Bf3 s;
+    s.h = __builtin_bit_cast(bf16x8, (u32x4){h[0], h[1], h[2], h[3]});
+    s.m = __builtin_bit_cast(bf16x8, (u32x4){m[0], m[1], m[2], m[3]});
+    s.l = __builtin_bit_cast(bf16x8, (u32x4){l[0], l[1], l[2], l[3]});
+    return s;
+}
+
+__device__ __forceinline__ f32x16 mfma_split6(const Bf3& a, const Bf3& b, f32x16 c) {
+    c = __builtin_amdgcn_mfma_f32_32x32x16_bf16(a.h, b.l, c, 0, 0, 0);
+    c = __builtin_amdgcn_mfma_f32_32x32x16_bf16(a.l, b.h, c, 0, 0, 0);
+    c = __builtin_amdgcn_mfma_f32_32x32x16_bf16(a.m, b.m, c, 0, 0, 0);
+    c = __builtin_amdgcn_mfma_f32_32x32x16_bf16(a.h, b.m, c, 0, 0, 0);
+    c = __builtin_amdgcn_mfma_f32_32x32x16_bf16(a.m, b.h, c, 0, 0, 0);
+    c = __builtin_amdgcn_mfma_f32_32x32x16_bf16(a.h, b.h, c, 0, 0, 0);
+    return c;
+}
+
+__device__ __forceinline__ Bf3 load_split_b(const u32x4* __restrict__ p, int64_t ps) {
+    Bf3 b;
+    b.h = __builtin_bit_cast(bf16x8, p[0]);
+    b.m = __builtin_bit_cast(bf16x8, p[ps]);
+    b.l = __builtin_bit_cast(bf16x8, p[2 * ps]);
+    return b;
+}
+
+__device__ __forceinline__ f32x16 mfma_split_step(const float4* __restrict__ At4, int g, int hi, int r31, const Bf3& b,
+                                                  f32x16 c) {
+    const float4 a0 = At4[at4_slot(g, hi, r31)], a1 = At4[at4_slot(g + 1, hi, r31)];
+    return mfma_split6(split8(a0, a1), b, c);
+}
+
+}
diff --git a/gnn_qot_estimation_amd/functional.py b/gnn_qot_estimation_amd/functional.py
--- a/gnn_qot_estimation_amd/functional.py
+++ b/gnn_qot_estimation_amd/functional.py
@@ -653,14 +653,34 @@
     return packed[:n_f], packed[n_f:n_f + n_a], packed[n_f + n_a:]
 
 
+def nnconv_split_bf16() -> bool:
+    return os.environ.get("QOT_NNCONV_F32_MFMA", "0") != "1"
+
+
+def nnconv_split_index(k: int, device) -> torch.Tensor:
+    key = ("splitidx", k, str(device))
+    if key not in _PERM_CACHE:
+        allidx, n_f, n_a, n_g = nnconv_fused_indices(k, "cpu")
+        fwd = allidx[:n_f].view(2, -1, 2, 64, 4).permute(0, 1, 3, 2, 4)
+        gh = allidx[n_f + n_a:].view(2 * k, 4, 2, 64, 4).permute(0, 1, 3, 2, 4)
+        _PERM_CACHE[key] = torch.cat([fwd.reshape(-1), gh.reshape(-1)]).contiguous().to(device)
+    return _PERM_CACHE[key]
+
+
 def nnconv_pack(w2, b2, wroot, h: int, k: int, group=None):
     allidx, n_f, n_a, n_g = nnconv_fused_indices(k, w2.device) if h == 64 else nnconv_gen_indices(h, k, w2.device)
     packed = torch.empty(allidx.numel(), dtype=torch.float32, device=w2.device)
+    ptrs, ints = [w2, b2, wroot, allidx, packed], [w2.numel(), b2.numel(), allidx.numel()]
+    split = None
+    if h == 64 and nnconv_split_bf16():
+        sidx = nnconv_split_index(k, w2.device)
+        split = torch.empty(3 * sidx.numel(), dtype=torch.int16, device=w2.device)
+        ptrs, ints = ptrs + [sidx, split], ints + [sidx.numel()]
     if group is not None:
-        group.add(_lib.ROLE_GATHER3, (w2, b2, wroot, allidx, packed), (w2.numel(), b2.numel(), allidx.numel()))
+        group.add(_lib.ROLE_GATHER3, tuple(ptrs), tuple(ints))
     else:
-        _lib.call("qot_gather3", P(w2), w2.numel(), P(b2), b2.numel(), P(wroot), P(allidx), P(packed), allidx.numel())
-    return packed[:n_f], packed[n_f:n_f + n_a], packed[n_f + n_a:]
+        _lib.run_roles([_lib.make_role(_lib.ROLE_GATHER3, ptrs, ints)])
+    return packed[:n_f], packed[n_f:n_f + n_a], packed[n_f + n_a:], split
 
 
 GEN_WIDTHS = (16, 32, 128, 256)
@@ -739,12 +759,18 @@
             raise _lib.QotError("NNConv HIP path: edge_dim <= 8 (include/qot_gnn.h)")
         if D > 4:
             return NNConvFn._forward_wide_edge(ctx, x, edge_attr, w1, b1, w2, b2, wroot, bias, graph, act, side)
-        wp, wp_adj, bp = packed if packed is not None else nnconv_pack(w2, b2, wroot, hin, K)
+        wp, wp_adj, bp, split = packed if packed is not None else nnconv_pack(w2, b2, wroot, hin, K)
         out = torch.empty(N, hout, dtype=torch.float32, device=x.device)
-        _lib.call("qot_nnconv_fused", P(x), hin, P(edge_attr), P(w1), P(b1), P(graph.rowptr), P(graph.col),
-                  P(graph.eid), P(graph.invdeg), 0, P(wp), P(bias), P(out), N, hin, D, *_act_args(act))
+        if split is not None:
+            _lib.call("qot_nnconv_fused_split", P(x), hin, P(edge_attr), P(w1), P(b1), P(graph.rowptr), P(graph.col),
+                      P(graph.eid), P(graph.invdeg), P(split), split.numel() // 3, P(bias), P(out), N, hin, D,
+                      *_act_args(act))
+        else:
+            _lib.call("qot_nnconv_fused", P(x), hin, P(edge_attr), P(w1), P(b1), P(graph.rowptr), P(graph.col),
+                      P(graph.eid), P(graph.invdeg), 0, P(wp), P(bias), P(out), N, hin, D, *_act_args(act))
         ctx.save_for_backward(x, edge_attr, w1, b1, w2, b2, wroot, None, wp_adj, bp, out if act is not None else None,
-                              act[3] if act is not None else None)
+                              act[3] if act is not None else None, split)
+        ctx.n_wcat = wp.numel()
         ctx.graph = graph
         ctx.act = None if act is None else (act[0], act[1], act[2])
         ctx.side = side if act is not None else None
@@ -764,7 +790,7 @@
             out = torch.empty_like(pre)
             _lib.call("qot_act_fwd", P(pre), P(out), pre.numel(), *_act_args(act)[1:])
         ctx.save_for_backward(x, edge_attr, w1, b1, w2, b2, wroot, A, None, None, out if act is not None else None,
-                              act[3] if act is not None else None)
+                              act[3] if act is not None else None, None)
         ctx.graph = graph
         ctx.act = None if act is None else (act[0], act[1], act[2])
         ctx.side = side if act is not None else None
@@ -772,7 +798,7 @@
 
     @staticmethod
     def _backward_wide_edge(ctx, g, gbias):
-        x, edge_attr, w1, b1, w2, b2, wroot, A, _, _, _, _ = ctx.saved_tensors
+        x, edge_attr, w1, b1, w2, b2, wroot, A, _, _, _, _, _ = ctx.saved_tensors
         graph = ctx.graph
         N, hin = x.shape
         hout = wroot.shape[0]
@@ -799,7 +825,7 @@
 
     @staticmethod
     def backward(ctx, g):
-        x, edge_attr, w1, b1, w2, b2, wroot, A, wp_adj, bp, y, act_step = ctx.saved_tensors
+        x, edge_attr, w1, b1, w2, b2, wroot, A, wp_adj, bp, y, act_step, split = ctx.saved_tensors
         graph = ctx.graph
         g = _f32c(g)
         if ctx.side is not None:
@@ -829,14 +855,18 @@
         wsh = torch.empty(_lib.load().qot_nnconv_gradh_workspace_floats(D), dtype=torch.float32, device=dev)
         gpar = torch.empty((K + 2) * hh, dtype=torch.float32, device=dev)
         gradh_args = (P(g), hout, P(x), hin, P(edge_attr), P(w1), P(b1), P(graph.rowptr), P(graph.col), P(graph.eid),
-                      P(graph.invdeg), P(bp))
+                      P(graph.invdeg))
+        if split is not None:
+            gradh_fn, gradh_args = "qot_nnconv_gradh_split", gradh_args + (P(split[ctx.n_wcat:]), split.numel() // 3)
+        else:
+            gradh_fn, gradh_args = "qot_nnconv_gradh_fused", gradh_args + (P(bp),)
         if hin == 64 and not os.environ.get("QOT_SPLIT_NNCONV_BWD"):
             gx = torch.empty(N, hin, dtype=torch.float32, device=dev)
             ws = torch.empty(_lib.load().qot_nnconv_adjoint_dw_workspace_floats(D), dtype=torch.float32, device=dev)
             deferred = LG.can_defer(*ctx.receivers)
             fork_mode = os.environ.get("QOT_FORK", "off") if deferred else "off"
-            launch_gradh = lambda: _lib.call("qot_nnconv_gradh_fused", *gradh_args, None, None, P(wsh), N, hin, D)
-            keep = (g, x, edge_attr, w1, b1, graph.rowptr, graph.col, graph.eid, graph.invdeg, bp, wsh)
+            launch_gradh = lambda: _lib.call(gradh_fn, *gradh_args, None, None, P(wsh), N, hin, D)
+            keep = (g, x, edge_attr, w1, b1, graph.rowptr, graph.col, graph.eid, graph.invdeg, bp, split, wsh)
             if fork_mode == "before":
                 LG.fork(launch_gradh, keep=keep)
             _lib.call("qot_nnconv_adjoint_dw", P(g), hout, P(x), hin, P(edge_attr), P(w1), P(b1), P(graph.rowptr_t),
@@ -859,7 +889,7 @@
             ws = torch.empty(_lib.load().qot_nnconv_dw_workspace_floats(N, hin, D), dtype=torch.float32, device=dev)
             _lib.call("qot_nnconv_dw", P(x), hin, P(g), hout, P(edge_attr), P(w1), P(b1), P(graph.rowptr), P(graph.col),
                       P(graph.eid), P(graph.invdeg), P(gpar), P(ws), N, hin, D)
-            _lib.call("qot_nnconv_gradh_fused", *gradh_args, P(gw1), P(gb1), P(wsh), N, hin, D)
+            _lib.call(gradh_fn, *gradh_args, P(gw1), P(gb1), P(wsh), N, hin, D)
         gw2, gb2, gwroot = gpar[:hh * K].view(hh, K), gpar[hh * K:hh * (K + 1)], gpar[hh * (K + 1):].view(hout, hin)
         return gx, gea, gw1, gb1, gw2, gb2, gwroot, gbias, None, None, None, None
 
diff --git a/include/qot_gnn.h b/include/qot_gnn.h
--- a/include/qot_gnn.h
+++ b/include/qot_gnn.h
@@ -10,7 +10,7 @@
 
 typedef void* qot_stream_t;
 
-#define QOT_ABI_VERSION 11
+#define QOT_ABI_VERSION 12
 #define QOT_OK 0
 #define QOT_ERR_UNSUPPORTED (-1)
 #define QOT_ERR_BADARG (-2)
@@ -119,6 +119,12 @@
                      const float* w_perm, const float* bias, float* out, int64_t N, int H, int D,
                      int act, float act_slope, float act_p, uint64_t act_seed, const int64_t* act_step,
                      qot_stream_t stream);
+int qot_nnconv_fused_split(const float* x, int ld_x, const float* edge_attr, const float* w1,
+                           const float* b1, const int32_t* rowptr, const int32_t* col,
+                           const int32_t* edge_ids, const float* invdeg, const void* w_split,
+                           int64_t split_stride, const float* bias, float* out, int64_t N, int H, int D,
+                           int act, float act_slope, float act_p, uint64_t act_seed, const int64_t* act_step,
+                           qot_stream_t stream);
 size_t qot_gemm_tn_workspace_floats(int KT);
 int qot_gemm_tn(const float* A, int lda, const float* G, int ldg, int64_t N, int KT, float* C,
                 float* workspace, qot_stream_t stream);
@@ -133,6 +139,11 @@
                            const float* edge_attr, const float* w1, const float* b1,
                            const int32_t* rowptr, const int32_t* col, const int32_t* eid,
                            const float* invdeg, const float* b_perm, float* gw1, float* gb1,
+                           float* workspace, int64_t N, int H, int D, qot_stream_t stream);
+int qot_nnconv_gradh_split(const float* grad_out, int ld_g, const float* x, int ld_x,
+                           const float* edge_attr, const float* w1, const float* b1,
+                           const int32_t* rowptr, const int32_t* col, const int32_t* eid,
+                           const float* invdeg, const void* b_split, int64_t split_stride, float* gw1, float* gb1,
                            float* workspace, int64_t N, int H, int D, qot_stream_t stream);
 size_t qot_nnconv_dw_workspace_floats(int64_t N, int H, int D);
 int qot_nnconv_dw(const float* x, int ld_x, const float* grad_out, int ld_g, const float* edge_attr,
```
